# wyhuai/DDNM

Measured on AMD Instinct MI355X. Metric: restored images/sec @256×256, 100 DDIM steps, 4×SR; 1/2/4/8 GPU, higher is better.
Workload: dtype f32 (3x3 convolutions: fp32 operands carried as hi + lo fp16 halves, three fp16 MFMA products per product, fp32 accumulate -- operand error 2^-22, measured closer to fp64 than the fp32 MFMA kernel; everything else fp32); 1 GPU; celeba_hq.yml SVD sr_bicubic 4x, sigma_y=0, eta=0.85, T_sampling=100, batch_size=8 per GPU (BASELINE configs[1]); global_batch=8, image=3x256x256, parallelism=dp1 (image sharding)

## Files before the change

ddnm_amd/_lib.py:

```python
import ctypes
import os
from ctypes import POINTER, Structure, c_char_p, c_float, c_int32, c_int64, c_uint32, c_void_p

_HERE = os.path.dirname(os.path.abspath(__file__))
LIB_PATH = os.path.join(_HERE, "libddnm_hip.so")

c_f32p = c_void_p


class ConvDesc(Structure):
    _fields_ = [
        ("src0", c_void_p), ("src1", c_void_p), ("weight", c_void_p), ("bias", c_void_p),
        ("badd", c_void_p), ("res", c_void_p), ("gn_scale", c_void_p), ("gn_shift", c_void_p),
        ("out", c_void_p),
        ("B", c_int32), ("Hin", c_int32), ("Win", c_int32),
        ("C0", c_int32), ("C1", c_int32), ("Cout", c_int32),
        ("ksize", c_int32), ("stride", c_int32), ("pad", c_int32),
        ("Ho", c_int32), ("Wo", c_int32),
        ("ups", c_int32), ("gn_silu", c_int32), ("out_nchw", c_int32),
        ("badd_stride", c_int32), ("tile", c_int32),
        ("workspace", c_void_p), ("workspace_floats", c_int64),
        ("res_ups", c_int32), ("src_f16", c_int32),
        ("stats_out", c_void_p),
        ("skip0", c_void_p), ("skip1", c_void_p), ("skip_weight", c_void_p),
        ("SC0", c_int32), ("SC1", c_int32),
        ("acc_scale", c_float), ("flags", c_int32),
        ("amax_in", c_void_p),
    ]


class GemmDesc(Structure):
    _fields_ = [
        ("A", c_void_p), ("Bm", c_void_p), ("D", c_void_p), ("C", c_void_p),
        ("M", c_int32), ("N", c_int32), ("K", c_int32),
        ("lda", c_int32), ("ldb", c_int32), ("ldc", c_int32), ("ldd", c_int32),
        ("transb", c_int32), ("batch", c_int32), ("inner", c_int32),
        ("sAo", c_int64), ("sAi", c_int64), ("sBo", c_int64), ("sBi", c_int64),
        ("sCo", c_int64), ("sCi", c_int64), ("sDo", c_int64), ("sDi", c_int64),
        ("alpha", c_float), ("beta", c_float),
        ("transa", c_int32), ("reserved", c_int32),
    ]


class Conv16Desc(Structure):
    _fields_ = [
        ("src", c_void_p), ("weight", c_void_p), ("bias", c_void_p), ("res", c_void_p),
        ("skip0", c_void_p), ("skip1", c_void_p), ("skip_weight", c_void_p),
        ("out", c_void_p), ("stats_out", c_void_p),
        ("workspace", c_void_p), ("workspace_floats", c_int64),
        ("B", c_int32), ("H", c_int32), ("W", c_int32),
        ("Cin", c_int32), ("Cout", c_int32), ("ksize", c_int32),
        ("ups", c_int32), ("res_ups", c_int32),
        ("SC0", c_int32), ("SC1", c_int32),
        ("src1", c_void_p), ("gn_scale", c_void_p), ("gn_shift", c_void_p),
        ("C0", c_int32), ("gn_silu", c_int32),
        ("out_nchw_f32", c_int32), ("reserved", c_int32),
        ("fin_gamma", c_void_p), ("fin_beta", c_void_p), ("fin_film", c_void_p),
        ("fin_scale", c_void_p), ("fin_shift", c_void_p),
        ("fin_eps", c_float), ("fin_film_stride", c_int32), ("fin_groups", c_int32), ("reserved2", c_int32),
    ]


class StepScalars(Structure):
    _fields_ = [("sqrt_1m_at", c_float), ("sqrt_at", c_float), ("sqrt_at_next", c_float),
                ("c1", c_float), ("c2", c_float), ("lam", c_float),
                ("rng_on", c_uint32), ("rng_seed_lo", c_uint32), ("rng_seed_hi", c_uint32), ("rng_iter", c_uint32),
                ("rng_image_base", c_uint32), ("reserved_rng", c_uint32)]


PROTOTYPES = {
    "ddnm_version": (c_int32, []),
    "ddnm_error_string": (c_char_p, [c_int32]),
    "ddnm_build_digest": (c_char_p, []),
    "ddnm_sizeof": (c_int32, [c_int32]),
    "ddnm_conv2d_f32": (c_int32, [POINTER(ConvDesc), c_void_p]),
    "ddnm_conv3x3_small_cout_f32": (c_int32, [POINTER(ConvDesc), c_void_p]),
    "ddnm_conv3x3_small_cout_f32_supported": (c_int32, [POINTER(ConvDesc)]),
    "ddnm_conv2d_f32_tile_n": (c_int32, [POINTER(ConvDesc)]),
    "ddnm_conv2d_f32_workspace_floats": (c_int64, [POINTER(ConvDesc)]),
    "ddnm_conv2d_f32_stats_tiles": (c_int32, [POINTER(ConvDesc)]),
    "ddnm_conv2d_f32_fuses_skip": (c_int32, [POINTER(ConvDesc)]),
    "ddnm_spectral_mix_f32": (c_int32, [c_void_p, c_void_p, c_void_p, c_int64, c_void_p, c_int64, c_float, c_float, c_float,
                                        c_float, c_int32, c_void_p]),
    "ddnm_hq_x0_f32": (c_int32, [c_void_p, c_void_p, c_int64, c_void_p, c_int32, c_int64, c_float, c_float, c_int32,
                                 c_void_p]),
    "ddnm_hq_project_f32": (c_int32, [c_void_p, c_void_p, c_void_p, c_void_p, c_int64, c_float, c_void_p]),
    "ddnm_copy_rect_f32": (c_int32, [c_void_p, c_int32, c_int32, c_int32, c_int32, c_void_p, c_int32, c_int32, c_int32,
                                     c_int32, c_int32, c_int32, c_int32, c_void_p]),
    "ddnm_hq_sample_f32": (c_int32, [c_void_p, c_void_p, c_void_p, c_void_p, c_void_p, c_int64, c_float, c_float, c_float,
                                     c_float, c_void_p]),
    "ddnm_patchify_f32": (c_int32, [c_void_p, c_void_p, c_int32, c_int32, c_int32, c_int32, c_void_p]),
    "ddnm_im2col3x3_f16": (c_int32, [c_void_p, c_void_p, c_void_p, c_void_p, c_void_p, c_int32, c_int32, c_int32, c_int32,
                                     c_int32, c_int32, c_void_p]),
    "ddnm_gn_apply_f16": (c_int32, [c_void_p, c_void_p, c_void_p, c_void_p, c_void_p, c_int32, c_int32, c_int32, c_int32,
                                    c_int32, c_void_p]),
    "ddnm_gn_finalize_tiles_f32": (c_int32, [c_void_p, c_int32, c_int32, c_void_p, c_int32, c_int32, c_void_p, c_void_p,
                                             c_int32, c_int32, c_int32, c_float, c_void_p, c_void_p, c_void_p, c_int32,
                                             c_void_p, c_void_p]),
    "ddnm_gn_finalize_tiles_amax_f32": (c_int32, [c_void_p, c_int32, c_int32, c_void_p, c_int32, c_int32, c_void_p, c_void_p,
                                                  c_int32, c_int32, c_int32, c_float, c_void_p, c_void_p, c_void_p, c_int32,
                                                  c_void_p, c_void_p, c_void_p]),
    "ddnm_amax_bound_f32": (c_int32, [c_void_p, c_int64, c_int32, c_void_p, c_int64, c_int32, c_void_p, c_int32, c_void_p]),
    "ddnm_conv3x3_f16_f32": (c_int32, [POINTER(ConvDesc), c_void_p]),
    "ddnm_conv3x3_f16_supported": (c_int32, [POINTER(ConvDesc)]),
    "ddnm_conv3x3_f16_workspace_floats": (c_int64, [POINTER(ConvDesc)]),
    "ddnm_conv3x3_f16_stats_tiles": (c_int32, [POINTER(ConvDesc)]),
    "ddnm_conv3x3_s16_f32": (c_int32, [POINTER(ConvDesc), c_void_p]),
    "ddnm_conv3x3_s16_supported": (c_int32, [POINTER(ConvDesc)]),
    "ddnm_conv3x3_s16_persistent": (c_int32, [POINTER(ConvDesc)]),
    "ddnm_conv3x3_s16_workspace_floats": (c_int64, [POINTER(ConvDesc)]),
    "ddnm_conv3x3_s16_stats_tiles": (c_int32, [POINTER(ConvDesc)]),
    "ddnm_conv3x3_s16_act_scale": (c_float, []),
    "ddnm_conv_gather_s16_f32": (c_int32, [POINTER(ConvDesc), c_void_p]),
    "ddnm_conv_gather_s16_supported": (c_int32, [POINTER(ConvDesc)]),
    "ddnm_conv_gather_s16_workspace_floats": (c_int64, [POINTER(ConvDesc)]),
    "ddnm_conv_gather_s16_stats_tiles": (c_int32, [POINTER(ConvDesc)]),
    "ddnm_conv16": (c_int32, [POINTER(Conv16Desc), c_void_p]),
    "ddnm_conv16_supported": (c_int32, [POINTER(Conv16Desc)]),
    "ddnm_conv16_fuses_fin": (c_int32, [POINTER(Conv16Desc)]),
    "ddnm_conv16_workspace_floats": (c_int64, [POINTER(Conv16Desc)]),
    "ddnm_conv16_stats_tiles": (c_int32, [POINTER(Conv16Desc)]),
    "ddnm_gn_apply_h16": (c_int32, [c_void_p, c_void_p, c_void_p, c_void_p, c_void_p, c_int32, c_int32, c_int32, c_int32,
                                    c_int32, c_int32, c_int32, c_void_p]),
    "ddnm_im2col3x3_h16": (c_int32, [c_void_p, c_void_p, c_void_p, c_void_p, c_void_p, c_int32, c_int32, c_int32, c_int32,
                                     c_int32, c_int32, c_void_p]),
    "ddnm_nchw_to_nhwc_h16": (c_int32, [c_void_p, c_void_p, c_int32, c_int32, c_int32, c_int32, c_void_p]),
    "ddnm_gn_stats_h16": (c_int32, [c_void_p, c_void_p, c_int32, c_int32, c_int32, c_int32, c_void_p]),
    "ddnm_attn16_d64": (c_int32, [c_void_p, c_void_p, c_int32, c_int32, c_int32, c_void_p]),
    "ddnm_conv1x1_f16_f32": (c_int32, [POINTER(ConvDesc), c_void_p]),
    "ddnm_conv1x1_f16_supported": (c_int32, [POINTER(ConvDesc)]),
    "ddnm_conv1x1_f16_workspace_floats": (c_int64, [POINTER(ConvDesc)]),
    "ddnm_conv1x1_f16_stats_tiles": (c_int32, [POINTER(ConvDesc)]),
    "ddnm_gn_stats_f32": (c_int32, [c_void_p, c_void_p, c_int32, c_int32, c_int32, c_int32, c_int32, c_void_p,
                                    c_int32, c_void_p]),
    "ddnm_gn_nchunk": (c_int32, [c_int32, c_int32]),
    "ddnm_gn_finalize_f32": (c_int32, [c_void_p, c_int32, c_void_p, c_void_p, c_int32, c_int32, c_int32, c_int32,
                                       c_float, c_void_p, c_void_p, c_void_p, c_int32, c_void_p, c_void_p]),
    "ddnm_bgemm_f32": (c_int32, [POINTER(GemmDesc), c_void_p]),
    "ddnm_gn_bwd_f32": (c_int32, [c_void_p, c_void_p, c_int32, c_void_p, c_void_p, c_void_p, c_int32, c_void_p, c_int32,
                                  c_int32, c_int32, c_int32, c_int32, c_int32, c_void_p, c_int32, c_void_p, c_void_p,
                                  c_void_p]),
    "ddnm_gn_bwd_nchunk": (c_int32, [c_int32, c_int32]),
    "ddnm_gn_bwd_h16": (c_int32, [c_void_p, c_void_p, c_int32, c_void_p, c_void_p, c_void_p, c_int32, c_void_p, c_int32,
                                  c_int32, c_int32, c_int32, c_int32, c_int32, c_void_p, c_int32, c_void_p, c_void_p,
                                  c_void_p]),
    "ddnm_pool_tokens_h16": (c_int32, [c_void_p, c_void_p, c_void_p, c_void_p, c_void_p, c_int32, c_int32, c_int32,
                                       c_void_p]),
    "ddnm_pool_tokens_bwd_h16": (c_int32, [c_void_p, c_void_p, c_int32, c_int32, c_int32, c_void_p]),
    "ddnm_attn16_d64_lse": (c_int32, [c_void_p, c_void_p, c_void_p, c_int32, c_int32, c_int32, c_void_p]),
    "ddnm_attn16_d64_bwd": (c_int32, [c_void_p, c_void_p, c_void_p, c_void_p, c_void_p, c_void_p, c_int32, c_int32,
                                      c_int32, c_void_p]),
    "ddnm_softmax_bwd_rows_f32": (c_int32, [c_void_p, c_void_p, c_int64, c_int32, c_int32, c_float, c_void_p]),
    "ddnm_pool_tokens_f32": (c_int32, [c_void_p, c_void_p, c_void_p, c_void_p, c_void_p, c_int32, c_int32, c_int32,
                                       c_void_p]),
    "ddnm_pool_attn_fwd_f32": (c_int32, [c_void_p, c_void_p, c_void_p, c_int32, c_int32, c_int32, c_int32, c_void_p]),
    "ddnm_pool_attn_bwd_f32": (c_int32, [c_void_p, c_void_p, c_void_p, c_void_p, c_int32, c_int32, c_int32, c_int32,
                                         c_void_p]),
    "ddnm_pool_tokens_bwd_f32": (c_int32, [c_void_p, c_void_p, c_int32, c_int32, c_int32, c_void_p]),
    "ddnm_logsoftmax_grad_f32": (c_int32, [c_void_p, c_void_p, c_void_p, c_int32, c_int32, c_void_p]),
    "ddnm_softmax_rows_f32": (c_int32, [c_void_p, c_int64, c_int32, c_int32, c_float, c_void_p]),
    "ddnm_linear_f32": (c_int32, [c_void_p, c_void_p, c_void_p, c_void_p, c_int32, c_int32, c_int32, c_int32,
                                  c_void_p]),
    "ddnm_timestep_embedding_f32": (c_int32, [c_void_p, c_void_p, c_void_p, c_int32, c_int32, c_int32, c_void_p]),
    "ddnm_avgpool2_nhwc_f32": (c_int32, [c_void_p, c_void_p, c_void_p, c_int32, c_void_p, c_int32, c_int32, c_int32,
                                         c_int32, c_void_p]),
    "ddnm_embedding_add_f32": (c_int32, [c_void_p, c_void_p, c_void_p, c_int32, c_int32, c_int32, c_void_p]),
    "ddnm_nchw_im2col3x3_pad_f32": (c_int32, [c_void_p, c_void_p, c_int32, c_int32, c_int32, c_int32, c_int32, c_void_p]),
    "ddnm_nchw_to_nhwc_pad_f32": (c_int32, [c_void_p, c_void_p, c_int32, c_int32, c_int32, c_int32, c_void_p]),
    "ddnm_step_x0_f32": (c_int32, [c_void_p, c_void_p, c_int64, c_void_p, c_int32, c_int64, POINTER(StepScalars),
                                   c_void_p]),
    "ddnm_step_combine_f32": (c_int32, [c_void_p, c_void_p, c_void_p, c_void_p, c_void_p, c_int64, c_void_p,
                                        c_int32, c_int64, POINTER(StepScalars), c_void_p]),
    "ddnm_step_sr_avgpool_f32": (c_int32, [c_void_p, c_void_p, c_int64, c_void_p, c_void_p, c_void_p, c_void_p,
                                           c_int32, c_int32, c_int32, c_int32, POINTER(StepScalars), c_void_p]),
    "ddnm_step_color_f32": (c_int32, [c_void_p, c_void_p, c_int64, c_void_p, c_void_p, c_void_p, c_void_p,
                                      c_int32, c_int32, POINTER(c_float), POINTER(StepScalars), c_void_p]),
    "ddnm_step_inpaint_f32": (c_int32, [c_void_p, c_void_p, c_int64, c_void_p, c_void_p, c_void_p, c_int32,
                                        c_void_p, c_void_p, c_int32, c_int32, POINTER(StepScalars), c_void_p]),
    "ddnm_step_denoise_f32": (c_int32, [c_void_p, c_void_p, c_int64, c_void_p, c_void_p, c_void_p, c_void_p,
                                        c_int32, c_int64, POINTER(StepScalars), c_void_p]),
    "ddnm_axpby_f32": (c_int32, [c_void_p, c_void_p, c_void_p, c_int64, c_float, c_float, c_void_p]),
    "ddnm_axpby_strided_f32": (c_int32, [c_void_p, c_int64, c_void_p, c_void_p, c_int32, c_int64, c_float, c_float,
                                         c_void_p]),
    "ddnm_mask_mix_f32": (c_int32, [c_void_p, c_void_p, c_void_p, c_int32, c_int64, c_void_p, c_int64, c_float, c_float,
                                    c_float, c_float, c_void_p]),
    "ddnm_site_spectral_f32": (c_int32, [c_void_p, c_void_p, c_void_p, c_int32, c_int32, c_int32, c_int32, c_int32,
                                         c_int32, c_int32, c_void_p, c_int32, c_float, c_float, c_float, c_float,
                                         c_void_p]),
    "ddnm_gather_scale_f32": (c_int32, [c_void_p, c_void_p, c_void_p, c_void_p, c_int32, c_int64, c_int64, c_void_p]),
    "ddnm_site_matmul_f32": (c_int32, [c_void_p, c_void_p, c_void_p, c_int32, c_int64, c_int32, c_int64, c_int64, c_int64,
                                       c_int32, c_void_p]),
    "ddnm_mul_planes_f32": (c_int32, [c_void_p, c_void_p, c_int32, c_int64, c_void_p, c_int64, c_void_p]),
    "ddnm_fill_f32": (c_int32, [c_void_p, c_int64, c_float, c_void_p]),
    "ddnm_attn_fused_f32": (c_int32, [c_void_p, c_void_p, c_int32, c_int32, c_int32, c_float, c_float, c_float, c_void_p]),
    "ddnm_attn_fused_supported": (c_int32, [c_int32, c_int32]),
    "ddnm_randn_philox_f32": (c_int32, [c_void_p, c_int32, c_int64, c_uint32, c_uint32, c_uint32, c_uint32, c_void_p]),
    "ddnm_randn_philox_keyed_f32": (c_int32, [c_void_p, c_int32, c_int64, c_void_p, c_uint32, c_void_p]),
    "ddnm_step_combine_keyed_f32": (c_int32, [c_void_p, c_void_p, c_void_p, c_void_p, c_void_p, c_int64, c_void_p,
                                              c_int32, c_int64, POINTER(StepScalars), c_void_p]),
    "ddnm_step_sr_avgpool_keyed_f32": (c_int32, [c_void_p, c_void_p, c_int64, c_void_p, c_void_p, c_void_p, c_void_p,
                                                 c_int32, c_int32, c_int32, c_int32, POINTER(StepScalars), c_void_p]),
    "ddnm_step_color_keyed_f32": (c_int32, [c_void_p, c_void_p, c_int64, c_void_p, c_void_p, c_void_p, c_void_p,
                                            c_int32, c_int32, POINTER(c_float), POINTER(StepScalars), c_void_p]),
    "ddnm_step_inpaint_keyed_f32": (c_int32, [c_void_p, c_void_p, c_int64, c_void_p, c_void_p, c_void_p, c_int32,
                                              c_void_p, c_void_p, c_int32, c_int32, POINTER(StepScalars), c_void_p]),
    "ddnm_step_inpaint_pi_f32": (c_int32, [c_void_p, c_void_p, c_int64, c_void_p, c_void_p, c_int64, c_void_p, c_int32,
                                           c_void_p, c_void_p, c_int32, c_int32, POINTER(StepScalars), c_void_p]),
    "ddnm_step_inpaint_pi_keyed_f32": (c_int32, [c_void_p, c_void_p, c_int64, c_void_p, c_void_p, c_int64, c_void_p, c_int32,
                                                 c_void_p, c_void_p, c_int32, c_int32, POINTER(StepScalars), c_void_p]),
    "ddnm_step_denoise_keyed_f32": (c_int32, [c_void_p, c_void_p, c_int64, c_void_p, c_void_p, c_void_p, c_void_p,
                                              c_int32, c_int64, POINTER(StepScalars), c_void_p]),
    "ddnm_step_plus_spectral_f32": (c_int32, [c_void_p, c_void_p, c_void_p, c_void_p, c_int64, c_void_p, c_void_p, c_int32,
                                              c_int32, c_int64, c_float, c_float, c_float, POINTER(StepScalars), c_void_p]),
    "ddnm_step_plus_spectral_keyed_f32": (c_int32, [c_void_p, c_void_p, c_void_p, c_void_p, c_int64, c_void_p, c_void_p,
                                                    c_int32, c_int32, c_int64, c_float, c_float, c_float,
                                                    POINTER(StepScalars), c_void_p]),
    "ddnm_step_plus_cs_pre_f32": (c_int32, [c_void_p, c_void_p, c_int64, c_void_p, c_void_p, c_void_p, c_void_p, c_void_p,
                                            c_int32, c_int32, c_int32, c_int32, c_float, c_float, c_float, c_float,
                                            c_float, POINTER(StepScalars), c_void_p]),
    "ddnm_step_plus_cs_pre_keyed_f32": (c_int32, [c_void_p, c_void_p, c_int64, c_void_p, c_void_p, c_void_p, c_void_p,
                                                  c_void_p, c_int32, c_int32, c_int32, c_int32, c_float, c_float, c_float,
                                                  c_float, c_float, POINTER(StepScalars), c_void_p]),
    "ddnm_step_plus_cs_post_f32": (c_int32, [c_void_p, c_void_p, c_int32, c_int32, c_int32, c_void_p]),
    "ddnm_renoise_f32": (c_int32, [c_void_p, c_void_p, c_void_p, c_int64, c_float, c_float, c_void_p]),
    "ddnm_op_avgpool_f32": (c_int32, [c_void_p, c_void_p, c_int32, c_int32, c_int32, c_int32, c_void_p]),
    "ddnm_op_upsample_f32": (c_int32, [c_void_p, c_void_p, c_int32, c_int32, c_int32, c_int32, c_void_p]),
    "ddnm_op_color_A_f32": (c_int32, [c_void_p, c_void_p, c_int32, c_int32, POINTER(c_float), c_void_p]),
    "ddnm_op_color_pinv_f32": (c_int32, [c_void_p, c_void_p, c_int32, c_int32, POINTER(c_float), c_void_p]),
    "ddnm_op_inpaint_A_f32": (c_int32, [c_void_p, c_void_p, c_int32, c_void_p, c_int32, c_int32, c_void_p]),
    "ddnm_op_inpaint_pinv_f32": (c_int32, [c_void_p, c_void_p, c_int32, c_void_p, c_int32, c_int32, c_void_p]),
    "ddnm_op_inpaint_A_pi_f32": (c_int32, [c_void_p, c_void_p, c_int32, c_void_p, c_int64, c_int32, c_int32, c_void_p]),
    "ddnm_op_inpaint_pinv_pi_f32": (c_int32, [c_void_p, c_int64, c_void_p, c_int32, c_void_p, c_int32, c_int32, c_void_p]),
    "ddnm_fwht2d_f32": (c_int32, [c_void_p, c_void_p, c_int32, c_int32, c_void_p]),
    "ddnm_fwht2d_masked_f32": (c_int32, [c_void_p, c_void_p, c_int32, c_void_p, c_int32, c_int32, c_void_p,
                                         c_void_p]),
    "ddnm_wh_gather_f32": (c_int32, [c_void_p, c_void_p, c_void_p, c_int32, c_int32, c_int32, c_int32, c_void_p]),
    "ddnm_wh_scatter_f32": (c_int32, [c_void_p, c_void_p, c_void_p, c_int32, c_int32, c_int32, c_int32, c_void_p]),
    "ddnm_finalize_psnr_f32": (c_int32, [c_void_p, c_void_p, c_void_p, c_void_p, c_int32, c_int64, c_void_p]),
    "ddnm_ssim_workspace_elems": (c_int64, [c_int32, c_int32, c_int32, c_int32]),
    "ddnm_ssim_f32": (c_int32, [c_void_p, c_void_p, c_void_p, c_void_p, c_int64, c_int32, c_int32, c_int32, c_int32,
                                c_int32, c_void_p]),
}

_lib = None


class DDNMHipError(RuntimeError):
    pass


ABI_VERSION = 7


def lib():
    global _lib
    if _lib is None:
        from . import build as _build
        want = _build._digest()
        stale = not os.path.exists(LIB_PATH) or not os.path.exists(_build.STAMP) or open(_build.STAMP).read() != want
        if stale and os.environ.get("DDNM_NO_AUTOBUILD") != "1":
            try:
                _build.build(force=False)
            except Exception as e:
                raise DDNMHipError(f"{LIB_PATH} is missing or older than its sources and could not be rebuilt: {e}")
        if not os.path.exists(LIB_PATH):
            raise DDNMHipError(
                f"{LIB_PATH} is missing: build it with `python -m ddnm_amd.build` "
                "(the DDNM hot path has no CPU/PyTorch fallback)")
        import torch
        l = ctypes.CDLL(LIB_PATH)
        for name, (res, args) in PROTOTYPES.items():
            fn = getattr(l, name)
            fn.restype = res
            fn.argtypes = args
        got = l.ddnm_build_digest().decode()
        if got != want:
            raise DDNMHipError(f"{LIB_PATH} was built from different sources (binary {got[:12]}, sources {want[:12]}): "
                               "rebuild it with `python -m ddnm_amd.build --force`")
        if l.ddnm_version() != ABI_VERSION:
            raise DDNMHipError(f"ABI version {l.ddnm_version()} != {ABI_VERSION}")
        for idx, st in enumerate((ConvDesc, GemmDesc, Conv16Desc, StepScalars)):
            if l.ddnm_sizeof(idx) != ctypes.sizeof(st):
                raise DDNMHipError(f"{st.__name__}: ctypes mirror is {ctypes.sizeof(st)} bytes, the binary's struct "
                                   f"{l.ddnm_sizeof(idx)}")
        _lib = l
    return _lib


def check(code, what):
    if code != 0:
        msg = lib().ddnm_error_string(code)
        raise DDNMHipError(f"{what} failed with code {code}: {msg.decode() if msg else '?'}")
```

ddnm_amd/build.py:

```python
import hashlib
import os
import shutil
import subprocess
import sys

HERE = os.path.dirname(os.path.abspath(__file__))
CSRC = os.path.join(HERE, "csrc")
LIB = os.path.join(HERE, "libddnm_hip.so")
STAMP = os.path.join(HERE, ".libddnm_hip.stamp")
OBJ = os.path.join(HERE, "_obj")
SOURCES = ["conv_igemm_f32.hip", "conv_igemm_f16.hip", "conv_s16_persist.hip", "conv_gather_s16.hip", "conv_small_f32.hip", "conv1x1_f16.hip", "conv16.hip", "act16.hip", "attn16.hip", "attn_d512.hip", "attn16_bwd.hip", "gemm_f32.hip", "groupnorm.hip", "misc.hip", "ddnm_step.hip", "fwht.hip", "backward.hip", "metrics.hip"]
FLAGS = ["--offload-arch=gfx950", "-O3", "-std=c++17", "-fPIC", "-shared", "-Wall", "-Wno-unused-function"]


def _hipcc():
    for c in (os.environ.get("HIPCC"), shutil.which("hipcc"), "/opt/rocm/bin/hipcc"):
        if c and os.path.exists(c):
            return c
    raise RuntimeError("hipcc not found (set HIPCC)")


def _digest():
    h = hashlib.sha256()
    for f in sorted(os.listdir(CSRC)) + ["../../include/ddnm_hip.h"]:
        with open(os.path.join(CSRC, f), "rb") as fh:
            h.update(f.encode() + fh.read())
    h.update(" ".join(FLAGS).encode())
    return h.hexdigest()


LAST_BUILD = {"compiled": False}


def build(force=False, verbose=False):
    dig = _digest()
    LAST_BUILD["compiled"] = False
    if not force and os.path.exists(LIB) and os.path.exists(STAMP) and open(STAMP).read() == dig:
        return LIB
    LAST_BUILD["compiled"] = True
    tmp = LIB + f".tmp{os.getpid()}"
    os.makedirs(OBJ, exist_ok=True)
    hh = hashlib.sha256()
    for f in sorted(os.listdir(CSRC)) + ["../../include/ddnm_hip.h"]:
        if f.endswith(".h"):
            with open(os.path.join(CSRC, f), "rb") as fh:
                hh.update(f.encode() + fh.read())
    hh.update(" ".join(FLAGS).encode())
    cflags = [f for f in FLAGS if f != "-shared"]
    jobs, objs = [], []
    for s in SOURCES:
        h = hashlib.sha256(hh.digest())
        with open(os.path.join(CSRC, s), "rb") as fh:
            h.update(fh.read())
        extra = [f'-DDDNM_BUILD_DIGEST="{dig}"'] if s == "misc.hip" else []
        h.update(" ".join(extra).encode())
        obj = os.path.join(OBJ, f"{s}.{h.hexdigest()[:16]}.o")
        objs.append(obj)
        if force or not os.path.exists(obj):
            jobs.append((s, [_hipcc()] + cflags + extra + ["-c", os.path.join(CSRC, s), "-o", obj + f".tmp{os.getpid()}"], obj))
    if jobs:
        from concurrent.futures import ThreadPoolExecutor

        def run(job):
            s, cmd, obj = job
            if verbose:
                print(" ".join(cmd), flush=True)
            r = subprocess.run(cmd, capture_output=True, text=True)
            if r.returncode == 0:
                os.replace(cmd[-1], obj)
            return s, r
        with ThreadPoolExecutor(max_workers=min(len(jobs), os.cpu_count() or 4)) as ex:
            results = list(ex.map(run, jobs))
        bad = [(s, r) for s, r in results if r.returncode != 0]
        for s, r in results:
            if r.returncode != 0 or (verbose and r.stderr):
                sys.stderr.write(r.stdout + r.stderr)
        if bad:
            raise RuntimeError("hipcc failed: " + ", ".join(s for s, _ in bad))
    keep = set(objs)
    for f in os.listdir(OBJ):
        if os.path.join(OBJ, f) not in keep and f.endswith(".o"):
            os.remove(os.path.join(OBJ, f))
    cmd = [_hipcc(), "--offload-arch=gfx950", "-shared", "-fPIC"] + objs + ["-o", tmp]
    if verbose:
        print(" ".join(cmd))
    r = subprocess.run(cmd, capture_output=True, text=True)
    if r.returncode != 0:
        sys.stderr.write(r.stdout + r.stderr)
        raise RuntimeError("hipcc (link) failed")
    os.replace(tmp, LIB)
    with open(STAMP, "w") as f:
        f.write(dig)
    return LIB


if __name__ == "__main__":
    print(build(force="--force" in sys.argv, verbose=True))
```

ddnm_amd/csrc/conv_common.h:

```cpp
#pragma once
#include "common.h"

struct ConvArgs {
    ddnm_conv_desc d;
    int Cin, ntaps, Hs, Ws;
    int m_tiles, n_tiles;
    int tiles_x;
    int TW, TW_log2;
    int ksplit;
    float* ws;
};

static inline bool conv_sizes_addressable(const ddnm_conv_desc* d) {
    const int64_t lim = (int64_t)1 << 31;
    const int64_t out_el = (int64_t)d->B * d->Ho * d->Wo * d->Cout;
    const int64_t hs = d->ups ? d->Hin / 2 : d->Hin, ws = d->ups ? d->Win / 2 : d->Win;
    const int64_t cmax = d->C0 > d->C1 ? d->C0 : d->C1;
    const int64_t src_b = (int64_t)d->B * hs * ws * cmax * (d->src_f16 ? 2 : 4);
    const int64_t cout_pad = ((int64_t)d->Cout + 127) / 128 * 128;
    const int64_t w_b = cout_pad * d->ksize * d->ksize * ((int64_t)d->C0 + d->C1) * 4;
    const int64_t sk_el = (int64_t)d->B * d->Ho * d->Wo * (d->SC0 > d->SC1 ? d->SC0 : d->SC1);
    return out_el < lim && src_b < lim && w_b < lim && sk_el < lim;
}

bool conv3x3_s16_persist_eligible(const ConvArgs& p);
int conv3x3_s16_persist_launch(const ConvArgs& p, hipStream_t s);

struct TileMap {
    int img, ty0, tx0, th_unused, TW, TW_log2, flat_base, Wo;
    bool two_d;
    __device__ __forceinline__ void pixel(int r, int& oy, int& ox) const {
        if (two_d) {
            oy = ty0 + (r >> TW_log2);
            ox = tx0 + (r & (TW - 1));
        } else {
            const int pix = flat_base + r;
            oy = pix / Wo;
            ox = pix - oy * Wo;
        }
    }
};

template <int BM>
__device__ __forceinline__ TileMap make_tilemap(const ConvArgs& p, int m_tile) {
    TileMap t;
    const int HWo = p.d.Ho * p.d.Wo;
    const int per_img = HWo / BM;
    t.img = m_tile / per_img;
    const int t_in_img = m_tile - t.img * per_img;
    t.TW = p.TW;
    t.TW_log2 = p.TW_log2;
    t.Wo = p.d.Wo;
    t.two_d = p.tiles_x != 0;
    if (t.two_d) {
        const int ty = t_in_img / p.tiles_x, tx = t_in_img - ty * p.tiles_x;
        t.ty0 = ty * (BM >> p.TW_log2);
        t.tx0 = tx << p.TW_log2;
        t.flat_base = 0;
    } else {
        t.ty0 = t.tx0 = 0;
        t.flat_base = t_in_img * BM;
    }
    return t;
}

template <int WM, int WN, int MT, int NT, bool RES_ALL_UPFRONT = false>
__device__ __forceinline__ void conv_epilogue(const ConvArgs& p, const TileMap& tm, int n_tile, int m_tile, int slice,
                                              f32x16 (&acc)[MT][NT], float* lds, const float acc_scale = 1.f) {
    constexpr int BN = WN * NT * 32;
    const ddnm_conv_desc& d = p.d;
    const int lane = threadIdx.x & 63, wave = threadIdx.x >> 6;
    const int wm = wave / WN, wn = wave % WN;
    const int ncol = lane & 31, rsel = 4 * (lane >> 5);
    const bool partial = p.ksplit > 1;
    float* __restrict__ ws = partial ? p.ws + (size_t)slice * d.B * d.Ho * d.Wo * d.Cout : nullptr;
    const float* __restrict__ res = d.res;
    float* __restrict__ out = d.out;
    const bool want_stats = d.stats_out != nullptr && !partial;
    float cs[NT], cq[NT];
#pragma unroll
    for (int j = 0; j < NT; ++j) cs[j] = cq[j] = 0.f;
    if (RES_ALL_UPFRONT && d.Cout % BN == 0 && !d.out_nchw) {
        unsigned o[MT][NT][16];
        float rv[MT][NT][16];
        const bool use_res = res && !partial;
#pragma unroll
        for (int i = 0; i < MT; ++i)
#pragma unroll
            for (int r = 0; r < 16; ++r) {
                const int row = (wm * MT + i) * 32 + (r & 3) + 8 * (r >> 2) + rsel;
                int oy, ox;
                tm.pixel(row, oy, ox);
                const unsigned pix = (unsigned)((tm.img * d.Ho + oy) * d.Wo + ox);
                const unsigned rpix = d.res_ups ? (unsigned)((tm.img * (d.Ho >> 1) + (oy >> 1)) * (d.Wo >> 1) + (ox >> 1)) : pix;
#pragma unroll
                for (int j = 0; j < NT; ++j) {
                    const unsigned n = (unsigned)(n_tile * BN + (wn * NT + j) * 32 + ncol);
                    o[i][j][r] = pix * (unsigned)d.Cout + n;
                    rv[i][j][r] = use_res ? res[(size_t)rpix * d.Cout + n] : 0.f;
                }
            }
#pragma unroll
        for (int j = 0; j < NT; ++j) {
            const int n = n_tile * BN + (wn * NT + j) * 32 + ncol;
            float add = 0.f;
            if (!partial) {
                if (d.bias) add = d.bias[n];
                if (d.badd) add += d.badd[(size_t)tm.img * d.badd_stride + n];
            }
#pragma unroll
            for (int i = 0; i < MT; ++i)
#pragma unroll
                for (int r = 0; r < 16; ++r) {
                    const float v = acc[i][j][r] * acc_scale + add + rv[i][j][r];
                    if (partial) ws[o[i][j][r]] = v;
                    else out[o[i][j][r]] = v;
                    cs[j] += v;
                    cq[j] = __builtin_fmaf(v, v, cq[j]);
                }
        }
    } else {
#pragma unroll
    for (int j = 0; j < NT; ++j) {
        const int n = n_tile * BN + (wn * NT + j) * 32 + ncol;
        if (n >= d.Cout) continue;
        float add = 0.f;
        if (!partial) {
            if (d.bias) add = d.bias[n];
            if (d.badd) add += d.badd[(size_t)tm.img * d.badd_stride + n];
        }
#pragma unroll
        for (int i = 0; i < MT; ++i) {
            unsigned o[16];
#pragma unroll
            for (int r = 0; r < 16; ++r) {
                const int row = (wm * MT + i) * 32 + (r & 3) + 8 * (r >> 2) + rsel;
                int oy, ox;
                tm.pixel(row, oy, ox);
                const unsigned pix = (unsigned)((tm.img * d.Ho + oy) * d.Wo + ox);
                if (d.res_ups && res && !partial) {
                    o[r] = pix;
                } else {
                    o[r] = d.out_nchw && !partial ? (unsigned)(((tm.img * d.Cout + n) * d.Ho + oy) * d.Wo + ox)
                                                  : pix * (unsigned)d.Cout + (unsigned)n;
                }
            }
            float rv[16];
            if (res && !partial && d.res_ups) {
                const unsigned hw = (unsigned)(d.Ho * d.Wo);
#pragma unroll
                for (int r = 0; r < 16; ++r) {
                    const unsigned pin = o[r] - (unsigned)tm.img * hw;
                    const unsigned oy = pin / (unsigned)d.Wo, ox = pin - oy * (unsigned)d.Wo;
                    rv[r] = res[(size_t)((tm.img * (d.Ho >> 1) + (int)(oy >> 1)) * (d.Wo >> 1) + (int)(ox >> 1)) * d.Cout + n];
                    o[r] = o[r] * (unsigned)d.Cout + (unsigned)n;
                }
            } else {
#pragma unroll
                for (int r = 0; r < 16; ++r) rv[r] = (res && !partial) ? res[o[r]] : 0.f;
            }
#pragma unroll
            for (int r = 0; r < 16; ++r) {
                const float v = acc[i][j][r] * acc_scale + add + rv[r];
                if (partial) ws[o[r]] = v;
                else out[o[r]] = v;
                cs[j] += v;
                cq[j] = __builtin_fmaf(v, v, cq[j]);
            }
            if constexpr (MT * NT > 4) __builtin_amdgcn_sched_barrier(0);
        }
    }
    }
    if (want_stats) {
#pragma unroll
        for (int j = 0; j < NT; ++j) {
            cs[j] += __shfl_xor(cs[j], 32);
            cq[j] += __shfl_xor(cq[j], 32);
        }
        __syncthreads();
        if (lane < 32) {
#pragma unroll
            for (int j = 0; j < NT; ++j) {
                const int c = (wn * NT + j) * 32 + lane;
                lds[(wm * BN + c) * 2 + 0] = cs[j];
                lds[(wm * BN + c) * 2 + 1] = cq[j];
            }
        }
        __syncthreads();
        for (int c = threadIdx.x; c < BN; c += 256) {
            const int n = n_tile * BN + c;
            if (n < d.Cout) {
                float a = 0.f, q = 0.f;
#pragma unroll
                for (int w = 0; w < WM; ++w) { a += lds[(w * BN + c) * 2]; q += lds[(w * BN + c) * 2 + 1]; }
                d.stats_out[((size_t)m_tile * d.Cout + n) * 2 + 0] = a;
                d.stats_out[((size_t)m_tile * d.Cout + n) * 2 + 1] = q;
            }
        }
    }
}

typedef _Float16 half8 __attribute__((ext_vector_type(8)));
typedef _Float16 half4 __attribute__((ext_vector_type(4)));

#define DDNM_S16_ASCALE 1.0f
__device__ __forceinline__ void split_store(_Float16* dst, f32x4 v, const float s) {
    v = v * s;
    const half4 h = {(_Float16)v.x, (_Float16)v.y, (_Float16)v.z, (_Float16)v.w};
    const half4 l = {(_Float16)(v.x - (float)h.x), (_Float16)(v.y - (float)h.y), (_Float16)(v.z - (float)h.z),
                     (_Float16)(v.w - (float)h.w)};
    *reinterpret_cast<half4*>(dst) = h;
    *reinterpret_cast<half4*>(dst + 32) = l;
}
__device__ __forceinline__ void split_store(_Float16* dst, f32x4 v) {
    const half4 h = {(_Float16)v.x, (_Float16)v.y, (_Float16)v.z, (_Float16)v.w};
    const half4 l = {(_Float16)(v.x - (float)h.x), (_Float16)(v.y - (float)h.y), (_Float16)(v.z - (float)h.z),
                     (_Float16)(v.w - (float)h.w)};
    *reinterpret_cast<half4*>(dst) = h;
    *reinterpret_cast<half4*>(dst + 32) = l;
}

__device__ __forceinline__ void s16_operand_scale(const float* __restrict__ amax_in, int img, bool down_only,
                                                  float& scale, float& inv_scale) {
    scale = inv_scale = 1.f;
    if (amax_in == nullptr) return;
    const unsigned* __restrict__ w = reinterpret_cast<const unsigned*>(amax_in) + (size_t)img * DDNM_AMAX_N;
    unsigned m = 0u;
#pragma unroll
    for (int i = 0; i < DDNM_AMAX_N; ++i) m = w[i] > m ? w[i] : m;
    m = __builtin_amdgcn_readfirstlane(m);
    int e = (int)((m >> 23) & 0xffu);
    e = e < 47 ? 47 : (e > 207 ? 207 : e);
    int k = 14 - (e - 127);
    if (down_only && k > 0) k = 0;
    scale = __uint_as_float((unsigned)(127 + k) << 23);
    inv_scale = __uint_as_float((unsigned)(127 - k) << 23);
}

__device__ __forceinline__ f32x4 gn_act(f32x4 v, const f32x4 gsc, const f32x4 gsh, int silu) {
    v = v * gsc + gsh;
    if (silu) { v.x = silu_f(v.x); v.y = silu_f(v.y); v.z = silu_f(v.z); v.w = silu_f(v.w); }
    return v;
}


static __global__ __launch_bounds__(256) void conv_splitk_reduce_kernel(const ConvArgs p, size_t total4) {
    const ddnm_conv_desc& d = p.d;
    const size_t slab4 = total4;
    const int c4n = d.Cout >> 2;
    const size_t hw = (size_t)d.Ho * d.Wo;
    for (size_t i = (size_t)blockIdx.x * 256 + threadIdx.x; i < total4; i += (size_t)gridDim.x * 256) {
        f32x4 v = reinterpret_cast<const f32x4*>(p.ws)[i];
        for (int s = 1; s < p.ksplit; ++s) v = v + reinterpret_cast<const f32x4*>(p.ws)[i + s * slab4];
        const int n = (int)(i % c4n) * 4;
        const size_t pix = i / c4n;
        const size_t b = pix / hw;
        if (d.bias) v = v + *reinterpret_cast<const f32x4*>(d.bias + n);
        if (d.badd) v = v + *reinterpret_cast<const f32x4*>(d.badd + b * d.badd_stride + n);
        if (d.res) {
            if (d.res_ups) {
                const size_t p2 = pix - b * hw;
                const size_t oy = p2 / d.Wo, ox = p2 - oy * d.Wo;
                v = v + *reinterpret_cast<const f32x4*>(d.res + ((b * (d.Ho >> 1) + (oy >> 1)) * (d.Wo >> 1) + (ox >> 1)) * d.Cout + n);
            } else {
                v = v + reinterpret_cast<const f32x4*>(d.res)[i];
            }
        }
        reinterpret_cast<f32x4*>(d.out)[i] = v;
    }
}

static __global__ __launch_bounds__(256) void conv_splitk_reduce_stats_kernel(const ConvArgs p, int tpi) {
    __shared__ f32x4 red[2][256];
    const ddnm_conv_desc& d = p.d;
    const int c4n = d.Cout >> 2;
    const int rows = 256 / c4n, active = rows * c4n;
    const int hw = d.Ho * d.Wo, P = hw / tpi;
    const int b = blockIdx.x / tpi, t = blockIdx.x - b * tpi;
    const size_t slab4 = (size_t)d.B * hw * c4n;
    const int tid = threadIdx.x;
    f32x4 s = {0.f, 0.f, 0.f, 0.f}, ss = {0.f, 0.f, 0.f, 0.f};
    if (tid < active) {
        const int c4 = tid % c4n, prow = tid / c4n, n = c4 * 4;
        f32x4 add = {0.f, 0.f, 0.f, 0.f};
        if (d.bias) add = add + *reinterpret_cast<const f32x4*>(d.bias + n);
        if (d.badd) add = add + *reinterpret_cast<const f32x4*>(d.badd + (size_t)b * d.badd_stride + n);
        for (int pp = prow; pp < P; pp += rows) {
            const int p2 = t * P + pp;
            const size_t i = ((size_t)b * hw + p2) * c4n + c4;
            f32x4 v = reinterpret_cast<const f32x4*>(p.ws)[i];
            for (int k = 1; k < p.ksplit; ++k) v = v + reinterpret_cast<const f32x4*>(p.ws)[i + k * slab4];
            v = v + add;
            if (d.res) {
                if (d.res_ups) {
                    const int oy = p2 / d.Wo, ox = p2 - oy * d.Wo;
                    v = v + *reinterpret_cast<const f32x4*>(d.res + (((size_t)b * (d.Ho >> 1) + (oy >> 1)) * (d.Wo >> 1) + (ox >> 1)) * d.Cout + n);
                } else {
                    v = v + reinterpret_cast<const f32x4*>(d.res)[i];
                }
            }
            reinterpret_cast<f32x4*>(d.out)[i] = v;
            s += v;
            ss += v * v;
        }
    }
    red[0][tid] = s;
    red[1][tid] = ss;
    __syncthreads();
    if (tid < c4n) {
        for (int r = 1; r < rows; ++r) { s += red[0][r * c4n + tid]; ss += red[1][r * c4n + tid]; }
        float* o = d.stats_out + ((size_t)blockIdx.x * d.Cout + tid * 4) * 2;
        f32x4 lo = {s.x, ss.x, s.y, ss.y}, hi = {s.z, ss.z, s.w, ss.w};
        reinterpret_cast<f32x4*>(o)[0] = lo;
        reinterpret_cast<f32x4*>(o)[1] = hi;
    }
}

static inline int splitk_stats_tiles(const ddnm_conv_desc* d) {
    const int hw = d->Ho * d->Wo;
    if (d->out_nchw || d->Cout % 4 || d->Cout > 1024 || hw % 4) return 0;
    int tpi = hw / 4 < 128 ? hw / 4 : 128;
    while (tpi > 1 && hw % tpi) --tpi;
    return tpi;
}

static inline int launch_splitk_reduce(const ConvArgs& p, hipStream_t s) {
    const ddnm_conv_desc& d = p.d;
    if (d.stats_out) {
        const int tpi = splitk_stats_tiles(&d);
// ... 11 lines not shown
```

ddnm_amd/csrc/conv_igemm_f16.hip:

```cpp
#include "conv_common.h"

typedef unsigned u32x4 __attribute__((ext_vector_type(4)));

constexpr int KC16 = 64;
constexpr int F16_BM = 256;
constexpr int F16_KS_TARGET = 256;
constexpr int LDH = KC16 + 8;

template <int WM, int WN, int MT, int NT, bool SRC16, bool SPLIT = false, bool ASCALE = false>
__global__ __launch_bounds__(WM * WN * 64, 1) void conv3x3_halo_f16_kernel(const ConvArgs p) {
    static_assert(!(SPLIT && SRC16), "the split form reads fp32 activations");
    static_assert(SPLIT || !ASCALE, "operand scaling belongs to the split form");
    constexpr int NTHREADS = WM * WN * 64;
    constexpr int BM = WM * MT * 32, BN = WN * NT * 32;
    constexpr int MAXH = BM == 512 ? 612 : (BM == 256 ? 340 : (BM == 128 ? 204 : 136));
    constexpr int KCH = SPLIT ? KC16 / 2 : KC16;
    constexpr int WE = SPLIT ? 2 : 1;
    constexpr int HVEC = SRC16 ? 8 : 4;
    constexpr int HCOLS = KCH / HVEC;
    constexpr int HROWS_PER_PASS = NTHREADS / HCOLS;
    constexpr int HR = (MAXH + HROWS_PER_PASS - 1) / HROWS_PER_PASS;
    static_assert(KC16 == 64, "an LDS weight row is 128 bytes");
    constexpr int BCOLS = 8;
    constexpr int BROWS_PER_PASS = NTHREADS / BCOLS;
// ... 98 lines not shown
            if (row < MAXH) {
                _Float16* dst = &Hs[hbuf * MAXH * LDH + row * LDH + hc * HVEC];
                if constexpr (SRC16) {
                    *reinterpret_cast<uint4*>(dst) = h_st[i];
                } else {
                    f32x4 v = __builtin_bit_cast(f32x4, h_st[i]);
                    if (has_gn && hoff[i] >= 0) v = gn_act(v, gsc, gsh, d.gn_silu);
                    if constexpr (SPLIT && ASCALE) {
                        split_store(dst, v, ascale);
                    } else if constexpr (SPLIT) {
                        split_store(dst, v);
                    } else {
                        half4 h = {(_Float16)v.x, (_Float16)v.y, (_Float16)v.z, (_Float16)v.w};
                        *reinterpret_cast<half4*>(dst) = h;
                    }
                }
            }
        }
    };
    auto stage_b = [&](int buf) {
        char* dst = Bs + buf * WTILE;
        auto put = [&](int r, const uint4& v) { *reinterpret_cast<uint4*>(dst + r * 128 + ((c8 ^ ((r >> 1) & 7)) << 4)) = v; };
        put(brow, b_st0);
        if constexpr (BR >= 2) put(brow + BROWS_PER_PASS, b_st1);
        if constexpr (BR == 4) {
            put(brow + 2 * BROWS_PER_PASS, b_st2);
            put(brow + 3 * BROWS_PER_PASS, b_st3);
        }
    };

    f32x16 acc[MT][NT];
#pragma unroll
    for (int i = 0; i < MT; ++i)
#pragma unroll
        for (int j = 0; j < NT; ++j)
#pragma unroll
            for (int r = 0; r < 16; ++r) acc[i][j][r] = 0.f;

    int a_off[MT];
#pragma unroll
    for (int i = 0; i < MT; ++i) {
        const int m = (wm * MT + i) * 32 + (lane & 31);
        const int ty = m >> p.TW_log2, tx = m & (p.TW - 1);
        a_off[i] = (ty * HWd + tx) * LDH + (lane >> 5) * 8;
    }
    const int b_frag = ((wn * NT * 32 + (lane & 31)) * 128) + ((((lane >> 5) ^ (((lane & 31) >> 1) & 7))) << 4);

    auto mfma_tap = [&](int tap, int buf, int hbuf = 0) {
        const int ky = tap / 3, kx = tap - 3 * ky;
        const int tap_off = (ky * HWd + kx) * LDH + hbuf * MAXH * LDH;
        const char* bf = Bs + buf * WTILE;
        if constexpr (SPLIT) {
#pragma unroll
            for (int ks = 0; ks < KC16 / 32; ++ks) {
                half8 ah[MT], al[MT], bh[NT], bl[NT];
#pragma unroll
                for (int i = 0; i < MT; ++i) {
                    ah[i] = *reinterpret_cast<const half8*>(Hs + a_off[i] + tap_off + ks * 16);
                    al[i] = *reinterpret_cast<const half8*>(Hs + a_off[i] + tap_off + ks * 16 + 32);
                }
#pragma unroll
                for (int j = 0; j < NT; ++j) {
                    bh[j] = *reinterpret_cast<const half8*>(bf + ((b_frag ^ (ks << 5)) + j * 32 * 128));
                    bl[j] = *reinterpret_cast<const half8*>(bf + ((b_frag ^ ((ks + 2) << 5)) + j * 32 * 128));
                }
#pragma unroll
                for (int i = 0; i < MT; ++i)
#pragma unroll
                    for (int j = 0; j < NT; ++j)
                        acc[i][j] = __builtin_amdgcn_mfma_f32_32x32x16_f16(al[i], bh[j], acc[i][j], 0, 0, 0);
#pragma unroll
                for (int i = 0; i < MT; ++i)
#pragma unroll
                    for (int j = 0; j < NT; ++j)
                        acc[i][j] = __builtin_amdgcn_mfma_f32_32x32x16_f16(ah[i], bl[j], acc[i][j], 0, 0, 0);
#pragma unroll
                for (int i = 0; i < MT; ++i)
#pragma unroll
                    for (int j = 0; j < NT; ++j)
                        acc[i][j] = __builtin_amdgcn_mfma_f32_32x32x16_f16(ah[i], bh[j], acc[i][j], 0, 0, 0);
            }
            return;
        }
#pragma unroll
        for (int ks = 0; ks < KC16 / 16; ++ks) {
            half8 a[MT], b[NT];
#pragma unroll
            for (int i = 0; i < MT; ++i) a[i] = *reinterpret_cast<const half8*>(Hs + a_off[i] + tap_off + ks * 16);
#pragma unroll
            for (int j = 0; j < NT; ++j) b[j] = *reinterpret_cast<const half8*>(bf + ((b_frag ^ (ks << 5)) + j * 32 * 128));
#pragma unroll
            for (int i = 0; i < MT; ++i)
#pragma unroll
                for (int j = 0; j < NT; ++j)
                    acc[i][j] = __builtin_amdgcn_mfma_f32_32x32x16_f16(a[i], b[j], acc[i][j], 0, 0, 0);
        }
    };

    if (SPLIT && wave >= WM * WN / 2) __builtin_amdgcn_s_setprio(1);
    if (c_begin < c_end) {
        prefetch_halo(c_begin);
        const int last_step = (c_end - c_begin) * 9 - 1;
        auto issue_step = [&](int q, int buf) {
            q = q < last_step ? q : last_step;
            const int ch = q / 9;
            issue_w(c_begin + ch, q - 9 * ch, buf);
        };
        issue_step(0, 0);
        issue_step(1, 1);
        stage_halo_part(0, 0, HR);
        int hb = 0, step0 = 0;
        for (int chunk = c_begin; chunk < c_end; ++chunk, step0 += 9) {
            const bool more = chunk + 1 < c_end;
#pragma unroll
            for (int tap = 0; tap < 9; ++tap) {
                const int cur = tap % NWB, step = step0 + tap;
                constexpr int GNV = SRC16 ? 0 : 2;
                if (tap == 1 || tap == 2) {
                    asm volatile("s_waitcnt vmcnt(%0) lgkmcnt(0)" ::"n"(BR + HSPLIT + GNV) : "memory");
                } else if (tap == 4 || tap == 5) {
                    asm volatile("s_waitcnt vmcnt(%0) lgkmcnt(0)" ::"n"(BR + HR - HSPLIT) : "memory");
                } else {
                    asm volatile("s_waitcnt vmcnt(%0) lgkmcnt(0)" ::"n"(BR) : "memory");
                }
                __builtin_amdgcn_s_barrier();
                asm volatile("" ::: "memory");
                issue_step(step + 2, cur >= 1 ? cur - 1 : NWB - 1);
                asm volatile("" ::: "memory");
                __builtin_amdgcn_sched_barrier(0);
                const int nchunk = more ? chunk + 1 : chunk;
                if (tap == 0) prefetch_halo_part(nchunk, 0, HSPLIT, more);
                if (tap == 3) {
                    if (more) stage_halo_part(hb ^ 1, 0, HSPLIT);
                    prefetch_halo_part(nchunk, HSPLIT, HR, more);
                }
                if (tap == 6 && more) stage_halo_part(hb ^ 1, HSPLIT, HR);
                __builtin_amdgcn_sched_barrier(0);
                mfma_tap(tap, cur, hb);
            }
            hb ^= 1;
        }
        asm volatile("s_waitcnt vmcnt(0)" ::: "memory");
        __syncthreads();
    }
    if (d.skip0 != nullptr) {
        const int SCin = d.SC0 + d.SC1, nsk_all = SCin / KCH;
        const int s_begin = (int)((long)nsk_all * slice / p.ksplit), s_end = (int)((long)nsk_all * (slice + 1) / p.ksplit);
        const _Float16* swbase = reinterpret_cast<const _Float16*>(d.skip_weight) + (size_t)(n_tile * BN + brow) * SCin * WE + c8 * 8;
        constexpr int SCOLS = KCH / 4;
        constexpr int SR = BM * SCOLS / NTHREADS;
        const int sc = tid % SCOLS, srow = tid / SCOLS;
        int soff[SR], sdst[SR];
#pragma unroll
        for (int i = 0; i < SR; ++i) {
            const int m = srow + (NTHREADS / SCOLS) * i;
            const int ty = m >> p.TW_log2, tx = m & (p.TW - 1);
            const int iy = tm.ty0 + ty, ix = tm.tx0 + tx;
            const int sy = d.ups ? (iy >> 1) : iy, sx = d.ups ? (ix >> 1) : ix;
            soff[i] = (img * p.Hs + sy) * p.Ws + sx;
            sdst[i] = ((ty + 1) * HWd + tx + 1) * LDH + sc * 4;
        }
        f32x4 s_st[SR];
        auto prefetch_skip = [&](int ch) {
            const int cb = ch * KCH;
            const float* src;
            int cs, coff;
            if (cb < d.SC0) { src = d.skip0; cs = d.SC0; coff = cb; }
            else { src = d.skip1; cs = d.SC1; coff = cb - d.SC0; }
#pragma unroll
            for (int i = 0; i < SR; ++i) s_st[i] = *reinterpret_cast<const f32x4*>(src + (size_t)soff[i] * cs + coff + sc * 4);
            b_st0 = *reinterpret_cast<const uint4*>(swbase + cb * WE);
            if constexpr (BR >= 2) b_st1 = *reinterpret_cast<const uint4*>(swbase + ((size_t)BROWS_PER_PASS * SCin + cb) * WE);
            if constexpr (BR == 4) {
                b_st2 = *reinterpret_cast<const uint4*>(swbase + ((size_t)(2 * BROWS_PER_PASS) * SCin + cb) * WE);
                b_st3 = *reinterpret_cast<const uint4*>(swbase + ((size_t)(3 * BROWS_PER_PASS) * SCin + cb) * WE);
            }
        };
        if (s_begin < s_end) prefetch_skip(s_begin);
        for (int ch = s_begin; ch < s_end; ++ch) {
            __syncthreads();
#pragma unroll
            for (int i = 0; i < SR; ++i) {
                const f32x4 v = s_st[i];
                if constexpr (SPLIT && ASCALE) {
                    split_store(&Hs[sdst[i]], v, ascale);
                } else if constexpr (SPLIT) {
                    split_store(&Hs[sdst[i]], v);
                } else {
                    half4 h = {(_Float16)v.x, (_Float16)v.y, (_Float16)v.z, (_Float16)v.w};
                    *reinterpret_cast<half4*>(&Hs[sdst[i]]) = h;
                }
            }
            stage_b(0);
            __syncthreads();
            if (ch + 1 < s_end) prefetch_skip(ch + 1);
            mfma_tap(4, 0);
        }
    }
    conv_epilogue<WM, WN, MT, NT, (MT * NT <= 4)>(p, tm, n_tile, m_tile, slice, acc, stat_lds, epi_scale);
}

struct PlanF16 {
    int BM, TW, TW_log2, tiles_x, ksplit;
};

static bool plan_f16(const ddnm_conv_desc* d, PlanF16* pl, int kch = KC16) {
    const int HWo = d->Ho * d->Wo;
    const int Cin = d->C0 + d->C1;
    if (d->ksize != 3 || d->stride != 1 || d->pad != 1 || d->Ho != d->Hin || d->Wo != d->Win) return false;
    if (Cin % kch || d->C0 % kch || d->Cout % 128 || d->out_nchw) return false;
    {
        const int64_t px = (int64_t)d->B * (d->ups ? d->Hin / 2 : d->Hin) * (d->ups ? d->Win / 2 : d->Win);
        const int64_t cmax = d->C0 > d->C1 ? d->C0 : d->C1;
        if (px * cmax * (d->src_f16 ? 2 : 4) >= (int64_t)1 << 31) return false;
    }
    pl->BM = F16_BM;
    if (HWo % pl->BM) return false;
    int tw = 32;
    while (tw > 8 && (d->Wo % tw || d->Ho % (pl->BM / tw))) tw >>= 1;
    if (d->Wo % tw || d->Ho % (pl->BM / tw)) return false;
    pl->TW = tw;
    pl->TW_log2 = tw == 32 ? 5 : (tw == 16 ? 4 : 3);
    pl->tiles_x = d->Wo / tw;
    const long tiles = (long)d->B * (HWo / pl->BM) * (d->Cout / 128);
    int ks = 1;
    const int nchunks = Cin / kch;
    if (tiles < 192) {
        ks = (int)((F16_KS_TARGET + tiles - 1) / tiles);
        if (ks > nchunks) ks = nchunks;
        if (ks > 16) ks = 16;
    }
    pl->ksplit = ks;
    return true;
}

extern "C" int ddnm_conv3x3_f16_supported(const ddnm_conv_desc* d) {
    PlanF16 pl;
    return d && plan_f16(d, &pl) ? 1 : 0;
}

extern "C" int64_t ddnm_conv3x3_f16_workspace_floats(const ddnm_conv_desc* d) {
    PlanF16 pl;
    if (!d || !plan_f16(d, &pl)) return DDNM_E_SHAPE;
    return pl.ksplit > 1 ? (int64_t)pl.ksplit * d->B * d->Ho * d->Wo * d->Cout : 0;
}

extern "C" int ddnm_conv3x3_f16_stats_tiles(const ddnm_conv_desc* d) {
    PlanF16 pl;
    if (!d || !plan_f16(d, &pl)) return DDNM_E_SHAPE;
    return pl.ksplit > 1 ? splitk_stats_tiles(d) : d->Ho * d->Wo / pl.BM;
}

static int run_f16(const ddnm_conv_desc* d, void* stream, bool split) {
    const int kch = split ? KC16 / 2 : KC16;
    if (!d || !d->src0 || !d->weight || !d->out) return DDNM_E_BADARG;
    if (split && (d->src_f16 || !(d->acc_scale > 0.f))) return DDNM_E_BADARG;
    if (split && !d->amax_in && (!d->gn_scale || d->skip0)) return DDNM_E_BADARG;
    if (d->B <= 0 || d->Cout <= 0 || d->Ho <= 0 || d->Wo <= 0) return DDNM_E_BADARG;
    if (!conv_sizes_addressable(d)) return DDNM_E_SHAPE;
    if (d->C1 > 0 && !d->src1) return DDNM_E_BADARG;
    if (d->gn_scale && !d->gn_shift) return DDNM_E_BADARG;
    if (d->src_f16 && d->gn_scale) return DDNM_E_BADARG;
    if (d->ups && ((d->Hin | d->Win) & 1)) return DDNM_E_SHAPE;
    if (d->res_ups && ((d->Ho | d->Wo) & 1)) return DDNM_E_SHAPE;
    PlanF16 pl;
    if (!plan_f16(d, &pl, kch)) return DDNM_E_SHAPE;
    if (d->skip0) {
        if (d->ups || !d->skip_weight || d->SC0 <= 0 || d->SC0 % kch || d->SC1 % kch || (d->SC1 > 0 && !d->skip1))
            return DDNM_E_SHAPE;
    }
    if (pl.ksplit > 1) {
        const int64_t need = (int64_t)pl.ksplit * d->B * d->Ho * d->Wo * d->Cout;
        if (!d->workspace || d->workspace_floats < need) {
            if (d->stats_out) return DDNM_E_BADARG;
            pl.ksplit = 1;
        }
    }
    ConvArgs p;
    p.d = *d;
    p.Cin = d->C0 + d->C1;
    p.ntaps = 9;
    p.Hs = d->ups ? d->Hin / 2 : d->Hin;
    p.Ws = d->ups ? d->Win / 2 : d->Win;
    p.m_tiles = d->B * (d->Ho * d->Wo / pl.BM);
    p.n_tiles = d->Cout / 128;
    p.TW = pl.TW;
    p.TW_log2 = pl.TW_log2;
    p.tiles_x = pl.tiles_x;
    p.ksplit = pl.ksplit;
    p.ws = d->workspace;
    hipStream_t s = (hipStream_t)stream;
    if (split && !(d->flags & DDNM_CONV_ONE_TILE) && conv3x3_s16_persist_eligible(p)) return conv3x3_s16_persist_launch(p, s);
    const dim3 grid(p.m_tiles * p.n_tiles, pl.ksplit);
    if (split && d->amax_in) { DDNM_LAUNCH((conv3x3_halo_f16_kernel<4, 2, 2, 2, false, true, true>), grid, dim3(512), 0, s, p); }
    else if (split) { DDNM_LAUNCH((conv3x3_halo_f16_kernel<4, 2, 2, 2, false, true>), grid, dim3(512), 0, s, p); }
    else if (d->src_f16) { DDNM_LAUNCH((conv3x3_halo_f16_kernel<4, 2, 2, 2, true>), grid, dim3(512), 0, s, p); }
    else { DDNM_LAUNCH((conv3x3_halo_f16_kernel<4, 2, 2, 2, false>), grid, dim3(512), 0, s, p); }
    if (pl.ksplit > 1) return launch_splitk_reduce(p, s);
    return 0;
}

extern "C" int ddnm_conv3x3_f16_f32(const ddnm_conv_desc* d, void* stream) { return run_f16(d, stream, false); }

extern "C" int ddnm_conv3x3_s16_f32(const ddnm_conv_desc* d, void* stream) { return run_f16(d, stream, true); }

extern "C" float ddnm_conv3x3_s16_act_scale(void) { return DDNM_S16_ASCALE; }

extern "C" int ddnm_conv3x3_s16_persistent(const ddnm_conv_desc* d) {
    PlanF16 pl;
    if (!d || d->src_f16 || (d->flags & DDNM_CONV_ONE_TILE) || !plan_f16(d, &pl, KC16 / 2) || pl.ksplit != 1) return 0;
    ConvArgs p;
    p.d = *d;
    p.Cin = d->C0 + d->C1;
    p.m_tiles = d->B * (d->Ho * d->Wo / pl.BM);
    p.n_tiles = d->Cout / 128;
    p.TW = pl.TW;
    p.ksplit = 1;
    return conv3x3_s16_persist_eligible(p) ? 1 : 0;
}

extern "C" int ddnm_conv3x3_s16_supported(const ddnm_conv_desc* d) {
    PlanF16 pl;
    return d && !d->src_f16 && plan_f16(d, &pl, KC16 / 2) ? 1 : 0;
}

extern "C" int64_t ddnm_conv3x3_s16_workspace_floats(const ddnm_conv_desc* d) {
    PlanF16 pl;
    if (!d || !plan_f16(d, &pl, KC16 / 2)) return DDNM_E_SHAPE;
    return pl.ksplit > 1 ? (int64_t)pl.ksplit * d->B * d->Ho * d->Wo * d->Cout : 0;
}

extern "C" int ddnm_conv3x3_s16_stats_tiles(const ddnm_conv_desc* d) {
    PlanF16 pl;
    if (!d || !plan_f16(d, &pl, KC16 / 2)) return DDNM_E_SHAPE;
    return pl.ksplit > 1 ? splitk_stats_tiles(d) : d->Ho * d->Wo / pl.BM;
}
```

ddnm_amd/csrc/conv_s16_persist.hip:

```cpp
#include <type_traits>

#include "conv_common.h"

typedef unsigned u32x4 __attribute__((ext_vector_type(4)));

namespace {
constexpr int P_WM = 4, P_WN = 2, P_MT = 2, P_NT = 2;
constexpr int P_NTHREADS = 512, P_BN = 128;
constexpr int P_LDH = 72, P_KCH = 32;
constexpr int P_MAXH = 340, P_HWD = 34;
constexpr int P_HCOLS = 8, P_HRPP = P_NTHREADS / P_HCOLS, P_HR = (P_MAXH + P_HRPP - 1) / P_HRPP, P_HSPLIT = (P_HR + 1) / 2;
constexpr int P_BR = P_BN / (P_NTHREADS / 8);
constexpr int P_NWB = 3, P_WTILE = P_BN * 128;
constexpr int P_HBYTES = 2 * P_MAXH * P_LDH * 2;
constexpr int P_NOUT = P_MT * P_NT * 16;
enum { K_MID = 0, K_LAST = 1, K_FIRST = 2 };

constexpr int p_spread(int tap) { return tap == 0 ? 10 : (tap <= 6 ? 9 : 0); }
constexpr int p_first_of(int tap) { return tap == 0 ? 0 : (tap <= 7 ? 10 + 9 * (tap - 1) : P_NOUT); }
static_assert(p_first_of(7) == P_NOUT, "64 values over taps 0..6");
constexpr int p_extra(int kind, int tap, bool has_res, bool ascale) {
    return kind == K_FIRST ? p_spread(tap) + (tap == 0 ? 1 : 0)
                           : (kind == K_LAST ? (tap == 0 ? 4 + (ascale ? 1 : 0) : 0) + (has_res ? p_spread(tap) : 0) : 0);
}
constexpr int p_base(int tap) {
    return (tap == 1 || tap == 2) ? P_BR + P_HSPLIT + 2 : ((tap == 4 || tap == 5) ? P_BR + P_HR - P_HSPLIT : P_BR);
}
constexpr int p_wait(int kind, int tap, bool has_res, bool ascale) {
    return p_base(tap) + (tap >= 1 ? p_extra(kind, tap - 1, has_res, ascale) : 0) + (tap >= 2 ? p_extra(kind, tap - 2, has_res, ascale) : 0);
}
static_assert(p_wait(K_FIRST, 2, true, true) < 64 && p_wait(K_LAST, 2, true, true) < 64, "vmcnt is a 6-bit field");

template <int V>
using ic = std::integral_constant<int, V>;

}

template <bool ASCALE, bool HAS_RES, bool HAS_SKIP = false>
__global__ __launch_bounds__(P_NTHREADS, 1) void conv3x3_s16_persist_kernel(const ConvArgs p, const int total) {
    static_assert(!HAS_SKIP || (ASCALE && !HAS_RES), "a fused shortcut reads a raw operand (bound required) and replaces the residual");
    constexpr int WM = P_WM, WN = P_WN, MT = P_MT, NT = P_NT, BN = P_BN, HR = P_HR, HSPLIT = P_HSPLIT, LDH = P_LDH, KCH = P_KCH;
    constexpr int MAXH = P_MAXH, HWd = P_HWD, NWB = P_NWB, WTILE = P_WTILE, BR = P_BR, NTHREADS = P_NTHREADS;
    __shared__ __attribute__((aligned(1024))) char lds_all[NWB * WTILE + P_HBYTES + WM * BN * 2 * 4];
    char* const Bs = lds_all;
    _Float16* const Hs = reinterpret_cast<_Float16*>(lds_all + NWB * WTILE);
    float* const stat_lds = reinterpret_cast<float*>(lds_all + NWB * WTILE + P_HBYTES);

    const ddnm_conv_desc& d = p.d;
    const int tid = threadIdx.x, lane = tid & 63;
    const int wave = __builtin_amdgcn_readfirstlane(tid >> 6);
    const int wm = wave / WN, wn = wave % WN;
    const int G = gridDim.x;
    const int per_img = (d.Ho * d.Wo) >> 8;
    const int Cout = d.Cout, Wo = d.Wo;

    int t_img, t_ty0, t_tx0, t_ntile, t_mtile;
    auto tile_of = [&](int v) {
        const int tile_id = xcd_swizzle(v, total);
        t_ntile = tile_id % p.n_tiles;
        t_mtile = tile_id / p.n_tiles;
        t_img = t_mtile / per_img;
        const int t = t_mtile - t_img * per_img;
        const int ty = t / p.tiles_x;
        t_ty0 = ty * 8;
        t_tx0 = (t - ty * p.tiles_x) * 32;
    };

    const int hc = tid % P_HCOLS, prow = tid / P_HCOLS;
    int hoff[HR];
    auto set_hoff = [&]() {
#pragma unroll
        for (int i = 0; i < HR; ++i) {
            const int row = prow + P_HRPP * i;
            const int hy = row / HWd, hx = row - hy * HWd;
            const int iy = t_ty0 - 1 + hy, ix = t_tx0 - 1 + hx;
            const bool ok = row < MAXH && (unsigned)iy < (unsigned)d.Hin && (unsigned)ix < (unsigned)d.Win;
            const int sy = d.ups ? (iy >> 1) : iy, sx = d.ups ? (ix >> 1) : ix;
            hoff[i] = ok ? (t_img * p.Hs + sy) * p.Ws + sx : -1;
        }
    };

    const int lrow = lane >> 3, lpiece = lane & 7;
    const int wswz = (((wave & 1) << 2) | (lrow >> 1));
    const unsigned w_rowlen = 9u * (unsigned)p.Cin * 4u;
    const __amdgpu_buffer_rsrc_t r_w = __builtin_amdgcn_make_buffer_rsrc(
        const_cast<void*>(reinterpret_cast<const void*>(d.weight)), 0, (unsigned)p.n_tiles * BN * w_rowlen, 0x00020000);
    const unsigned w_lane = (unsigned)(wave * 8 + lrow) * w_rowlen + (unsigned)((lpiece ^ wswz) * 16);
    unsigned w_soff = 0;
    auto issue_w = [&](int chunk, int tap, int buf) {
        char* dst = Bs + buf * WTILE + wave * 1024;
        const unsigned so = w_soff + ((unsigned)tap * p.Cin + (unsigned)chunk * KCH) * 4u;
#pragma unroll
        for (int j = 0; j < BR; ++j)
            __builtin_amdgcn_raw_ptr_buffer_load_lds(r_w, (__attribute__((address_space(3))) void*)(dst + j * (NTHREADS / 64) * 1024), 16,
                                                     w_lane, so + (unsigned)j * (NTHREADS / 8) * w_rowlen, 0, 0);
    };

    const int nchunks = p.Cin / KCH;
    uint4 h_st[HR];
    f32x4 gsc = {1.f, 1.f, 1.f, 1.f}, gsh = {0.f, 0.f, 0.f, 0.f};
    const bool has_gn = d.gn_scale != nullptr;
    constexpr unsigned HOOB = 0x80000000u;
    const __amdgpu_buffer_rsrc_t r_s0 = __builtin_amdgcn_make_buffer_rsrc(
        const_cast<void*>(reinterpret_cast<const void*>(d.src0)), 0, (unsigned)d.B * p.Hs * p.Ws * d.C0 * 4, 0x00020000);
    const __amdgpu_buffer_rsrc_t r_s1 = __builtin_amdgcn_make_buffer_rsrc(
        const_cast<void*>(reinterpret_cast<const void*>(d.C1 > 0 ? d.src1 : d.src0)), 0,
        (unsigned)d.B * p.Hs * p.Ws * (d.C1 > 0 ? d.C1 : d.C0) * 4, 0x00020000);
    const __amdgpu_buffer_rsrc_t r_amax = __builtin_amdgcn_make_buffer_rsrc(
        const_cast<void*>(reinterpret_cast<const void*>(d.amax_in)), 0, d.amax_in ? (unsigned)d.B * DDNM_AMAX_N * 4u : 0u, 0x00020000);
    auto amax_request = [&](int img, bool live) {
        return __builtin_amdgcn_raw_buffer_load_b32(r_amax, (lane < DDNM_AMAX_N && live) ? (unsigned)lane * 4u : HOOB, (unsigned)img * DDNM_AMAX_N * 4u, 0);
    };
    auto amax_scales = [&](unsigned m, bool down_only, float& scale, float& inv_scale) {
#pragma unroll
        for (int o = 32; o >= 1; o >>= 1) {
            const unsigned t = (unsigned)__shfl_xor((int)m, o);
            m = t > m ? t : m;
        }
        m = __builtin_amdgcn_readfirstlane(m);
        int e = (int)((m >> 23) & 0xffu);
        e = e < 47 ? 47 : (e > 207 ? 207 : e);
        int k = 14 - (e - 127);
        if (down_only && k > 0) k = 0;
        scale = __uint_as_float((unsigned)(127 + k) << 23);
        inv_scale = __uint_as_float((unsigned)(127 - k) << 23);
    };
    unsigned amax_bits = 0;
    int gn_img = 0;
    float ascale_stage = 1.f;
    auto prefetch_halo_part = [&](int chunk, int i0, int i1, bool live = true) {
        const int cb = chunk * KCH;
        const bool first = cb < d.C0;
        const unsigned cs = first ? d.C0 : d.C1, coff = first ? cb : cb - d.C0;
        const __amdgpu_buffer_rsrc_t r_s = first ? r_s0 : r_s1;
#pragma unroll
        for (int i = 0; i < HR; ++i) {
            if (i < i0 || i >= i1) continue;
            const unsigned vo = (hoff[i] >= 0 && live) ? ((unsigned)hoff[i] * cs + hc * 4) * 4 : HOOB;
            const u32x4 v = __builtin_amdgcn_raw_buffer_load_b128(r_s, vo, coff * 4, 0);
            h_st[i] = uint4{v.x, v.y, v.z, v.w};
        }
        if (i0 == 0) {
            const float* gb = has_gn ? d.gn_scale + (size_t)gn_img * p.Cin + hc * 4 + cb : reinterpret_cast<const float*>(d.weight);
            const float* hb2 = has_gn ? d.gn_shift + (size_t)gn_img * p.Cin + hc * 4 + cb : reinterpret_cast<const float*>(d.weight);
            gsc = *reinterpret_cast<const f32x4*>(gb);
            gsh = *reinterpret_cast<const f32x4*>(hb2);
        }
    };
    auto stage_halo_part = [&](int hbuf, int i0, int i1) {
#pragma unroll
        for (int i = 0; i < HR; ++i) {
            if (i < i0 || i >= i1) continue;
            const int row = prow + P_HRPP * i;
            if (row < MAXH) {
                _Float16* dst = &Hs[hbuf * MAXH * LDH + row * LDH + hc * 4];
                f32x4 v = __builtin_bit_cast(f32x4, h_st[i]);
                if (has_gn && hoff[i] >= 0) v = gn_act(v, gsc, gsh, d.gn_silu);
                if constexpr (ASCALE) split_store(dst, v, ascale_stage);
                else split_store(dst, v);
            }
        }
    };

    f32x16 acc[MT][NT];
#pragma unroll
    for (int i = 0; i < MT; ++i)
#pragma unroll
        for (int j = 0; j < NT; ++j)
#pragma unroll
            for (int r = 0; r < 16; ++r) acc[i][j][r] = 0.f;
    int a_off[MT];
#pragma unroll
    for (int i = 0; i < MT; ++i) {
        const int m = (wm * MT + i) * 32 + (lane & 31);
        a_off[i] = ((m >> 5) * HWd + (m & 31)) * LDH + (lane >> 5) * 8;
    }
    const int b_frag = ((wn * NT * 32 + (lane & 31)) * 128) + ((((lane >> 5) ^ (((lane & 31) >> 1) & 7))) << 4);
    auto mfma_tap = [&](int tap, int buf, int hbuf) {
        const int ky = tap / 3, kx = tap - 3 * ky;
        const int tap_off = (ky * HWd + kx) * LDH + hbuf * MAXH * LDH;
        const char* bf = Bs + buf * WTILE;
#pragma unroll
        for (int ks = 0; ks < 2; ++ks) {
            half8 ah[MT], al[MT], bh[NT], bl[NT];
#pragma unroll
            for (int i = 0; i < MT; ++i) {
                ah[i] = *reinterpret_cast<const half8*>(Hs + a_off[i] + tap_off + ks * 16);
                al[i] = *reinterpret_cast<const half8*>(Hs + a_off[i] + tap_off + ks * 16 + 32);
            }
#pragma unroll
            for (int j = 0; j < NT; ++j) {
                bh[j] = *reinterpret_cast<const half8*>(bf + ((b_frag ^ (ks << 5)) + j * 32 * 128));
                bl[j] = *reinterpret_cast<const half8*>(bf + ((b_frag ^ ((ks + 2) << 5)) + j * 32 * 128));
            }
#pragma unroll
            for (int i = 0; i < MT; ++i)
#pragma unroll
                for (int j = 0; j < NT; ++j) acc[i][j] = __builtin_amdgcn_mfma_f32_32x32x16_f16(al[i], bh[j], acc[i][j], 0, 0, 0);
#pragma unroll
            for (int i = 0; i < MT; ++i)
#pragma unroll
                for (int j = 0; j < NT; ++j) acc[i][j] = __builtin_amdgcn_mfma_f32_32x32x16_f16(ah[i], bl[j], acc[i][j], 0, 0, 0);
#pragma unroll
            for (int i = 0; i < MT; ++i)
#pragma unroll
                for (int j = 0; j < NT; ++j) acc[i][j] = __builtin_amdgcn_mfma_f32_32x32x16_f16(ah[i], bh[j], acc[i][j], 0, 0, 0);
        }
    };

    const int ncol = lane & 31, rsel = 4 * (lane >> 5);
    const unsigned out_bytes = (unsigned)d.B * d.Ho * Wo * Cout * 4u;
    const __amdgpu_buffer_rsrc_t r_out = __builtin_amdgcn_make_buffer_rsrc(reinterpret_cast<void*>(d.out), 0, out_bytes, 0x00020000);
    const __amdgpu_buffer_rsrc_t r_res = __builtin_amdgcn_make_buffer_rsrc(
        const_cast<void*>(reinterpret_cast<const void*>(d.res)), 0, d.res ? out_bytes : 0u, 0x00020000);
    const __amdgpu_buffer_rsrc_t r_bias = __builtin_amdgcn_make_buffer_rsrc(
        const_cast<void*>(reinterpret_cast<const void*>(d.bias)), 0, d.bias ? (unsigned)Cout * 4u : 0u, 0x00020000);
    const __amdgpu_buffer_rsrc_t r_badd = __builtin_amdgcn_make_buffer_rsrc(
        const_cast<void*>(reinterpret_cast<const void*>(d.badd)), 0, d.badd ? (unsigned)d.B * d.badd_stride * 4u : 0u, 0x00020000);
    const __amdgpu_buffer_rsrc_t r_stats = __builtin_amdgcn_make_buffer_rsrc(
        reinterpret_cast<void*>(d.stats_out), 0, d.stats_out ? (unsigned)p.m_tiles * Cout * 8u : 0u, 0x00020000);
    const unsigned o_lane = (unsigned)(((wm * MT * Wo + rsel) * Cout + wn * NT * 32 + ncol) * 4);
    auto o_soff = [&](unsigned base, int k) {
        const int i = k >> 5, j = (k >> 4) & 1, r = k & 15;
        return base + (unsigned)(((i * Wo + (r & 3) + 8 * (r >> 2)) * Cout + j * 32) * 4);
    };
    auto tile_base = [&]() { return (unsigned)((((t_img * d.Ho + t_ty0) * Wo + t_tx0) * Cout + t_ntile * BN) * 4); };
    const unsigned c_lane = (unsigned)((wn * NT * 32 + ncol) * 4);
    const unsigned st_lane = tid < 2 * BN ? (unsigned)(tid * 4) : HOOB;

    float outv[P_NOUT];
    float addv[NT][2];
#pragma unroll
    for (int k = 0; k < P_NOUT; ++k) outv[k] = 0.f;
#pragma unroll
    for (int j = 0; j < NT; ++j) addv[j][0] = addv[j][1] = 0.f;
    unsigned pend_base = 0, pend_stats = 0;
    unsigned cur_base = 0, cur_stats = 0;
    float epi_cur = d.acc_scale;

    auto finalize = [&]() {
        float cs[NT], cq[NT];
#pragma unroll
        for (int j = 0; j < NT; ++j) {
            cs[j] = cq[j] = 0.f;
            const float add = addv[j][0];
#pragma unroll
            for (int i = 0; i < MT; ++i)
#pragma unroll
                for (int r = 0; r < 16; ++r) {
                    const int k = (i * NT + j) * 16 + r;
                    const float v = acc[i][j][r] * epi_cur + add + (HAS_RES ? outv[k] : 0.f);
                    outv[k] = v;
                    cs[j] += v;
                    cq[j] = __builtin_fmaf(v, v, cq[j]);
                    acc[i][j][r] = 0.f;
                }
            cs[j] += __shfl_xor(cs[j], 32);
            cq[j] += __shfl_xor(cq[j], 32);
        }
        if (lane < 32) {
#pragma unroll
            for (int j = 0; j < NT; ++j) {
                const int c = (wn * NT + j) * 32 + lane;
                stat_lds[(wm * BN + c) * 2 + 0] = cs[j];
                stat_lds[(wm * BN + c) * 2 + 1] = cq[j];
            }
        }
        pend_base = cur_base;
        pend_stats = cur_stats;
    };
    auto store_stats = [&]() {
        const int c = (tid >> 1) & (BN - 1), which = tid & 1;
        float a = 0.f;
#pragma unroll
        for (int w = 0; w < WM; ++w) a += stat_lds[(w * BN + c) * 2 + which];
        __builtin_amdgcn_raw_buffer_store_b32(__float_as_uint(a), r_stats, st_lane, pend_stats, 0);
    };

    int v = blockIdx.x;
    tile_of(v);
    set_hoff();
    gn_img = t_img;
    w_soff = (unsigned)t_ntile * BN * w_rowlen;
    cur_base = tile_base();
    cur_stats = (unsigned)((t_mtile * Cout + t_ntile * BN) * 8);
    if constexpr (ASCALE) {
        float inv;
        amax_scales(amax_request(t_img, true), has_gn, ascale_stage, inv);
        epi_cur = d.acc_scale * inv;
    }
    prefetch_halo_part(0, 0, HR);
    issue_w(0, 0, 0);
    issue_w(0, 1, 1);
    stage_halo_part(0, 0, HR);
    if (wave >= WM * WN / 2) __builtin_amdgcn_s_setprio(1);

    int hb = 0, n_img_next = 0;
    bool have_next = false;
    float epi_next = epi_cur;
    unsigned next_base = 0, next_stats = 0, next_wsoff = 0;

    auto tap_body = [&](auto KIND, auto TAP, int chunk) {
        constexpr int kind = decltype(KIND)::value, tap = decltype(TAP)::value;
        constexpr int cur = tap % NWB;
        asm volatile("s_waitcnt vmcnt(%0) lgkmcnt(0)" ::"n"(p_wait(kind, tap, HAS_RES, ASCALE)) : "memory");
        __builtin_amdgcn_s_barrier();
        asm volatile("" ::: "memory");
        if constexpr (kind == K_LAST && tap >= 7) {
            if (tap == 7 && have_next) w_soff = next_wsoff;
            issue_w(0, tap - 7, cur >= 1 ? cur - 1 : NWB - 1);
        } else {
            issue_w(tap + 2 < 9 ? chunk : chunk + 1, (tap + 2) % 9, cur >= 1 ? cur - 1 : NWB - 1);
        }
        asm volatile("" ::: "memory");
        __builtin_amdgcn_sched_barrier(0);
        const int nchunk = kind == K_LAST ? 0 : chunk + 1;
        const bool live = kind == K_LAST ? have_next : true;
        if constexpr (tap == 0) prefetch_halo_part(nchunk, 0, HSPLIT, live);
        if constexpr (tap == 3) {
            if constexpr (kind == K_LAST && ASCALE) {
                if (have_next) {
                    float inv;
                    amax_scales(amax_bits, has_gn, ascale_stage, inv);
                    epi_next = d.acc_scale * inv;
                }
            }
            if (live) stage_halo_part(hb ^ 1, 0, HSPLIT);
            prefetch_halo_part(nchunk, HSPLIT, HR, live);
        }
        if constexpr (tap == 6) {
            if (live) stage_halo_part(hb ^ 1, HSPLIT, HR);
        }
        asm volatile("" ::: "memory");
        __builtin_amdgcn_sched_barrier(0);
        if constexpr (kind == K_FIRST) {
            if constexpr (tap == 0) store_stats();
#pragma unroll
            for (int k = p_first_of(tap); k < p_first_of(tap + 1); ++k)
                __builtin_amdgcn_raw_buffer_store_b32(__float_as_uint(outv[k]), r_out, o_lane, o_soff(pend_base, k), 0);
        }
        if constexpr (kind == K_LAST) {
            if constexpr (tap == 0) {
                if constexpr (ASCALE) amax_bits = amax_request(n_img_next, have_next);
#pragma unroll
                for (int j = 0; j < NT; ++j) {
                    addv[j][0] = __uint_as_float(__builtin_amdgcn_raw_buffer_load_b32(r_bias, c_lane + j * 128, (unsigned)(t_ntile * BN * 4), 0));
                    addv[j][1] = __uint_as_float(__builtin_amdgcn_raw_buffer_load_b32(r_badd, c_lane + j * 128, (unsigned)((t_img * d.badd_stride + t_ntile * BN) * 4), 0));
                }
            }
            if constexpr (tap == 4) {
#pragma unroll
                for (int j = 0; j < NT; ++j) addv[j][0] = addv[j][0] + addv[j][1];
            }
            if constexpr (HAS_RES) {
#pragma unroll
                for (int k = p_first_of(tap); k < p_first_of(tap + 1); ++k)
                    outv[k] = __uint_as_float(__builtin_amdgcn_raw_buffer_load_b32(r_res, o_lane, o_soff(cur_base, k), 0));
            }
        }
        asm volatile("" ::: "memory");
        __builtin_amdgcn_sched_barrier(0);
        mfma_tap(tap, cur, hb);
    };
    auto run_chunk = [&](auto KIND, int chunk) {
        tap_body(KIND, ic<0>{}, chunk);
        tap_body(KIND, ic<1>{}, chunk);
        tap_body(KIND, ic<2>{}, chunk);
        tap_body(KIND, ic<3>{}, chunk);
        tap_body(KIND, ic<4>{}, chunk);
        tap_body(KIND, ic<5>{}, chunk);
        tap_body(KIND, ic<6>{}, chunk);
        tap_body(KIND, ic<7>{}, chunk);
        tap_body(KIND, ic<8>{}, chunk);
        hb ^= 1;
    };

    constexpr int SR = 4;
    const int sc8 = tid & 7, srow = tid >> 3;
    int s_img = 0, s_ty0 = 0, s_tx0 = 0;
    f32x4 s_st[SR];
    const int SCin = d.SC0 + d.SC1;
    const unsigned sw_rowlen = (unsigned)SCin * 4u;
    const __amdgpu_buffer_rsrc_t r_sw = __builtin_amdgcn_make_buffer_rsrc(
        const_cast<void*>(reinterpret_cast<const void*>(d.skip_weight)), 0, HAS_SKIP ? (unsigned)p.n_tiles * BN * sw_rowlen : 0u, 0x00020000);
    const unsigned sw_lane = (unsigned)(wave * 8 + lrow) * sw_rowlen + (unsigned)((lpiece ^ wswz) * 16);
    unsigned sw_soff = 0;
    auto skip_setup = [&](int img, int ty0, int tx0, int ntile) {
        s_img = img;
        s_ty0 = ty0;
        s_tx0 = tx0;
        sw_soff = (unsigned)ntile * BN * sw_rowlen;
    };
    auto skip_prefetch = [&](int ch) {
        const int cb = ch * KCH;
        const float* src;
        int cs, coff;
        if (cb < d.SC0) { src = d.skip0; cs = d.SC0; coff = cb; }
        else { src = d.skip1; cs = d.SC1; coff = cb - d.SC0; }
#pragma unroll
        for (int i = 0; i < SR; ++i) {
            const int m = srow + 64 * i;
            const int so = (s_img * p.Hs + s_ty0 + (m >> 5)) * p.Ws + s_tx0 + (m & 31);
            s_st[i] = *reinterpret_cast<const f32x4*>(src + (size_t)so * cs + coff + sc8 * 4);
        }
    };
    auto skip_issue_w = [&](int ch) {
        char* dst = Bs + 2 * WTILE + wave * 1024;
#pragma unroll
        for (int j = 0; j < BR; ++j)
            __builtin_amdgcn_raw_ptr_buffer_load_lds(r_sw, (__attribute__((address_space(3))) void*)(dst + j * (NTHREADS / 64) * 1024), 16,
                                                     sw_lane, sw_soff + (unsigned)ch * KCH * 4u + (unsigned)j * (NTHREADS / 8) * sw_rowlen, 0, 0);
    };
    auto skip_phase = [&](int hbuf, float ascale_cur, int img, int ty0, int tx0, int ntile) {
        const int nsk = SCin / KCH;
        skip_setup(img, ty0, tx0, ntile);
        skip_prefetch(0);
        for (int ch = 0; ch < nsk; ++ch) {
            __syncthreads();
            skip_issue_w(ch);
#pragma unroll
            for (int i = 0; i < SR; ++i) {
                const int m = srow + 64 * i;
                split_store(&Hs[hbuf * MAXH * LDH + (((m >> 5) + 1) * HWd + (m & 31) + 1) * LDH + sc8 * 4], s_st[i], ascale_cur);
            }
            asm volatile("s_waitcnt vmcnt(0)" ::: "memory");
            __syncthreads();
            if (ch + 1 < nsk) skip_prefetch(ch + 1);
            mfma_tap(4, 2, hbuf);
        }
    };

    bool pending = false;
    for (;;) {
        int c0 = 0;
        if (pending) {
            run_chunk(ic<K_FIRST>{}, 0);
            c0 = 1;
        }
        for (int chunk = c0; chunk < nchunks - 1; ++chunk) run_chunk(ic<K_MID>{}, chunk);
        const int vn = v + G;
        have_next = vn < total;
        const int c_img = t_img, c_ntile = t_ntile;
        const float ascale_cur = ascale_stage;
        const int c_ty0 = t_ty0, c_tx0 = t_tx0;
        if (have_next) {
            tile_of(vn);
            set_hoff();
            gn_img = t_img;
            next_wsoff = (unsigned)t_ntile * BN * w_rowlen;
            next_base = tile_base();
            next_stats = (unsigned)((t_mtile * Cout + t_ntile * BN) * 8);
            n_img_next = t_img;
        }
        {
            const int n_img = t_img, n_ntile = t_ntile;
            t_img = c_img;
            t_ntile = c_ntile;
            run_chunk(ic<K_LAST>{}, nchunks - 1);
            t_img = n_img;
            t_ntile = n_ntile;
        }
        if constexpr (HAS_SKIP) skip_phase(hb ^ 1, ascale_cur, c_img, c_ty0, c_tx0, c_ntile);
        finalize();
        if (!have_next) break;
        v = vn;
        cur_base = next_base;
        cur_stats = next_stats;
        epi_cur = epi_next;
        pending = true;
    }
    __syncthreads();
    store_stats();
#pragma unroll
    for (int k = 0; k < P_NOUT; ++k) __builtin_amdgcn_raw_buffer_store_b32(__float_as_uint(outv[k]), r_out, o_lane, o_soff(pend_base, k), 0);
}

bool conv3x3_s16_persist_eligible(const ConvArgs& p) {
    const ddnm_conv_desc& d = p.d;
    const long tiles = (long)p.m_tiles * p.n_tiles;
    if (d.skip0 && (!d.amax_in || d.res)) return false;
    return p.ksplit == 1 && tiles >= 512 && p.TW == 32 && !d.res_ups && !d.out_nchw && p.Cin / P_KCH >= 2 &&
           (int64_t)d.B * d.Ho * d.Wo * d.Cout * 4 < ((int64_t)1 << 31) && (int64_t)p.m_tiles * d.Cout * 8 < ((int64_t)1 << 31);
}

int conv3x3_s16_persist_launch(const ConvArgs& p, hipStream_t s) {
    int dev = 0, cus = 0;
    if (hipGetDevice(&dev) != hipSuccess || hipDeviceGetAttribute(&cus, hipDeviceAttributeMultiprocessorCount, dev) != hipSuccess || cus <= 0)
        cus = 256;
    const int total = p.m_tiles * p.n_tiles;
    cus -= cus % 8;
    const dim3 grid(total < cus ? total : cus);
    const bool asc = p.d.amax_in != nullptr, res = p.d.res != nullptr;
    if (p.d.skip0) { DDNM_LAUNCH((conv3x3_s16_persist_kernel<true, false, true>), grid, dim3(P_NTHREADS), 0, s, p, total); }
    else if (asc && res) { DDNM_LAUNCH((conv3x3_s16_persist_kernel<true, true>), grid, dim3(P_NTHREADS), 0, s, p, total); }
    else if (asc) { DDNM_LAUNCH((conv3x3_s16_persist_kernel<true, false>), grid, dim3(P_NTHREADS), 0, s, p, total); }
    else if (res) { DDNM_LAUNCH((conv3x3_s16_persist_kernel<false, true>), grid, dim3(P_NTHREADS), 0, s, p, total); }
    else { DDNM_LAUNCH((conv3x3_s16_persist_kernel<false, false>), grid, dim3(P_NTHREADS), 0, s, p, total); }
    return 0;
}
```

ddnm_amd/guided_diffusion/models.py:

```python
import math
import os
from collections import OrderedDict

import torch

from .. import ops
from . import _net

GN_EPS = 1e-6
SPLIT16 = os.environ.get("DDNM_CONV_F32", "split16") != "mfma32"
CIN_PAD = 32


class _ResBlock:
    def __init__(self, name, cin, cout):
        self.name, self.cin, self.cout = name, cin, cout
        self.temb_off = None


class _Attn:
    def __init__(self, name, c):
        self.name, self.c = name, c


class Model(_net.GraphedNet):
    def __init__(self, config, device=None, split16=None):
        self.config = config
        self.split16 = SPLIT16 if split16 is None else bool(split16)
        self.fused_attn = self.split16
        self.fused_attn_max_tokens = 64
        m = config.model
        self.ch, self.out_ch, self.ch_mult = m.ch, m.out_ch, tuple(m.ch_mult)
        self.num_res_blocks = m.num_res_blocks
        self.attn_resolutions = list(m.attn_resolutions)
        self.in_channels = m.in_channels
        self.resolution = config.data.image_size
        self.temb_ch = 4 * self.ch
        self.num_resolutions = len(self.ch_mult)
        if not m.resamp_with_conv:
            raise NotImplementedError("resamp_with_conv=False is not on the DDNM hot path")
        self.device = torch.device("cuda") if device is None else torch.device(device)
        self._plan()
        self.w = None
        self._reset_host_state()

    def _plan(self):
        ch, mult, nrb = self.ch, self.ch_mult, self.num_res_blocks
        in_mult = (1,) + mult
        res = self.resolution
        self.down = []
        self.res_blocks = []
        block_in = None
        chans = [ch]
        for lvl in range(self.num_resolutions):
            block_in = ch * in_mult[lvl]
            block_out = ch * mult[lvl]
            blocks, attns = [], []
            for ib in range(nrb):
                rb = _ResBlock(f"down.{lvl}.block.{ib}", block_in, block_out)
                rb.res = res
                blocks.append(rb)
                self.res_blocks.append(rb)
                block_in = block_out
                if res in self.attn_resolutions:
                    attns.append(_Attn(f"down.{lvl}.attn.{ib}", block_in))
                    attns[-1].res = res
                chans.append(block_in)
            has_down = lvl != self.num_resolutions - 1
            if has_down:
                res //= 2
                chans.append(block_in)
            self.down.append((blocks, attns, has_down, block_in))
        self.mid = [_ResBlock("mid.block_1", block_in, block_in), _Attn("mid.attn_1", block_in),
                    _ResBlock("mid.block_2", block_in, block_in)]
        for m in self.mid:
            m.res = res
        self.res_blocks += [self.mid[0], self.mid[2]]
        self.up = {}
        for lvl in reversed(range(self.num_resolutions)):
            block_out = ch * mult[lvl]
            blocks, attns = [], []
            for ib in range(nrb + 1):
                skip = chans.pop()
                rb = _ResBlock(f"up.{lvl}.block.{ib}", block_in + skip, block_out)
                rb.split = (block_in, skip)
                rb.res = res
                blocks.append(rb)
                self.res_blocks.append(rb)
                block_in = block_out
                if res in self.attn_resolutions:
                    attns.append(_Attn(f"up.{lvl}.attn.{ib}", block_in))
                    attns[-1].res = res
            has_up = lvl != 0
            if has_up:
                res *= 2
            self.up[lvl] = (blocks, attns, has_up, block_in)
        self.final_ch = block_in
        off = 0
        for rb in self.res_blocks:
            rb.temb_off = off
            off += rb.cout
        self.temb_total = off
        self.max_ch = max(rb.cin for rb in self.res_blocks)

    def state_dict_shapes(self):
        s = OrderedDict()

        def conv(n, co, ci, k):
            s[n + ".weight"], s[n + ".bias"] = (co, ci, k, k), (co,)

        def vec2(n, c):
            s[n + ".weight"], s[n + ".bias"] = (c,), (c,)

        def resblock(rb):
            n = rb.name
            vec2(n + ".norm1", rb.cin)
            conv(n + ".conv1", rb.cout, rb.cin, 3)
            s[n + ".temb_proj.weight"], s[n + ".temb_proj.bias"] = (rb.cout, self.temb_ch), (rb.cout,)
            vec2(n + ".norm2", rb.cout)
            conv(n + ".conv2", rb.cout, rb.cout, 3)
            if rb.cin != rb.cout:
                conv(n + ".nin_shortcut", rb.cout, rb.cin, 1)

        def attn(a):
            vec2(a.name + ".norm", a.c)
            for p in ("q", "k", "v", "proj_out"):
                conv(f"{a.name}.{p}", a.c, a.c, 1)

        s["temb.dense.0.weight"], s["temb.dense.0.bias"] = (self.temb_ch, self.ch), (self.temb_ch,)
        s["temb.dense.1.weight"], s["temb.dense.1.bias"] = (self.temb_ch, self.temb_ch), (self.temb_ch,)
        conv("conv_in", self.ch, self.in_channels, 3)
        for lvl, (blocks, attns, has_down, c) in enumerate(self.down):
            for rb in blocks:
                resblock(rb)
            for a in attns:
                attn(a)
            if has_down:
                conv(f"down.{lvl}.downsample.conv", c, c, 3)
        resblock(self.mid[0]), attn(self.mid[1]), resblock(self.mid[2])
        for lvl in range(self.num_resolutions):
            blocks, attns, has_up, c = self.up[lvl]
            for rb in blocks:
                resblock(rb)
            for a in attns:
                attn(a)
            if has_up:
                conv(f"up.{lvl}.upsample.conv", c, c, 3)
        vec2("norm_out", self.final_ch)
        conv("conv_out", self.out_ch, self.final_ch, 3)
        return s

    def random_state_dict(self, seed=1234):
        return _net.random_state_dict(self.state_dict_shapes(), seed)

    def load_state_dict(self, sd, strict=True):
        dev = self.device
        g = lambda k: sd[k].detach().to(device=dev, dtype=torch.float32).contiguous()
        w = {}

        def s16(t):
            sc = ops.s16_weight_scale(t)
            return (ops.pack_conv_weight_s16(t, sc), sc, None)
        for k in ("temb.dense.0", "temb.dense.1"):
            w[k + ".weight"], w[k + ".bias"] = g(k + ".weight"), g(k + ".bias")
        w["conv_in.weight"] = ops.pack_conv_weight(g("conv_in.weight"), cin_pad=CIN_PAD)
        w["conv_in.bias"] = g("conv_in.bias")
        if 9 * self.in_channels <= CIN_PAD:
            w["conv_in.weight.im2col"] = ops.pack_conv_in_weight_im2col(g("conv_in.weight"), CIN_PAD)
        tw, tb = [], []
        for rb in self.res_blocks:
            n = rb.name
            for norm in ("norm1", "norm2"):
                w[f"{n}.{norm}.weight"], w[f"{n}.{norm}.bias"] = g(f"{n}.{norm}.weight"), g(f"{n}.{norm}.bias")
            w[f"{n}.conv1.weight"] = ops.pack_conv_weight(g(f"{n}.conv1.weight"))
            w[f"{n}.conv2.weight"] = ops.pack_conv_weight(g(f"{n}.conv2.weight"))
            w[f"{n}.conv2.bias"] = g(f"{n}.conv2.bias")
            if self.split16:
                w1, w2 = g(f"{n}.conv1.weight"), g(f"{n}.conv2.weight")
                wsk = g(f"{n}.nin_shortcut.weight") if rb.cin != rb.cout else None
                s1 = ops.s16_weight_scale(w1)
                s2 = ops.s16_weight_scale(w2) if wsk is None else ops.s16_weight_scale(w2, wsk)
                w[f"{n}.conv1.s16"] = (ops.pack_conv_weight_s16(w1, s1), s1, None)
                w[f"{n}.conv2.s16"] = (ops.pack_conv_weight_s16(w2, s2), s2,
                                       None if wsk is None else ops.pack_conv_weight_s16(wsk, s2))
                if wsk is not None:
                    w[f"{n}.nin_shortcut.s16"] = s16(wsk)
            tw.append(g(f"{n}.temb_proj.weight"))
            tb.append(g(f"{n}.temb_proj.bias") + g(f"{n}.conv1.bias"))
            if rb.cin != rb.cout:
                w[f"{n}.nin_shortcut.weight"] = ops.pack_conv_weight(g(f"{n}.nin_shortcut.weight"))
                w[f"{n}.nin_shortcut.bias"] = g(f"{n}.nin_shortcut.bias")
                w[f"{n}.nin_shortcut.fused"] = ops.pack_skip_weight(g(f"{n}.nin_shortcut.weight"))
                w[f"{n}.conv2_plus_shortcut.bias"] = (g(f"{n}.conv2.bias") + g(f"{n}.nin_shortcut.bias")).contiguous()
        w["temb_proj_cat.weight"] = torch.cat(tw, 0).contiguous()
        w["temb_proj_cat.bias"] = torch.cat(tb, 0).contiguous()
        attns = [a for (_, at, _, _) in self.down for a in at] + [self.mid[1]] + \
                [a for lvl in self.up for a in self.up[lvl][1]]
        for a in attns:
            n = a.name
            w[f"{n}.norm.weight"], w[f"{n}.norm.bias"] = g(f"{n}.norm.weight"), g(f"{n}.norm.bias")
            wq = torch.cat([g(f"{n}.{p}.weight") for p in ("q", "k", "v")], 0)
            w[f"{n}.qkv.weight"] = ops.pack_conv_weight(wq)
            if self.split16:
                w[f"{n}.qkv.s16"] = s16(wq)
                w[f"{n}.proj_out.s16"] = s16(g(f"{n}.proj_out.weight"))
            w[f"{n}.qkv.bias"] = torch.cat([g(f"{n}.{p}.bias") for p in ("q", "k", "v")], 0).contiguous()
            gmax = math.sqrt(a.res * a.res * max(1, a.c // 32)) * float(sd[f"{n}.norm.weight"].detach().abs().max()) + \
                float(sd[f"{n}.norm.bias"].detach().abs().max())

            def _pow2(*names):
                bnd = max(float(sd[f"{n}.{p}.weight"].detach().float().abs().flatten(1).sum(1).max()) * gmax +
                          float(sd[f"{n}.{p}.bias"].detach().abs().max()) for p in names)
                return 2.0 ** (14 - math.ceil(math.log2(max(bnd, 1e-30))))
            w[f"{n}.attn_scales"] = (_pow2("q", "k"), _pow2("v"))
            w[f"{n}.proj_out.weight"] = ops.pack_conv_weight(g(f"{n}.proj_out.weight"))
            w[f"{n}.proj_out.bias"] = g(f"{n}.proj_out.bias")
        for lvl, (_, _, has_down, c) in enumerate(self.down):
            if has_down:
                w[f"down.{lvl}.downsample.conv.weight"] = ops.pack_conv_weight(g(f"down.{lvl}.downsample.conv.weight"))
                w[f"down.{lvl}.downsample.conv.bias"] = g(f"down.{lvl}.downsample.conv.bias")
                if self.split16:
                    w[f"down.{lvl}.downsample.conv.s16"] = s16(g(f"down.{lvl}.downsample.conv.weight"))
        for lvl, (_, _, has_up, c) in self.up.items():
            if has_up:
                w[f"up.{lvl}.upsample.conv.weight"] = ops.pack_conv_weight(g(f"up.{lvl}.upsample.conv.weight"))
                if self.split16:
                    wu = g(f"up.{lvl}.upsample.conv.weight")
                    su = ops.s16_weight_scale(wu)
                    w[f"up.{lvl}.upsample.conv.s16"] = (ops.pack_conv_weight_s16(wu, su), su, None)
                w[f"up.{lvl}.upsample.conv.bias"] = g(f"up.{lvl}.upsample.conv.bias")
        w["norm_out.weight"], w["norm_out.bias"] = g("norm_out.weight"), g("norm_out.bias")
        w["conv_out.weight"] = ops.pack_conv_weight(g("conv_out.weight"))
        w["conv_out.bias"] = g("conv_out.bias")
        if self.split16:
            self._guard_normalised_operands(sd, w)
        half = self.ch // 2
        freq = torch.exp(torch.arange(half, dtype=torch.float32) * -(math.log(10000) / (half - 1)))
        w["temb.freq"] = freq.to(dev)
        self.w = w
        self._reset_host_state()
        return self

    def _guard_normalised_operands(self, sd, w):
        groups = 32
        dropped = []

        def bound(norm, res, channels):
            g = sd[norm + ".weight"].detach().abs().max().item()
            b = sd[norm + ".bias"].detach().abs().max().item()
            return math.sqrt(res * res * max(1, channels // groups)) * g + b
        for rb in self.res_blocks:
            for norm, conv, ch in (("norm1", "conv1", rb.cin), ("norm2", "conv2", rb.cout)):
                if bound(f"{rb.name}.{norm}", rb.res, ch) >= 32768.0 and w.pop(f"{rb.name}.{conv}.s16", None) is not None:
                    dropped.append(f"{rb.name}.{conv}")
        attns = [a for (_, at, _, _) in self.down for a in at] + [self.mid[1]] + [a for lvl in self.up for a in self.up[lvl][1]]
        for a in attns:
            if bound(f"{a.name}.norm", a.res, a.c) >= 32768.0 and w.pop(f"{a.name}.qkv.s16", None) is not None:
                dropped.append(f"{a.name}.qkv")
        self.s16_dropped = dropped
        return dropped

    def _max_gn_partials(self):
        max_partial = 0
        res = self.resolution
        for _ in range(self.num_resolutions):
            for c in (self.ch, self.max_ch):
                max_partial = max(max_partial, ops.gn_nchunk(res * res, c))
            res //= 2
        return max_partial

    def _gn(self, x0, x1, name, want_amax=False):
        return ops.group_norm_affine(x0, x1, self.w[name + ".weight"], self.w[name + ".bias"], GN_EPS, self._ws,
                                     want_amax=want_amax)

    def _resblock(self, rb, x0, x1, tproj):
        w, n = self.w, rb.name
        x_amax = None
        if rb.cin != rb.cout and self.split16:
            *gn1, x_amax = self._gn(x0, x1, n + ".norm1", want_amax=True)
            gn1 = tuple(gn1)
        else:
            gn1 = self._gn(x0, x1, n + ".norm1")
        h = ops.conv2d(x0, w[n + ".conv1.weight"], rb.cout, 3, src1=x1, gn=gn1, gn_silu=True,
                       badd=tproj[:, rb.temb_off:], badd_stride=self.temb_total, emit_stats=True,
                       weight_s16=w.get(n + ".conv1.s16"))
        gn2 = self._gn(h, None, n + ".norm2")
        if rb.cin != rb.cout:
            B, H, W, _ = h.t.shape
            fuse = ops.conv_fuses_skip(B, H, W, rb.cout, rb.cout)
            if (fuse and self.split16 and not ops.conv_runs_s16(B, H, W, rb.cout, rb.cout)
                    and ops.conv_runs_s16_gather(B, H, W, rb.cout, rb.cout)):
                fuse = False
            if fuse:
                return ops.conv2d(h, w[n + ".conv2.weight"], rb.cout, 3, gn=gn2, gn_silu=True,
                                  bias=w[n + ".conv2_plus_shortcut.bias"], skip=(x0, x1),
                                  skip_weight=w[n + ".nin_shortcut.fused"], emit_stats=True,
                                  weight_s16=w.get(n + ".conv2.s16"), raw_amax=x_amax)
            xs = ops.conv2d(x0, w[n + ".nin_shortcut.weight"], rb.cout, 1, src1=x1, bias=w[n + ".nin_shortcut.bias"],
                            weight_s16=w.get(n + ".nin_shortcut.s16"), raw_amax=x_amax)
        else:
            assert x1 is None
            xs = x0
        s16 = w.get(n + ".conv2.s16")
        if s16 is not None:
            s16 = (s16[0], s16[1], None)
        return ops.conv2d(h, w[n + ".conv2.weight"], rb.cout, 3, gn=gn2, gn_silu=True, bias=w[n + ".conv2.bias"],
                          res=xs, emit_stats=True, weight_s16=s16)

    def _attn(self, a, x):
        w, n = self.w, a.name
        B, H, W, C = x.t.shape
        T = H * W
        gn = self._gn(x, None, n + ".norm")
        qkv = ops.conv2d(x, w[n + ".qkv.weight"], 3 * C, 1, gn=gn, gn_silu=False, bias=w[n + ".qkv.bias"],
                         weight_s16=w.get(n + ".qkv.s16"))
        sc = w.get(n + ".attn_scales")
        if sc is not None and self.fused_attn and T <= self.fused_attn_max_tokens and ops.attn_fused_supported(T, C):
            o = ops.attn_fused(qkv, B, T, C, sc[0], sc[1], float(int(C) ** (-0.5))).view(B, H, W, C)
            return ops.conv2d(o, w[n + ".proj_out.weight"], C, 1, bias=w[n + ".proj_out.bias"], res=x, emit_stats=True,
                              weight_s16=w.get(n + ".proj_out.s16"))
        S = torch.empty(B, T, T, dtype=torch.float32, device=qkv.device)
        q, k, v = qkv.view(-1)[0:], qkv.view(-1)[C:], qkv.view(-1)[2 * C:]
        ops.bgemm(q, k, S, T, T, C, lda=3 * C, ldb=3 * C, ldc=T, transb=True, batch=B,
                  sA=(T * 3 * C, 0), sB=(T * 3 * C, 0), sC=(T * T, 0))
        ops.softmax_rows_(S, B * T, T, T, float(int(C) ** (-0.5)))
        o = torch.empty(B, H, W, C, dtype=torch.float32, device=qkv.device)
        ops.bgemm(S, v, o, T, C, T, lda=T, ldb=3 * C, ldc=C, transb=False, batch=B,
                  sA=(T * T, 0), sB=(T * 3 * C, 0), sC=(T * C, 0))
        return ops.conv2d(o, w[n + ".proj_out.weight"], C, 1, bias=w[n + ".proj_out.bias"], res=x, emit_stats=True,
                          weight_s16=w.get(n + ".proj_out.s16"))

    @property
    def max_forward_batch(self):
        return ops.max_launch_batch(self.resolution * self.resolution * self.ch * 4)

    def _forward_eager(self, x, t, y=None):
        if self.w is None:
            raise RuntimeError("load_state_dict() must be called before forward()")
        assert x.shape[2] == x.shape[3] == self.resolution
        w = self.w
        B = x.shape[0]
        self._workspace(B)
        t = t.to(device=x.device, dtype=torch.float32).contiguous()
        emb = ops.timestep_embedding(t, w["temb.freq"], order=0)
        temb = ops.linear(emb, w["temb.dense.0.weight"], w["temb.dense.0.bias"])
        temb = ops.linear(temb, w["temb.dense.1.weight"], w["temb.dense.1.bias"], silu_in=True)
        tproj = ops.linear(temb, w["temb_proj_cat.weight"], w["temb_proj_cat.bias"], silu_in=True)

        if "conv_in.weight.im2col" in w:
            xin = ops.nchw_im2col3x3_pad(x.contiguous(), CIN_PAD)
            hs = [ops.conv2d(xin, w["conv_in.weight.im2col"], self.ch, 1, bias=w["conv_in.bias"], emit_stats=True)]
        else:
            xin = ops.nchw_to_nhwc_pad(x.contiguous(), CIN_PAD)
            hs = [ops.conv2d(xin, w["conv_in.weight"], self.ch, 3, bias=w["conv_in.bias"], emit_stats=True)]
        for lvl, (blocks, attns, has_down, c) in enumerate(self.down):
            for ib, rb in enumerate(blocks):
                h = self._resblock(rb, hs[-1], None, tproj)
                if attns:
                    h = self._attn(attns[ib], h)
                hs.append(h)
            if has_down:
                n = f"down.{lvl}.downsample.conv"
                src = hs[-1]
                hs.append(ops.conv2d(src, w[n + ".weight"], c, 3, bias=w[n + ".bias"], stride=2, pad=0,
                                     out_hw=(src.t.shape[1] // 2, src.t.shape[2] // 2), emit_stats=True,
                                     weight_s16=w.get(n + ".s16")))
        h = hs[-1]
        h = self._resblock(self.mid[0], h, None, tproj)
        h = self._attn(self.mid[1], h)
        h = self._resblock(self.mid[2], h, None, tproj)
        for lvl in reversed(range(self.num_resolutions)):
            blocks, attns, has_up, c = self.up[lvl]
            for ib, rb in enumerate(blocks):
                h = self._resblock(rb, h, hs.pop(), tproj)
                if attns:
                    h = self._attn(attns[ib], h)
            if has_up:
                n = f"up.{lvl}.upsample.conv"
                h = ops.conv2d(h, w[n + ".weight"], c, 3, bias=w[n + ".bias"], ups=True, emit_stats=True,
                               weight_s16=w.get(n + ".s16"))
        gn = self._gn(h, None, "norm_out")
        return ops.conv2d(h, w["conv_out.weight"], self.out_ch, 3, gn=gn, gn_silu=True, bias=w["conv_out.bias"],
                          out_nchw=True)

    def __call__(self, x, t):
        return self.forward(x, t)
```

ddnm_amd/ops.py:

```python
import ctypes

import numpy as np
import torch

from . import _lib
from ._lib import Conv16Desc, ConvDesc, GemmDesc, StepScalars, check


def _p(t):
    return None if t is None else t.data_ptr()


def _stream():
    return torch.cuda.current_stream().cuda_stream


def _f32c(t, name):
    if t.dtype != torch.float32 or not t.is_contiguous() or not t.is_cuda:
        raise ValueError(f"{name}: expected a contiguous float32 device tensor, got {t.dtype} "
                         f"contiguous={t.is_contiguous()} device={t.device}")
    return t


class KernelTimer:

    def __init__(self):
        self.records = []
        self.shapes = []

    def summary(self):
        torch.cuda.synchronize()
        out = {}
        for variant, flops, e0, e1 in self.records:
            r = out.setdefault(variant, {"launches": 0, "flops": 0.0, "ms": 0.0})
            r["launches"] += 1
            r["flops"] += flops
            r["ms"] += e0.elapsed_time(e1)
        return out


_timer = None


def set_kernel_timer(t):
    global _timer
    _timer = t


def _launch(fn, d, label, record):
    if _timer is None:
        check(fn(ctypes.byref(d), _stream()), label)
        return
    variant, flops, shape = record()
    e0, e1 = torch.cuda.Event(enable_timing=True), torch.cuda.Event(enable_timing=True)
    e0.record()
    check(fn(ctypes.byref(d), _stream()), label)
    e1.record()
    _timer.records.append((variant, flops, e0, e1))
    _timer.shapes.append(shape)


def max_launch_batch(per_image_bytes, margin=2):
    return max(1, (1 << 31) // int(per_image_bytes) // margin)


CONV_COUT_ALIGN = 128


_conv_ws = {}


def _conv_workspace(device, floats):
    key = (device, _stream())
    ws = _conv_ws.get(key)
    if ws is None or ws.numel() < floats:
        ws = torch.empty(int(floats), dtype=torch.float32, device=device)
        _conv_ws[key] = ws
    return ws


def pack_conv_weight(w, cin_pad=None):
    cout, cin, kh, kw = w.shape
    cin_pad = cin if cin_pad is None else cin_pad
    cout_pad = (cout + CONV_COUT_ALIGN - 1) // CONV_COUT_ALIGN * CONV_COUT_ALIGN
    out = torch.zeros(cout_pad, kh * kw, cin_pad, dtype=torch.float32, device=w.device)
    out[:cout, :, :cin] = w.float().permute(0, 2, 3, 1).reshape(cout, kh * kw, cin)
    return out.contiguous()


import os as _os
_NO_FUSED_GN = False
FORCE_ONE_TILE = False


class Act:
    __slots__ = ("t", "stats", "tiles", "gn")

    def __init__(self, t, stats=None, tiles=0, gn=None):
        self.t, self.stats, self.tiles = t, stats, tiles
        self.gn = gn


def tensor_of(x):
    return x.t if isinstance(x, Act) else x


def _shape_desc(B, H, W, cin, cout, ksize=3, stride=1):
    d = ConvDesc()
    d.B, d.Hin, d.Win, d.C0, d.C1, d.Cout = B, H, W, cin, 0, cout
    d.ksize, d.stride, d.pad, d.Ho, d.Wo = ksize, stride, (ksize // 2 if stride == 1 else 0), H // stride, W // stride
    return d


def conv_fuses_skip(B, H, W, cin, cout):
    return _lib.lib().ddnm_conv2d_f32_fuses_skip(ctypes.byref(_shape_desc(B, H, W, cin, cout))) == 1


def pack_skip_weight(w, f16=False):
    p = pack_conv_weight(w).reshape(-1, w.shape[1]).contiguous()
    return p.to(torch.float16) if f16 else p


def pack_conv_weight_f16(w, cin_pad=None):
    return pack_conv_weight(w, cin_pad=cin_pad).to(torch.float16).contiguous()


def s16_weight_scale(*ws):
    import math
    m = max(float(w.abs().max()) for w in ws)
    if not (m > 0.0) or not math.isfinite(m):
        return 1.0
    return 2.0 ** (13 - math.floor(math.log2(m)))


def pack_conv_weight_s16(w, scale):
    p = pack_conv_weight(w) * float(scale)
    cp, taps, cin = p.shape
    if cin % 32:
        raise ValueError("split packing needs Cin % 32 == 0")
    hi = p.to(torch.float16)
    lo = (p - hi.float()).to(torch.float16)
    hi, lo = hi.view(cp, taps, cin // 32, 1, 32), lo.view(cp, taps, cin // 32, 1, 32)
    return torch.cat([hi, lo], 3).contiguous()


def conv_runs_s16(B, H, W, cin, cout, ups=False):
    return _lib.lib().ddnm_conv3x3_s16_supported(ctypes.byref(_shape_desc(B, H, W, cin, cout))) == 1


def conv_runs_s16_gather(B, H, W, cin, cout, ksize=3, stride=1):
    if _NO_S16_GATHER:
        return False
    return _lib.lib().ddnm_conv_gather_s16_supported(ctypes.byref(_shape_desc(B, H, W, cin, cout, ksize, stride))) == 1


_S16_ACT_SCALE = None
_NO_S16_GATHER = False


def _s16_act_scale():
    global _S16_ACT_SCALE
    if _S16_ACT_SCALE is None:
        _S16_ACT_SCALE = float(_lib.lib().ddnm_conv3x3_s16_act_scale())
    return _S16_ACT_SCALE


def conv_runs_f16(B, H, W, cin, cout, ksize=3):
    L = _lib.lib()
    d = _shape_desc(B, H, W, cin, cout, ksize)
    return (L.ddnm_conv3x3_f16_supported if ksize == 3 else L.ddnm_conv1x1_f16_supported)(ctypes.byref(d)) == 1


_F16_PREPASS_MIN_COUT = 256
_f16_scratch_buf = {}


def _f16_scratch(device, numel, slot=0):
    key = (device, slot, _stream())
    buf = _f16_scratch_buf.get(key)
    if buf is None or buf.numel() < numel:
        buf = torch.empty(numel, dtype=torch.float16, device=device)
        _f16_scratch_buf[key] = buf
    return buf


AMAX_N = 32
_S16_CHECK = False


def amax_bound(a0, a1=None):
    def src(a):
        if a is None:
            return None, 0, 0
        if isinstance(a, Act) and a.stats is not None:
            B = a.t.shape[0]
            return a.stats, a.stats.numel() // B, 1
        t = tensor_of(a)
        return _f32c(t, "amax source"), t.numel() // t.shape[0], 0
    t0 = tensor_of(a0)
    B = t0.shape[0]
    p0, n0, k0 = src(a0)
    p1, n1, k1 = src(a1)
    out = torch.empty(B * AMAX_N, dtype=torch.float32, device=t0.device)
    check(_lib.lib().ddnm_amax_bound_f32(_p(p0), n0, k0, _p(p1), n1, k1, _p(out), B, _stream()), "ddnm_amax_bound_f32")
    return out


def conv2d(src0, weight, cout, ksize, *, src1=None, bias=None, badd=None, badd_stride=0, res=None, res_ups=False,
           gn=None, gn_silu=True, stride=1, pad=None, ups=False, out=None, out_nchw=False, out_hw=None, tile=0,
           emit_stats=False, weight_f16=None, skip=None, skip_weight=None, skip_weight_f16=None, weight_s16=None,
           raw_amax=None, one_tile=False):
    a_src0, a_src1 = src0, src1
    src0, src1, res = tensor_of(src0), tensor_of(src1), tensor_of(res)
    B, Hs, Ws, C0 = src0.shape
    C1 = 0 if src1 is None else src1.shape[3]
    Hin, Win = (2 * Hs, 2 * Ws) if ups else (Hs, Ws)
    if pad is None:
        pad = ksize // 2
    if out_hw is None:
        Ho, Wo = (Hin // stride, Win // stride)
    else:
        Ho, Wo = out_hw
    if out is None:
        shape = (B, cout, Ho, Wo) if out_nchw else (B, Ho, Wo, cout)
        out = torch.empty(shape, dtype=torch.float32, device=src0.device)
    d = ConvDesc()
    d.src0, d.src1, d.weight = _p(_f32c(src0, "src0")), _p(src1), _p(_f32c(weight, "weight"))
    d.bias, d.badd, d.res = _p(bias), _p(badd), _p(res)
    d.gn_scale, d.gn_shift = (None, None) if gn is None else (_p(gn[0]), _p(gn[1]))
    d.out = _p(out)
    d.B, d.Hin, d.Win, d.C0, d.C1, d.Cout = B, Hin, Win, C0, C1, cout
    d.ksize, d.stride, d.pad, d.Ho, d.Wo = ksize, stride, pad, Ho, Wo
    d.ups, d.gn_silu, d.out_nchw = int(ups), int(gn_silu), int(out_nchw)
    d.badd_stride, d.tile, d.res_ups = badd_stride, tile, int(res_ups)
    d.flags = 1 if (one_tile or FORCE_ONE_TILE) else 0
    L = _lib.lib()
    if out_nchw and cout <= 4 and skip is None and weight_f16 is None and L.ddnm_conv3x3_small_cout_f32_supported(ctypes.byref(d)) == 1:
        _launch(L.ddnm_conv3x3_small_cout_f32, d, "ddnm_conv3x3_small_cout_f32",
                lambda: ("conv3x3_small_cout_f32", 2.0 * B * Ho * Wo * cout * 9 * C0,
                         (B, Ho, Wo, C0, cout, 3, 1, 0, 0, gn is not None, False)))
        return Act(out, None, 0) if emit_stats else out
    f16, f16_1x1 = False, False
    if skip is not None:
        s0, s1 = tensor_of(skip[0]), tensor_of(skip[1])
        d.skip0, d.skip1 = _p(s0), _p(s1)
        d.SC0, d.SC1 = s0.shape[3], (0 if s1 is None else s1.shape[3])
    s16 = (weight_s16 is not None and weight_f16 is None and ksize == 3 and stride == 1
           and (skip is None or (weight_s16[2] is not None and gn is not None and d.SC0 % 32 == 0 and d.SC1 % 32 == 0))
           and L.ddnm_conv3x3_s16_supported(ctypes.byref(d)) == 1)
    s16g = (not s16 and weight_s16 is not None and weight_f16 is None and skip is None and not _NO_S16_GATHER
            and L.ddnm_conv_gather_s16_supported(ctypes.byref(d)) == 1)
    if s16 or s16g:
        d.weight = weight_s16[0].data_ptr()
        d.acc_scale = 1.0 / (float(weight_s16[1]) * _s16_act_scale())
        if gn is None or skip is not None:
            if raw_amax is None:
                raw_amax = amax_bound(*skip) if skip is not None else amax_bound(a_src0, a_src1)
            d.amax_in = raw_amax.data_ptr()
    if weight_f16 is not None:
        if ksize == 3:
            f16 = L.ddnm_conv3x3_f16_supported(ctypes.byref(d)) == 1
            if (not f16 and stride == 1 and not ups and skip is None and not out_nchw and not res_ups
                    and Hs * Ws < 256 and (C0 | C1) % 8 == 0):
                d.ksize, d.pad, d.C0, d.C1, d.gn_scale, d.gn_shift = 1, 0, 9 * (C0 + C1), 0, None, None
                if L.ddnm_conv1x1_f16_supported(ctypes.byref(d)) == 1:
                    col = _f16_scratch(src0.device, B * Hs * Ws * 9 * (C0 + C1), slot=1)
                    check(L.ddnm_im2col3x3_f16(_p(src0), _p(src1), None if gn is None else _p(gn[0]),
                                               None if gn is None else _p(gn[1]), col.data_ptr(), B, Hs, Ws, C0, C1,
                                               int(gn_silu), _stream()), "ddnm_im2col3x3_f16")
                    d.src0, d.src1, d.src_f16 = col.data_ptr(), None, 1
                    f16 = f16_1x1 = True
                    gn = None
                else:
                    d.ksize, d.pad, d.C0, d.C1 = 3, pad, C0, C1
                    d.gn_scale, d.gn_shift = (None, None) if gn is None else (_p(gn[0]), _p(gn[1]))
        elif ksize == 1 and skip is None:
            d.gn_scale, d.gn_shift = None, None
            f16 = f16_1x1 = L.ddnm_conv1x1_f16_supported(ctypes.byref(d)) == 1
            if not f16 and gn is not None:
                d.gn_scale, d.gn_shift = _p(gn[0]), _p(gn[1])
    if f16:
        d.weight = weight_f16.data_ptr()
        if gn is not None and (f16_1x1 or cout >= _F16_PREPASS_MIN_COUT):
            h16 = _f16_scratch(src0.device, B * Hs * Ws * (C0 + C1))
            check(L.ddnm_gn_apply_f16(_p(src0), _p(src1), _p(gn[0]), _p(gn[1]), h16.data_ptr(), B, Hs * Ws, C0, C1,
                                      int(gn_silu), _stream()), "ddnm_gn_apply_f16")
            d.src0, d.src1, d.C0, d.C1 = h16.data_ptr(), None, C0 + C1, 0
            d.gn_scale, d.gn_shift, d.src_f16 = None, None, 1
    if skip is not None:
        d.skip_weight = _p(skip_weight_f16) if f16 else (weight_s16[2].data_ptr() if s16 else _p(skip_weight))
        if f16 and skip_weight_f16 is None:
            raise ValueError("fp16 launch with a fused shortcut needs skip_weight_f16")
    if f16_1x1:
        fn_run, fn_tiles, fn_ws = L.ddnm_conv1x1_f16_f32, L.ddnm_conv1x1_f16_stats_tiles, L.ddnm_conv1x1_f16_workspace_floats
    elif f16:
        fn_run, fn_tiles, fn_ws = L.ddnm_conv3x3_f16_f32, L.ddnm_conv3x3_f16_stats_tiles, L.ddnm_conv3x3_f16_workspace_floats
    elif s16:
        fn_run, fn_tiles, fn_ws = L.ddnm_conv3x3_s16_f32, L.ddnm_conv3x3_s16_stats_tiles, L.ddnm_conv3x3_s16_workspace_floats
    elif s16g:
        fn_run, fn_tiles, fn_ws = (L.ddnm_conv_gather_s16_f32, L.ddnm_conv_gather_s16_stats_tiles,
                                   L.ddnm_conv_gather_s16_workspace_floats)
    else:
        fn_run, fn_tiles, fn_ws = L.ddnm_conv2d_f32, L.ddnm_conv2d_f32_stats_tiles, L.ddnm_conv2d_f32_workspace_floats
    stats, tiles = None, 0
    if emit_stats and not _NO_FUSED_GN:
        tiles = fn_tiles(ctypes.byref(d))
        if tiles > 0:
            stats = torch.empty(B * tiles * cout * 2, dtype=torch.float32, device=src0.device)
            d.stats_out = stats.data_ptr()
    need = fn_ws(ctypes.byref(d))
    if need > 0:
        ws = _conv_workspace(src0.device, need)
        d.workspace, d.workspace_floats = ws.data_ptr(), ws.numel()

    def record():
        if f16_1x1:
            variant = "conv1x1_f16<256x128>"
        elif f16:
            variant = "conv3x3_halo_f16<256x128>"
        elif s16:
            variant = "conv3x3_s16_persist<256x128>" if L.ddnm_conv3x3_s16_persistent(ctypes.byref(d)) == 1 else "conv3x3_halo_s16<256x128>"
        elif s16g:
            variant = "conv_gather_s16"
        else:
            tn = L.ddnm_conv2d_f32_tile_n(ctypes.byref(d))
            kind = "conv3x3_halo_f32" if (ksize == 3 and stride == 1) else "conv_gather_f32"
            variant = kind + {128: "<128x128>", 64: "<64x64>", 32: "<128x32>"}[tn]
        flops = 2.0 * B * Ho * Wo * cout * (ksize * ksize * (C0 + C1) + d.SC0 + d.SC1)
        return variant, flops, (B, Ho, Wo, C0 + C1, cout, ksize, stride, int(ups), d.SC0 + d.SC1, gn is not None,
                                res is not None)
    _launch(fn_run, d, "ddnm_conv2d", record)
    if _S16_CHECK and (s16 or s16g) and not bool(torch.isfinite(out).all()):
        raise FloatingPointError(f"split-fp16 launch produced non-finite values (B={B}, {Hin}x{Win}, Cin={C0 + C1}, "
                                 f"Cout={cout}, k={ksize}): an operand left fp16 range; DDNM_CONV_F32=mfma32 selects the "
                                 "all-fp32 engine")
    if emit_stats:
        return Act(out, stats, tiles)
    return out


CONV16_COUT_ALIGN = 256


def _f16c(t, name):
    if t.dtype != torch.float16 or not t.is_contiguous() or not t.is_cuda:
        raise ValueError(f"{name}: expected a contiguous float16 device tensor, got {t.dtype} "
                         f"contiguous={t.is_contiguous()} device={t.device}")
    return t


def pack_conv_weight16(w, cin_pad=None):
    if w.dim() == 2:
        w = w[:, :, None, None]
    cout, cin, kh, kw = w.shape
    cin_pad = cin if cin_pad is None else cin_pad
    cout_pad = (cout + CONV16_COUT_ALIGN - 1) // CONV16_COUT_ALIGN * CONV16_COUT_ALIGN
    out = torch.zeros(cout_pad, kh * kw, cin_pad, dtype=torch.float16, device=w.device)
    out[:cout, :, :cin] = w.float().permute(0, 2, 3, 1).reshape(cout, kh * kw, cin).to(torch.float16)
    return out.contiguous()


def _conv16_desc(src, weight, cout, ksize, H, W, ups, skip, skip_weight, bias, res, res_ups, src1=None, gn=None,
                 gn_silu=True):
    B = src.shape[0]
    d = Conv16Desc()
    d.src, d.weight, d.bias, d.res = _p(_f16c(src, "src")), _p(_f16c(weight, "weight")), _p(bias), _p(res)
    cin = src.shape[-1]
    if src1 is not None:
        d.src1, d.C0 = _p(_f16c(src1, "src1")), cin
        cin += src1.shape[-1]
    if gn is not None:
        d.gn_scale, d.gn_shift, d.gn_silu = _p(gn[0]), _p(gn[1]), int(gn_silu)
    d.B, d.H, d.W, d.Cin, d.Cout, d.ksize = B, H, W, cin, cout, ksize
    d.ups, d.res_ups = int(ups), int(res_ups)
    if skip is not None:
        s0, s1 = skip
        d.skip0, d.skip1, d.skip_weight = _p(_f16c(s0, "skip0")), _p(s1), _p(_f16c(skip_weight, "skip_weight"))
        d.SC0, d.SC1 = s0.shape[-1], (0 if s1 is None else s1.shape[-1])
    return d


def conv16_supported(B, H, W, cin, cout, ksize, ups=False):
    d = Conv16Desc()
    d.B, d.H, d.W, d.Cin, d.Cout, d.ksize, d.ups = B, H, W, cin, cout, ksize, int(ups)
    return _lib.lib().ddnm_conv16_supported(ctypes.byref(d)) == 1


def conv16(src, weight, cout, ksize, *, src1=None, gn=None, gn_silu=True, bias=None, res=None, res_ups=False, ups=False,
           skip=None, skip_weight=None, emit_stats=True, out=None, fin=None):
    src, src1, res = tensor_of(src), tensor_of(src1), tensor_of(res)
    B, Hs, Ws, _ = src.shape
    H, W = (2 * Hs, 2 * Ws) if ups else (Hs, Ws)
    if skip is not None:
        skip = tuple(tensor_of(s) for s in skip)
    d = _conv16_desc(src, weight, cout, ksize, H, W, ups, skip, skip_weight, bias, res, res_ups, src1, gn, gn_silu)
    L = _lib.lib()
    if out is None:
        out = torch.empty(B, H, W, cout, dtype=torch.float16, device=src.device)
    d.out = _p(_f16c(out, "out"))
    fused_fin = False
    if fin is not None and emit_stats:
        name, gamma, beta, film, film_stride, eps, ws = fin
        d.fin_gamma, d.fin_beta, d.fin_film = _p(gamma), _p(beta), _p(film)
        d.fin_scale, d.fin_shift = _p(ws.scale), _p(ws.shift)
        d.fin_eps, d.fin_film_stride, d.fin_groups = eps, film_stride, 32
        fused_fin = ws.scale.numel() >= B * cout and L.ddnm_conv16_fuses_fin(ctypes.byref(d)) == 1
        if not fused_fin:
            d.fin_gamma = None
        else:
            ws.generation += 1
    stats, tiles = None, 0
    if emit_stats:
        tiles = L.ddnm_conv16_stats_tiles(ctypes.byref(d))
        if tiles < 0:
            check(tiles, "ddnm_conv16_stats_tiles")
        if tiles > 0:
            stats = torch.empty(B * tiles * cout * 2, dtype=torch.float32, device=src.device)
            d.stats_out = stats.data_ptr()
    need = L.ddnm_conv16_workspace_floats(ctypes.byref(d))
    if need < 0:
        check(int(need), "ddnm_conv16_workspace_floats")
    if need > 0:
        ws = _conv_workspace(src.device, need)
        d.workspace, d.workspace_floats = ws.data_ptr(), ws.numel()
    _launch(L.ddnm_conv16, d, "ddnm_conv16",
            lambda: (f"conv16<{ksize}x{ksize}>", 2.0 * B * H * W * cout * (ksize * ksize * d.Cin + d.SC0 + d.SC1),
                     (B, H, W, d.Cin, cout, ksize, 1, int(ups), d.SC0 + d.SC1, False, res is not None)))
    return Act(out, stats, tiles, gn=(fin[6].scale, fin[6].shift, fin[0], fin[6], fin[6].generation) if fused_fin else None)


def conv16_out(src, weight, cout, bias=None, gn=None, gn_silu=True):
    src = tensor_of(src)
    B, H, W, _ = src.shape
    d = _conv16_desc(src, weight, cout, 3, H, W, False, None, None, bias, None, False, None, gn, gn_silu)
    d.out_nchw_f32 = 1
    out = torch.empty(B, cout, H, W, dtype=torch.float32, device=src.device)
    d.out = out.data_ptr()
    _launch(_lib.lib().ddnm_conv16, d, "ddnm_conv16(out)",
            lambda: ("conv16<out>", 2.0 * B * H * W * cout * 9 * d.Cin, (B, H, W, d.Cin, cout, 3, 1, 0, 0, False, False)))
    return out


def gn_apply16(src0, src1, gn, silu, pool=False):
    src0, src1 = tensor_of(src0), tensor_of(src1)
    B, H, W, C0 = src0.shape
    C1 = 0 if src1 is None else src1.shape[3]
    Ho, Wo = (H // 2, W // 2) if pool else (H, W)
    out = torch.empty(B, Ho, Wo, C0 + C1, dtype=torch.float16, device=src0.device)
    sc, sh = (None, None) if gn is None else gn
    check(_lib.lib().ddnm_gn_apply_h16(_p(_f16c(src0, "src0")), _p(src1), _p(sc), _p(sh), _p(out), B, H, W, C0, C1,
                                       int(silu), int(pool), _stream()), "ddnm_gn_apply_h16")
    return out


def im2col16(src0, src1, gn, silu):
    src0, src1 = tensor_of(src0), tensor_of(src1)
    B, H, W, C0 = src0.shape
    C1 = 0 if src1 is None else src1.shape[3]
    out = torch.empty(B, H, W, 9 * (C0 + C1), dtype=torch.float16, device=src0.device)
    sc, sh = (None, None) if gn is None else gn
    check(_lib.lib().ddnm_im2col3x3_h16(_p(_f16c(src0, "src0")), _p(src1), _p(sc), _p(sh), _p(out), B, H, W, C0, C1,
                                        int(silu), _stream()), "ddnm_im2col3x3_h16")
    return out


def nchw_to_nhwc16(x, cpad):
    B, C, H, W = x.shape
    out = torch.empty(B, H, W, cpad, dtype=torch.float16, device=x.device)
    check(_lib.lib().ddnm_nchw_to_nhwc_h16(_p(_f32c(x, "x")), _p(out), B, C, H * W, cpad, _stream()),
          "ddnm_nchw_to_nhwc_h16")
    return out


def gn_stats16(t):
    B, H, W, C = t.shape
    hw = H * W
    tiles = 1
    for cand in (64, 32, 16, 8, 4, 2):
        if hw % cand == 0 and hw // cand >= 4:
            tiles = cand
            break
    stats = torch.empty(B * tiles * C * 2, dtype=torch.float32, device=t.device)
    check(_lib.lib().ddnm_gn_stats_h16(_p(_f16c(t, "t")), _p(stats), B, hw, C, tiles, _stream()), "ddnm_gn_stats_h16")
    return Act(t, stats, tiles)


def attn16(qkv, C, lse=None):
    B, H, W, C3 = qkv.shape
    assert C3 == 3 * C
    out = torch.empty(B, H, W, C, dtype=torch.float16, device=qkv.device)
    if lse is None:
        check(_lib.lib().ddnm_attn16_d64(_p(_f16c(qkv, "qkv")), _p(out), B, H * W, C, _stream()), "ddnm_attn16_d64")
    else:
        if lse.dtype != torch.float32 or lse.numel() != B * (C // 64) * H * W or not lse.is_contiguous():
            raise ValueError("attn16: lse must be a contiguous float32 tensor [B, C/64, H*W]")
        check(_lib.lib().ddnm_attn16_d64_lse(_p(_f16c(qkv, "qkv")), _p(out), _p(lse), B, H * W, C, _stream()),
              "ddnm_attn16_d64_lse")
    return out


def attn16_bwd(qkv, o, dO, lse):
    B, H, W, C3 = qkv.shape
    C = C3 // 3
    dqkv = torch.empty_like(qkv)
    dsum = torch.empty_like(lse)
    check(_lib.lib().ddnm_attn16_d64_bwd(_p(_f16c(qkv, "qkv")), _p(_f16c(o, "o")), _p(_f16c(dO, "dO")), _p(lse), _p(dsum),
                                         _p(dqkv), B, H * W, C, _stream()), "ddnm_attn16_d64_bwd")
    return dqkv


class GroupNormWorkspace:

    def __init__(self, device, max_batch, max_channels, max_partial_doubles):
        self.partial = torch.empty(max_partial_doubles, dtype=torch.float64, device=device)
        self.scale = torch.empty(max_batch * max_channels, dtype=torch.float32, device=device)
        self.shift = torch.empty(max_batch * max_channels, dtype=torch.float32, device=device)
        self.generation = 0


def gn_nchunk(hw, c):
    n = _lib.lib().ddnm_gn_nchunk(hw, c)
    if n <= 0:
        check(n, "ddnm_gn_nchunk")
    return n


def group_norm_affine(src0, src1, gamma, beta, eps, ws, groups=32, film=None, film_stride=0, keep=None, want_amax=False):
    a0 = src0 if isinstance(src0, Act) else Act(src0)
    a1 = None if src1 is None else (src1 if isinstance(src1, Act) else Act(src1))
    if a0.t.dtype == torch.float16:
        if a0.stats is None:
            a0 = gn_stats16(a0.t)
        if a1 is not None and a1.stats is None:
            a1 = gn_stats16(a1.t)
    src0, src1 = a0.t, (None if a1 is None else a1.t)
    B, H, W, C0 = src0.shape
    C1 = 0 if src1 is None else src1.shape[3]
    C, HW = C0 + C1, H * W
    sc_buf, sh_buf, mr = ws.scale, ws.shift, None
    if keep is None:
        ws.generation += 1
    if keep is not None:
        sc_buf = torch.empty(B * C, dtype=torch.float32, device=src0.device)
        sh_buf = torch.empty(B * C, dtype=torch.float32, device=src0.device)
        mr = torch.empty(B * groups * 2, dtype=torch.float32, device=src0.device)
        keep.update(scale=sc_buf, shift=sh_buf, mean_rstd=mr, groups=groups)
    if a0.stats is not None and (a1 is None or a1.stats is not None):
        if sc_buf.numel() < B * C:
            raise ValueError("GroupNorm workspace too small")
        amax = None
        if want_amax and groups == AMAX_N:
            amax = torch.empty(B * AMAX_N, dtype=torch.float32, device=src0.device)
        check(_lib.lib().ddnm_gn_finalize_tiles_amax_f32(_p(a0.stats), a0.tiles, C0, None if a1 is None else _p(a1.stats),
                                                         0 if a1 is None else a1.tiles, C1, _p(gamma), _p(beta), B, HW,
                                                         groups, eps, _p(sc_buf), _p(sh_buf), _p(film), film_stride,
                                                         _p(mr), _p(amax), _stream()), "ddnm_gn_finalize_tiles_amax_f32")
        if want_amax:
            return sc_buf, sh_buf, (amax if amax is not None else amax_bound(a0, a1))
        return sc_buf, sh_buf
    nchunk = gn_nchunk(HW, C)
    need = B * nchunk * groups * 2
    if ws.partial.numel() < need or sc_buf.numel() < B * C:
        raise ValueError("GroupNorm workspace too small")
    L = _lib.lib()
    check(L.ddnm_gn_stats_f32(_p(src0), _p(src1), B, HW, C0, C1, groups, _p(ws.partial), nchunk, _stream()),
          "ddnm_gn_stats_f32")
    check(L.ddnm_gn_finalize_f32(_p(ws.partial), nchunk, _p(gamma), _p(beta), B, HW, C, groups, eps, _p(sc_buf),
                                 _p(sh_buf), _p(film), film_stride, _p(mr), _stream()), "ddnm_gn_finalize_f32")
    if want_amax:
        return sc_buf, sh_buf, amax_bound(a0, a1)
    return sc_buf, sh_buf


def bgemm(A, Bm, C, M, N, K, *, lda, ldb, ldc, transb, batch=1, inner=1, sA=(0, 0), sB=(0, 0), sC=(0, 0),
          D=None, ldd=0, sD=(0, 0), alpha=1.0, beta=0.0, transa=False):
    d = GemmDesc()
    d.A, d.Bm, d.D, d.C = _p(A), _p(Bm), _p(D), _p(C)
    d.M, d.N, d.K, d.lda, d.ldb, d.ldc, d.ldd = M, N, K, lda, ldb, ldc, ldd
    d.transb, d.batch, d.inner = int(transb), batch, inner
    d.sAo, d.sAi, d.sBo, d.sBi, d.sCo, d.sCi, d.sDo, d.sDi = sA[0], sA[1], sB[0], sB[1], sC[0], sC[1], sD[0], sD[1]
    d.alpha, d.beta, d.transa = alpha, beta, int(transa)
    _launch(_lib.lib().ddnm_bgemm_f32, d, "ddnm_bgemm_f32",
            lambda: ("bgemm_f32", 2.0 * M * N * K * batch, (batch, M, N, K, 0, 1, 1, 0, 0, False, False)))
    return C


def attn_fused_supported(T, C):
    return _lib.lib().ddnm_attn_fused_supported(int(T), int(C)) == 1


def attn_fused(qkv, B, T, C, s_qk, s_v, scale, out=None):
    if out is None:
        out = torch.empty(B, T, C, dtype=torch.float32, device=qkv.device)
    check(_lib.lib().ddnm_attn_fused_f32(_p(_f32c(qkv, "qkv")), _p(out), B, T, C, float(s_qk), float(s_v), float(scale), _stream()),
          "ddnm_attn_fused_f32")
    return out


def softmax_rows_(x, rows, n, ld, scale):
    check(_lib.lib().ddnm_softmax_rows_f32(_p(x), rows, n, ld, scale, _stream()), "ddnm_softmax_rows_f32")
    return x


def linear(x, W, bias, silu_in=False, out=None):
    B, K = x.shape
    N = W.shape[0]
    if out is None:
        out = torch.empty(B, N, dtype=torch.float32, device=x.device)
    check(_lib.lib().ddnm_linear_f32(_p(x), _p(W), _p(bias), _p(out), B, K, N, int(silu_in), _stream()),
          "ddnm_linear_f32")
    return out


def timestep_embedding(t, freq, order):
    B, half = t.shape[0], freq.shape[0]
    emb = torch.empty(B, 2 * half, dtype=torch.float32, device=t.device)
    check(_lib.lib().ddnm_timestep_embedding_f32(_p(t), _p(freq), _p(emb), B, half, order, _stream()),
          "ddnm_timestep_embedding_f32")
    return emb


def avgpool2_nhwc(x, gn=None, silu=False):
    B, H, W, C = x.shape
    out = torch.empty(B, H // 2, W // 2, C, dtype=torch.float32, device=x.device)
    sc, sh = (None, None) if gn is None else gn
    check(_lib.lib().ddnm_avgpool2_nhwc_f32(_p(_f32c(x, "x")), _p(sc), _p(sh), int(silu), _p(out), B, H // 2, W // 2, C,
                                            _stream()), "ddnm_avgpool2_nhwc_f32")
    return out


def embedding_add_(emb, table, idx):
# ... 240 lines not shown
```

include/ddnm_hip.h:

```cpp
#ifndef DDNM_HIP_H
#define DDNM_HIP_H

#include <stdint.h>

#ifdef __cplusplus
extern "C" {
#endif

#define DDNM_E_BADARG (-1)
#define DDNM_E_SHAPE (-2)

int ddnm_version(void);
const char* ddnm_build_digest(void);
int ddnm_sizeof(int which);
const char* ddnm_error_string(int code);

typedef struct ddnm_conv_desc {
    const float* src0;
    const float* src1;
    const float* weight;
    const float* bias;
    const float* badd;
    const float* res;
    const float* gn_scale;
    const float* gn_shift;
    float* out;
    int32_t B, Hin, Win;
    int32_t C0, C1;
    int32_t Cout;
    int32_t ksize;
    int32_t stride;
    int32_t pad;
    int32_t Ho, Wo;
    int32_t ups;
    int32_t gn_silu;
    int32_t out_nchw;
    int32_t badd_stride;
    int32_t tile;
    float* workspace;
    int64_t workspace_floats;
    int32_t res_ups;
    int32_t src_f16;
    float* stats_out;
    const float* skip0;
    const float* skip1;
    const float* skip_weight;
    int32_t SC0, SC1;
    float acc_scale;
    int32_t flags;
    const float* amax_in;
} ddnm_conv_desc;

#define DDNM_CONV_ONE_TILE 1
#define DDNM_AMAX_N 32

int ddnm_conv2d_f32(const ddnm_conv_desc* d, void* stream);
int ddnm_conv2d_f32_tile_n(const ddnm_conv_desc* d);
int64_t ddnm_conv2d_f32_workspace_floats(const ddnm_conv_desc* d);
int ddnm_conv2d_f32_stats_tiles(const ddnm_conv_desc* d);
int ddnm_conv2d_f32_fuses_skip(const ddnm_conv_desc* d);

int ddnm_conv3x3_small_cout_f32(const ddnm_conv_desc* d, void* stream);
int ddnm_conv3x3_small_cout_f32_supported(const ddnm_conv_desc* d);

int ddnm_conv3x3_f16_f32(const ddnm_conv_desc* d, void* stream);
int ddnm_conv3x3_f16_supported(const ddnm_conv_desc* d);
int64_t ddnm_conv3x3_f16_workspace_floats(const ddnm_conv_desc* d);
int ddnm_conv3x3_f16_stats_tiles(const ddnm_conv_desc* d);

int ddnm_conv3x3_s16_f32(const ddnm_conv_desc* d, void* stream);
int ddnm_conv3x3_s16_supported(const ddnm_conv_desc* d);
int ddnm_conv3x3_s16_persistent(const ddnm_conv_desc* d);
int64_t ddnm_conv3x3_s16_workspace_floats(const ddnm_conv_desc* d);
int ddnm_conv3x3_s16_stats_tiles(const ddnm_conv_desc* d);
float ddnm_conv3x3_s16_act_scale(void);

int ddnm_conv_gather_s16_f32(const ddnm_conv_desc* d, void* stream);
int ddnm_conv_gather_s16_supported(const ddnm_conv_desc* d);
int64_t ddnm_conv_gather_s16_workspace_floats(const ddnm_conv_desc* d);
int ddnm_conv_gather_s16_stats_tiles(const ddnm_conv_desc* d);

int ddnm_conv1x1_f16_f32(const ddnm_conv_desc* d, void* stream);
int ddnm_conv1x1_f16_supported(const ddnm_conv_desc* d);
int64_t ddnm_conv1x1_f16_workspace_floats(const ddnm_conv_desc* d);
int ddnm_conv1x1_f16_stats_tiles(const ddnm_conv_desc* d);

typedef struct ddnm_conv16_desc {
    const void* src;
    const void* weight;
    const float* bias;
    const void* res;
    const void* skip0;
    const void* skip1;
    const void* skip_weight;
    void* out;
    float* stats_out;
    float* workspace;
    int64_t workspace_floats;
    int32_t B, H, W;
    int32_t Cin, Cout;
    int32_t ksize;
    int32_t ups, res_ups;
    int32_t SC0, SC1;
    const void* src1;
    const float* gn_scale;
    const float* gn_shift;
    int32_t C0;
    int32_t gn_silu;
    int32_t out_nchw_f32;
    int32_t reserved;
    const float* fin_gamma;
    const float* fin_beta;
    const float* fin_film;
    float* fin_scale;
    float* fin_shift;
    float fin_eps;
    int32_t fin_film_stride;
    int32_t fin_groups;
    int32_t reserved2;
} ddnm_conv16_desc;

int ddnm_conv16(const ddnm_conv16_desc* d, void* stream);
int ddnm_conv16_fuses_fin(const ddnm_conv16_desc* d);
int ddnm_conv16_supported(const ddnm_conv16_desc* d);
int64_t ddnm_conv16_workspace_floats(const ddnm_conv16_desc* d);
int ddnm_conv16_stats_tiles(const ddnm_conv16_desc* d);

int ddnm_gn_apply_h16(const void* src0, const void* src1, const float* scale, const float* shift, void* out, int32_t B,
                      int32_t H, int32_t W, int32_t C0, int32_t C1, int32_t silu, int32_t pool, void* stream);
int ddnm_im2col3x3_h16(const void* src0, const void* src1, const float* scale, const float* shift, void* out, int32_t B,
                       int32_t H, int32_t W, int32_t C0, int32_t C1, int32_t silu, void* stream);
int ddnm_nchw_to_nhwc_h16(const float* x, void* out, int32_t B, int32_t C, int32_t HW, int32_t cpad, void* stream);
int ddnm_gn_stats_h16(const void* src, float* stats, int32_t B, int32_t HW, int32_t C, int32_t tiles, void* stream);

int ddnm_attn16_d64(const void* qkv, void* out, int32_t B, int32_t T, int32_t C, void* stream);
int ddnm_attn16_d64_lse(const void* qkv, void* out, float* lse, int32_t B, int32_t T, int32_t C, void* stream);
int ddnm_attn16_d64_bwd(const void* qkv, const void* o, const void* dO, const float* lse, float* dsum, void* dqkv,
                        int32_t B, int32_t T, int32_t C, void* stream);

int ddnm_gn_stats_f32(const float* src0, const float* src1, int32_t B, int32_t HW, int32_t C0, int32_t C1,
                      int32_t groups, double* partial , int32_t nchunk, void* stream);
int ddnm_gn_nchunk(int32_t HW, int32_t C);
int ddnm_gn_finalize_f32(const double* partial, int32_t nchunk, const float* gamma, const float* beta,
                         int32_t B, int32_t HW, int32_t C, int32_t groups, float eps,
                         float* scale , float* shift ,
                         const float* film ,
                         int32_t film_stride, float* mean_rstd ,
                         void* stream);

int ddnm_gn_apply_f16(const float* src0, const float* src1, const float* scale, const float* shift, void* out_f16,
                      int32_t B, int32_t HW, int32_t C0, int32_t C1, int32_t silu, void* stream);
int ddnm_im2col3x3_f16(const float* src0, const float* src1, const float* scale, const float* shift, void* out_f16,
                       int32_t B, int32_t H, int32_t W, int32_t C0, int32_t C1, int32_t silu, void* stream);
int ddnm_gn_finalize_tiles_f32(const float* part0, int32_t tiles_per_img0, int32_t C0, const float* part1,
                               int32_t tiles_per_img1, int32_t C1, const float* gamma, const float* beta, int32_t B,
                               int32_t HW, int32_t groups, float eps, float* scale, float* shift, const float* film,
                               int32_t film_stride, float* mean_rstd, void* stream);
int ddnm_gn_finalize_tiles_amax_f32(const float* part0, int32_t tiles_per_img0, int32_t C0, const float* part1,
                                    int32_t tiles_per_img1, int32_t C1, const float* gamma, const float* beta, int32_t B,
                                    int32_t HW, int32_t groups, float eps, float* scale, float* shift, const float* film,
                                    int32_t film_stride, float* mean_rstd, float* amax_out, void* stream);
int ddnm_amax_bound_f32(const float* src0, int64_t per_image0, int32_t kind0, const float* src1, int64_t per_image1,
                        int32_t kind1, float* out, int32_t B, void* stream);

typedef struct ddnm_gemm_desc {
    const float* A; const float* Bm; const float* D; float* C;
    int32_t M, N, K;
    int32_t lda, ldb, ldc, ldd;
    int32_t transb;
    int32_t batch, inner;
    int64_t sAo, sAi, sBo, sBi, sCo, sCi, sDo, sDi;
    float alpha, beta;
    int32_t transa;
    int32_t reserved;
} ddnm_gemm_desc;
int ddnm_bgemm_f32(const ddnm_gemm_desc* d, void* stream);

int ddnm_gn_bwd_f32(const float* x, const float* dA, int32_t dA_ups, const float* gn_scale, const float* gn_shift,
                    const float* mean_rstd, int32_t silu, const float* add, int32_t add_ups, int32_t B, int32_t H,
                    int32_t W, int32_t C, int32_t groups, double* partial , int32_t nchunk,
                    float* coef , float* dx, void* stream);
int ddnm_gn_bwd_nchunk(int32_t HW, int32_t C);
int ddnm_gn_bwd_h16(const void* x, const void* dA, int32_t dA_ups, const float* gn_scale, const float* gn_shift,
                    const float* mean_rstd, int32_t silu, const void* add, int32_t add_ups, int32_t B, int32_t H,
                    int32_t W, int32_t C, int32_t groups, double* partial , int32_t nchunk,
                    float* coef , void* dx, void* stream);
int ddnm_softmax_bwd_rows_f32(const float* P, float* dP, int64_t rows, int32_t n, int32_t ld, float scale, void* stream);
int ddnm_pool_tokens_f32(const float* h, const float* gn_scale, const float* gn_shift, const float* pos ,
                         float* X , int32_t B, int32_t HW, int32_t C, void* stream);
int ddnm_pool_attn_fwd_f32(const float* qkv , float* P , float* a0 ,
                           int32_t B, int32_t T, int32_t C, int32_t heads, void* stream);
int ddnm_pool_attn_bwd_f32(const float* qkv, const float* P, const float* da0, float* dqkv, int32_t B, int32_t T,
                           int32_t C, int32_t heads, void* stream);
int ddnm_pool_tokens_bwd_f32(const float* dX, float* dact , int32_t B, int32_t HW, int32_t C, void* stream);
int ddnm_logsoftmax_grad_f32(const float* logits, const int64_t* y, float* dlogits, int32_t B, int32_t N, void* stream);
int ddnm_pool_tokens_h16(const void* h, const float* gn_scale, const float* gn_shift, const float* pos ,
                         float* X , int32_t B, int32_t HW, int32_t C, void* stream);
int ddnm_pool_tokens_bwd_h16(const float* dX, void* dact , int32_t B, int32_t HW, int32_t C, void* stream);

int ddnm_attn_fused_f32(const float* qkv, float* out, int32_t B, int32_t T, int32_t C, float s_qk, float s_v,
                        float softmax_scale, void* stream);
int ddnm_attn_fused_supported(int32_t T, int32_t C);

int ddnm_softmax_rows_f32(float* x, int64_t rows, int32_t n, int32_t ld, float scale, void* stream);

int ddnm_linear_f32(const float* x, const float* W, const float* bias, float* y, int32_t B, int32_t K,
                    int32_t N, int32_t silu_in, void* stream);
int ddnm_timestep_embedding_f32(const float* t, const float* freq, float* emb, int32_t B, int32_t half,
                                int32_t order, void* stream);

int ddnm_avgpool2_nhwc_f32(const float* in, const float* gn_scale, const float* gn_shift, int32_t silu, float* out,
                           int32_t B, int32_t Ho, int32_t Wo, int32_t C, void* stream);
int ddnm_embedding_add_f32(float* emb, const float* table, const int64_t* idx, int32_t B, int32_t D, int32_t rows,
                           void* stream);

int ddnm_nchw_to_nhwc_pad_f32(const float* src, float* dst, int32_t B, int32_t C, int32_t HW, int32_t Cpad,
                              void* stream);
int ddnm_nchw_im2col3x3_pad_f32(const float* src, float* dst, int32_t B, int32_t C, int32_t H, int32_t W, int32_t Cpad,
                                void* stream);

typedef struct ddnm_step_scalars {
    float sqrt_1m_at;
    float sqrt_at;
    float sqrt_at_next;
    float c1, c2;
    float lambda;
    uint32_t rng_on;
    uint32_t rng_seed_lo, rng_seed_hi;
    uint32_t rng_iter;
    uint32_t rng_image_base;
    uint32_t reserved_rng;
} ddnm_step_scalars;


int ddnm_randn_philox_f32(float* out, int32_t B, int64_t chw, uint32_t seed_lo, uint32_t seed_hi, uint32_t iter,
                          uint32_t image_base, void* stream);

int ddnm_randn_philox_keyed_f32(float* out, int32_t B, int64_t n, const uint32_t* rng_keys, uint32_t iter,
                                void* stream);
int ddnm_step_combine_keyed_f32(const float* x0, const float* proj, const float* apy, const uint32_t* rng_keys,
                                const float* et, int64_t et_bstride, float* xt_next, int32_t B, int64_t chw,
                                const ddnm_step_scalars* s, void* stream);
int ddnm_step_sr_avgpool_keyed_f32(const float* xt, const float* et, int64_t et_bstride, const uint32_t* rng_keys,
                                   const float* y, float* x0, float* xt_next, int32_t B, int32_t H, int32_t W,
                                   int32_t r, const ddnm_step_scalars* s, void* stream);
int ddnm_step_color_keyed_f32(const float* xt, const float* et, int64_t et_bstride, const uint32_t* rng_keys,
                              const float* y, float* x0, float* xt_next, int32_t B, int32_t HW,
                              const float* w3_host, const ddnm_step_scalars* s, void* stream);
int ddnm_step_inpaint_keyed_f32(const float* xt, const float* et, int64_t et_bstride, const uint32_t* rng_keys,
                                const float* y, const int32_t* rank, int32_t n_kept, float* x0, float* xt_next,
                                int32_t B, int32_t HW, const ddnm_step_scalars* s, void* stream);
int ddnm_step_denoise_keyed_f32(const float* xt, const float* et, int64_t et_bstride, const uint32_t* rng_keys,
                                const float* y, float* x0, float* xt_next, int32_t B, int64_t chw,
                                const ddnm_step_scalars* s, void* stream);

int ddnm_step_x0_f32(const float* xt, const float* et, int64_t et_bstride, float* x0, int32_t B, int64_t chw,
                     const ddnm_step_scalars* s, void* stream);
int ddnm_step_combine_f32(const float* x0, const float* proj, const float* apy, const float* noise,
                          const float* et, int64_t et_bstride, float* xt_next, int32_t B, int64_t chw,
                          const ddnm_step_scalars* s, void* stream);
int ddnm_step_sr_avgpool_f32(const float* xt, const float* et, int64_t et_bstride, const float* noise,
                             const float* y , float* x0, float* xt_next, int32_t B,
                             int32_t H, int32_t W, int32_t r, const ddnm_step_scalars* s, void* stream);
int ddnm_step_color_f32(const float* xt, const float* et, int64_t et_bstride, const float* noise,
                        const float* y , float* x0, float* xt_next, int32_t B, int32_t HW,
                        const float* w3_host, const ddnm_step_scalars* s, void* stream);
int ddnm_step_inpaint_f32(const float* xt, const float* et, int64_t et_bstride, const float* noise,
                          const float* y ,
                          const int32_t* rank ,
                          int32_t n_kept, float* x0, float* xt_next, int32_t B, int32_t HW,
                          const ddnm_step_scalars* s, void* stream);
int ddnm_step_denoise_f32(const float* xt, const float* et, int64_t et_bstride, const float* noise,
                          const float* y, float* x0, float* xt_next, int32_t B, int64_t chw,
                          const ddnm_step_scalars* s, void* stream);
int ddnm_step_inpaint_pi_f32(const float* xt, const float* et, int64_t et_bstride, const float* noise, const float* y,
                             int64_t y_stride, const int32_t* rank, int32_t n_kept_max, float* x0, float* xt_next,
                             int32_t B, int32_t HW, const ddnm_step_scalars* s, void* stream);
int ddnm_step_inpaint_pi_keyed_f32(const float* xt, const float* et, int64_t et_bstride, const uint32_t* rng_keys,
                                   const float* y, int64_t y_stride, const int32_t* rank, int32_t n_kept_max, float* x0,
                                   float* xt_next, int32_t B, int32_t HW, const ddnm_step_scalars* s, void* stream);
int ddnm_renoise_f32(const float* x0, const float* noise, float* xt_next, int64_t n, float a, float b, void* stream);

int ddnm_axpby_f32(const float* x, const float* y, float* out, int64_t n, float a, float b, void* stream);
int ddnm_axpby_strided_f32(const float* x, int64_t x_bstride, const float* y, float* out, int32_t B, int64_t chw,
                           float a, float b, void* stream);
int ddnm_fill_f32(float* out, int64_t n, float value, void* stream);
int ddnm_mask_mix_f32(const float* x, const float* y, const float* mask, int32_t planes_mask, int64_t plane_elems,
                      float* out, int64_t total, float cx_m, float cx_n, float cy_m, float cy_n, void* stream);
int ddnm_gather_scale_f32(const float* in, const int32_t* idx, const float* scale, float* out, int32_t B, int64_t n_in,
                          int64_t n_out, void* stream);
int ddnm_site_matmul_f32(const float* in, const float* M, float* out, int32_t B, int64_t sites, int32_t n, int64_t sb,
                         int64_t ss, int64_t sj, int32_t trans, void* stream);
int ddnm_site_spectral_f32(const float* x, const float* y, const float* V, int32_t n, int32_t mode, int32_t r,
                           int32_t B, int32_t C, int32_t H, int32_t W, float* out, int32_t op, float c0, float c1,
                           float c2, float c3, void* stream);

int ddnm_mul_planes_f32(const float* x, const float* table, int32_t planes_table, int64_t plane_elems, float* out,
                        int64_t total, void* stream);

int ddnm_spectral_mix_f32(const float* x, const float* y, const float* singulars, int64_t plane_elems, float* out,
                          int64_t total, float a, float sigma_y, float sigma_t, float eta, int32_t mode, void* stream);

int ddnm_step_plus_spectral_f32(const float* xt_hat, const float* et_hat, const float* y_hat, const float* gains,
                                int64_t gains_cstride, const float* noise, float* out_hat, int32_t B, int32_t C,
                                int64_t plane, float sigma_y, float sigma_t, float eta, const ddnm_step_scalars* s,
                                void* stream);
int ddnm_step_plus_spectral_keyed_f32(const float* xt_hat, const float* et_hat, const float* y_hat, const float* gains,
                                      int64_t gains_cstride, const uint32_t* rng_keys, float* out_hat, int32_t B,
                                      int32_t C, int64_t plane, float sigma_y, float sigma_t, float eta,
                                      const ddnm_step_scalars* s, void* stream);

int ddnm_op_avgpool_f32(const float* x, float* y, int32_t BC, int32_t H, int32_t W, int32_t r, void* stream);
int ddnm_op_upsample_f32(const float* y, float* x, int32_t BC, int32_t H, int32_t W, int32_t r, void* stream);
int ddnm_op_color_A_f32(const float* x, float* y, int32_t B, int32_t HW, const float* w3_host, void* stream);
int ddnm_op_color_pinv_f32(const float* y, float* x, int32_t B, int32_t HW, const float* w3_host, void* stream);
int ddnm_op_inpaint_A_f32(const float* x, const int32_t* rank, int32_t n_kept, float* y, int32_t B, int32_t HW,
                          void* stream);
int ddnm_op_inpaint_pinv_f32(const float* y, const int32_t* rank, int32_t n_kept, float* x, int32_t B,
                             int32_t HW, void* stream);
int ddnm_op_inpaint_A_pi_f32(const float* x, const int32_t* rank, int32_t n_kept_max, float* y, int64_t y_stride,
                             int32_t B, int32_t HW, void* stream);
int ddnm_op_inpaint_pinv_pi_f32(const float* y, int64_t y_stride, const int32_t* rank, int32_t n_kept_max, float* x,
                                int32_t B, int32_t HW, void* stream);
int ddnm_fwht2d_f32(const float* in, float* out, int32_t planes, int32_t n, void* stream);
int ddnm_fwht2d_masked_f32(const float* in, const float* mask, int32_t planes_mask, float* out,
                           int32_t planes, int32_t n, float* scratch , void* stream);
int ddnm_wh_gather_f32(const float* planes, const int32_t* perm, float* y, int32_t B, int32_t C, int32_t N,
                       int32_t n_keep, void* stream);
int ddnm_wh_scatter_f32(const float* y, const int32_t* perm, float* planes, int32_t B, int32_t C, int32_t N,
                        int32_t n_keep, void* stream);

int ddnm_patchify_f32(const float* src, float* dst, int32_t planes, int32_t D, int32_t ps, int32_t inverse, void* stream);

int ddnm_step_plus_cs_pre_f32(const float* xt, const float* et, int64_t et_bstride, const float* noise, const float* aty,
                              float* x0_out, float* xt_next, float* w, int32_t B, int32_t C, int32_t D, int32_t ps,
                              float a_lambda, float d1n, float d2n, float dd1, float dd2, const ddnm_step_scalars* s,
                              void* stream);
int ddnm_step_plus_cs_pre_keyed_f32(const float* xt, const float* et, int64_t et_bstride, const uint32_t* rng_keys,
                                    const float* aty, float* x0_out, float* xt_next, float* w, int32_t B, int32_t C,
                                    int32_t D, int32_t ps, float a_lambda, float d1n, float d2n, float dd1, float dd2,
                                    const ddnm_step_scalars* s, void* stream);
int ddnm_step_plus_cs_post_f32(const float* P, float* xt_next, int32_t planes, int32_t D, int32_t ps, void* stream);

int ddnm_hq_x0_f32(const float* xt, const float* eps, int64_t eps_bstride, float* x0, int32_t B, int64_t chw,
                   float c_recip, float c_recipm1, int32_t clip, void* stream);
int ddnm_hq_project_f32(const float* x0, const float* apy, const float* apax0, float* x0_hat, int64_t n, float lam,
                        void* stream);
int ddnm_copy_rect_f32(const float* src, int32_t Hs, int32_t Ws, int32_t sy, int32_t sx, float* dst, int32_t Hd, int32_t Wd,
                       int32_t dy, int32_t dx, int32_t planes, int32_t h, int32_t w, void* stream);
int ddnm_hq_sample_f32(const float* x0_hat, const float* xt, const float* grad, const float* noise, float* out, int64_t n,
                       float coef1, float coef2, float gamma, float noise_scale, void* stream);

int ddnm_finalize_psnr_f32(const float* x, const float* x_orig, float* img , double* sse ,
                           int32_t B, int64_t chw, void* stream);

int64_t ddnm_ssim_workspace_elems(int32_t B, int32_t C, int32_t H, int32_t W);
int ddnm_ssim_f32(const float* x, const float* y, double* ssim , double* work, int64_t work_elems, int32_t B,
                  int32_t C, int32_t H, int32_t W, int32_t transform, void* stream);

#ifdef __cplusplus
}
#endif
#endif
```

Measured before the change: 6.122 images/sec.

## Replace nearest-upsample 3x3 convs with sub-pixel 2x2 phase convolutions

Nearest-neighbour upsampling followed by a 3x3 conv is rewritten as four 2x2 phase convolutions on the low-resolution input. Phase weights are precomputed in fp64 and packed as split fp16 hi/lo pairs, and a new persistent MFMA kernel writes the interleaved high-resolution output and GroupNorm stats directly. This cuts the upsample-conv FLOPs to 16/36 and avoids reading the upsampled input. The cost is a new kernel path with its own tiling and a changed rounding order from folding the weight sums. It is enabled by default, gated on a minimum tile count, and also includes a small fix to a buffer-resource bound.

Result: faster. 6.308 images/sec, median of 6 (+3.0%).

```diff
diff --git a/ddnm_amd/_lib.py b/ddnm_amd/_lib.py
--- a/ddnm_amd/_lib.py
+++ b/ddnm_amd/_lib.py
@@ -108,6 +108,7 @@
     "ddnm_conv3x3_s16_f32": (c_int32, [POINTER(ConvDesc), c_void_p]),
     "ddnm_conv3x3_s16_supported": (c_int32, [POINTER(ConvDesc)]),
     "ddnm_conv3x3_s16_persistent": (c_int32, [POINTER(ConvDesc)]),
+    "ddnm_conv3x3_s16_ups_subpixel_supported": (c_int32, [POINTER(ConvDesc)]),
     "ddnm_conv3x3_s16_workspace_floats": (c_int64, [POINTER(ConvDesc)]),
     "ddnm_conv3x3_s16_stats_tiles": (c_int32, [POINTER(ConvDesc)]),
     "ddnm_conv3x3_s16_act_scale": (c_float, []),
diff --git a/ddnm_amd/build.py b/ddnm_amd/build.py
--- a/ddnm_amd/build.py
+++ b/ddnm_amd/build.py
@@ -9,7 +9,7 @@
 LIB = os.path.join(HERE, "libddnm_hip.so")
 STAMP = os.path.join(HERE, ".libddnm_hip.stamp")
 OBJ = os.path.join(HERE, "_obj")
-SOURCES = ["conv_igemm_f32.hip", "conv_igemm_f16.hip", "conv_s16_persist.hip", "conv_gather_s16.hip", "conv_small_f32.hip", "conv1x1_f16.hip", "conv16.hip", "act16.hip", "attn16.hip", "attn_d512.hip", "attn16_bwd.hip", "gemm_f32.hip", "groupnorm.hip", "misc.hip", "ddnm_step.hip", "fwht.hip", "backward.hip", "metrics.hip"]
+SOURCES = ["conv_igemm_f32.hip", "conv_igemm_f16.hip", "conv_s16_persist.hip", "conv_s16_subpixel.hip", "conv_gather_s16.hip", "conv_small_f32.hip", "conv1x1_f16.hip", "conv16.hip", "act16.hip", "attn16.hip", "attn_d512.hip", "attn16_bwd.hip", "gemm_f32.hip", "groupnorm.hip", "misc.hip", "ddnm_step.hip", "fwht.hip", "backward.hip", "metrics.hip"]
 FLAGS = ["--offload-arch=gfx950", "-O3", "-std=c++17", "-fPIC", "-shared", "-Wall", "-Wno-unused-function"]
 
 
diff --git a/ddnm_amd/csrc/conv_common.h b/ddnm_amd/csrc/conv_common.h
--- a/ddnm_amd/csrc/conv_common.h
+++ b/ddnm_amd/csrc/conv_common.h
@@ -25,6 +25,9 @@
 
 bool conv3x3_s16_persist_eligible(const ConvArgs& p);
 int conv3x3_s16_persist_launch(const ConvArgs& p, hipStream_t s);
+bool conv3x3_s16_ups_subpixel_ok(const ddnm_conv_desc* d);
+int conv3x3_s16_ups_subpixel_run(const ddnm_conv_desc* d, hipStream_t s);
+int conv_persist_grid_cus();
 
 struct TileMap {
     int img, ty0, tx0, th_unused, TW, TW_log2, flat_base, Wo;
diff --git a/ddnm_amd/csrc/conv_igemm_f16.hip b/ddnm_amd/csrc/conv_igemm_f16.hip
--- a/ddnm_amd/csrc/conv_igemm_f16.hip
+++ b/ddnm_amd/csrc/conv_igemm_f16.hip
@@ -424,13 +424,18 @@
 
 extern "C" int ddnm_conv3x3_f16_f32(const ddnm_conv_desc* d, void* stream) { return run_f16(d, stream, false); }
 
-extern "C" int ddnm_conv3x3_s16_f32(const ddnm_conv_desc* d, void* stream) { return run_f16(d, stream, true); }
+extern "C" int ddnm_conv3x3_s16_f32(const ddnm_conv_desc* d, void* stream) {
+    if (d && (d->flags & DDNM_CONV_UPS_SUBPIXEL)) return conv3x3_s16_ups_subpixel_run(d, (hipStream_t)stream);
+    return run_f16(d, stream, true);
+}
+
+extern "C" int ddnm_conv3x3_s16_ups_subpixel_supported(const ddnm_conv_desc* d) { return conv3x3_s16_ups_subpixel_ok(d) ? 1 : 0; }
 
 extern "C" float ddnm_conv3x3_s16_act_scale(void) { return DDNM_S16_ASCALE; }
 
 extern "C" int ddnm_conv3x3_s16_persistent(const ddnm_conv_desc* d) {
     PlanF16 pl;
-    if (!d || d->src_f16 || (d->flags & DDNM_CONV_ONE_TILE) || !plan_f16(d, &pl, KC16 / 2) || pl.ksplit != 1) return 0;
+    if (!d || (d->flags & DDNM_CONV_UPS_SUBPIXEL) || d->src_f16 || (d->flags & DDNM_CONV_ONE_TILE) || !plan_f16(d, &pl, KC16 / 2) || pl.ksplit != 1) return 0;
     ConvArgs p;
     p.d = *d;
     p.Cin = d->C0 + d->C1;
@@ -448,12 +453,14 @@
 
 extern "C" int64_t ddnm_conv3x3_s16_workspace_floats(const ddnm_conv_desc* d) {
     PlanF16 pl;
+    if (d && (d->flags & DDNM_CONV_UPS_SUBPIXEL)) return conv3x3_s16_ups_subpixel_ok(d) ? 0 : DDNM_E_SHAPE;
     if (!d || !plan_f16(d, &pl, KC16 / 2)) return DDNM_E_SHAPE;
     return pl.ksplit > 1 ? (int64_t)pl.ksplit * d->B * d->Ho * d->Wo * d->Cout : 0;
 }
 
 extern "C" int ddnm_conv3x3_s16_stats_tiles(const ddnm_conv_desc* d) {
     PlanF16 pl;
+    if (d && (d->flags & DDNM_CONV_UPS_SUBPIXEL)) return conv3x3_s16_ups_subpixel_ok(d) ? d->Ho * d->Wo / 256 : DDNM_E_SHAPE;
     if (!d || !plan_f16(d, &pl, KC16 / 2)) return DDNM_E_SHAPE;
     return pl.ksplit > 1 ? splitk_stats_tiles(d) : d->Ho * d->Wo / pl.BM;
 }
diff --git a/ddnm_amd/csrc/conv_s16_persist.hip b/ddnm_amd/csrc/conv_s16_persist.hip
--- a/ddnm_amd/csrc/conv_s16_persist.hip
+++ b/ddnm_amd/csrc/conv_s16_persist.hip
@@ -216,7 +216,8 @@
     const __amdgpu_buffer_rsrc_t r_bias = __builtin_amdgcn_make_buffer_rsrc(
         const_cast<void*>(reinterpret_cast<const void*>(d.bias)), 0, d.bias ? (unsigned)Cout * 4u : 0u, 0x00020000);
     const __amdgpu_buffer_rsrc_t r_badd = __builtin_amdgcn_make_buffer_rsrc(
-        const_cast<void*>(reinterpret_cast<const void*>(d.badd)), 0, d.badd ? (unsigned)d.B * d.badd_stride * 4u : 0u, 0x00020000);
+        const_cast<void*>(reinterpret_cast<const void*>(d.badd)), 0,
+        d.badd ? (unsigned)((d.B - 1) * d.badd_stride + Cout) * 4u : 0u, 0x00020000);
     const __amdgpu_buffer_rsrc_t r_stats = __builtin_amdgcn_make_buffer_rsrc(
         reinterpret_cast<void*>(d.stats_out), 0, d.stats_out ? (unsigned)p.m_tiles * Cout * 8u : 0u, 0x00020000);
     const unsigned o_lane = (unsigned)(((wm * MT * Wo + rsel) * Cout + wn * NT * 32 + ncol) * 4);
@@ -484,11 +485,8 @@
 }
 
 int conv3x3_s16_persist_launch(const ConvArgs& p, hipStream_t s) {
-    int dev = 0, cus = 0;
-    if (hipGetDevice(&dev) != hipSuccess || hipDeviceGetAttribute(&cus, hipDeviceAttributeMultiprocessorCount, dev) != hipSuccess || cus <= 0)
-        cus = 256;
+    const int cus = conv_persist_grid_cus();
     const int total = p.m_tiles * p.n_tiles;
-    cus -= cus % 8;
     const dim3 grid(total < cus ? total : cus);
     const bool asc = p.d.amax_in != nullptr, res = p.d.res != nullptr;
     if (p.d.skip0) { DDNM_LAUNCH((conv3x3_s16_persist_kernel<true, false, true>), grid, dim3(P_NTHREADS), 0, s, p, total); }
diff --git a/ddnm_amd/csrc/conv_s16_subpixel.hip b/ddnm_amd/csrc/conv_s16_subpixel.hip
--- /dev/null
+++ b/ddnm_amd/csrc/conv_s16_subpixel.hip
@@ -0,0 +1,417 @@
+#include <type_traits>
+
+#include "conv_common.h"
+
+typedef unsigned u32x4 __attribute__((ext_vector_type(4)));
+
+namespace {
+constexpr int Q_WM = 4, Q_WN = 2, Q_MT = 2, Q_NT = 2;
+constexpr int Q_NTHREADS = 512, Q_BN = 128;
+constexpr int Q_LDH = 72, Q_KCH = 32;
+constexpr int Q_MAXH = 340, Q_HWD = 34;
+constexpr int Q_HCOLS = 8, Q_HRPP = Q_NTHREADS / Q_HCOLS, Q_HR = (Q_MAXH + Q_HRPP - 1) / Q_HRPP;
+constexpr int Q_BR = Q_BN / (Q_NTHREADS / 8);
+constexpr int Q_NWB = 3, Q_WTILE = Q_BN * 128;
+constexpr int Q_HBYTES = 2 * Q_MAXH * Q_LDH * 2;
+constexpr int Q_NOUT = Q_MT * Q_NT * 16;
+constexpr int Q_STEPS = 4;
+enum { Q_MID = 0, Q_LAST = 1, Q_FIRST = 2 };
+
+constexpr int q_first_of(int s) { return s == 0 ? 0 : (s == 1 ? 22 : (s == 2 ? 43 : Q_NOUT)); }
+constexpr int q_extra(int kind, int s) {
+    return (s == 0 ? Q_HR : 0) + (kind == Q_FIRST ? q_first_of(s + 1) - q_first_of(s) + (s == 0 ? 1 : 0) : (kind == Q_LAST && s == 0 ? 3 : 0));
+}
+constexpr int q_wait(int kind, int s) { return Q_BR + (s >= 1 ? q_extra(kind, s - 1) : q_extra(kind, 3)); }
+static_assert(q_extra(Q_FIRST, 3) == 0 && q_extra(Q_MID, 3) == 0 && q_extra(Q_LAST, 3) == 0, "step 3 issues its weight tile only");
+static_assert(q_wait(Q_FIRST, 1) < 64 && q_wait(Q_FIRST, 2) < 64 && q_wait(Q_FIRST, 3) < 64 && q_wait(Q_LAST, 1) < 64, "vmcnt is a 6-bit field");
+
+template <int V>
+using ic = std::integral_constant<int, V>;
+}
+
+__global__ __launch_bounds__(Q_NTHREADS, 1) void conv2x2x4_s16_subpixel_kernel(const ConvArgs p, const int total) {
+    constexpr int WM = Q_WM, WN = Q_WN, MT = Q_MT, NT = Q_NT, BN = Q_BN, HR = Q_HR, LDH = Q_LDH, KCH = Q_KCH;
+    constexpr int MAXH = Q_MAXH, HWd = Q_HWD, NWB = Q_NWB, WTILE = Q_WTILE, BR = Q_BR, NTHREADS = Q_NTHREADS;
+    __shared__ __attribute__((aligned(1024))) char lds_all[NWB * WTILE + Q_HBYTES + WM * BN * 2 * 4];
+    char* const Bs = lds_all;
+    _Float16* const Hs = reinterpret_cast<_Float16*>(lds_all + NWB * WTILE);
+    float* const stat_lds = reinterpret_cast<float*>(lds_all + NWB * WTILE + Q_HBYTES);
+
+    const ddnm_conv_desc& d = p.d;
+    const int tid = threadIdx.x, lane = tid & 63;
+    const int wave = __builtin_amdgcn_readfirstlane(tid >> 6);
+    const int wm = wave / WN, wn = wave % WN;
+    const int G = gridDim.x;
+    const int per_img = (p.Hs * p.Ws) >> 8;
+    const int Cout = d.Cout, Wo = d.Wo, Ho = d.Ho;
+
+    int t_img, t_ty0, t_tx0, t_ntile, t_mtile;
+    auto tile_of = [&](int v) {
+        const int tile_id = xcd_swizzle(v, total);
+        t_ntile = tile_id % p.n_tiles;
+        t_mtile = tile_id / p.n_tiles;
+        t_img = t_mtile / per_img;
+        const int t = t_mtile - t_img * per_img;
+        const int ty = t / p.tiles_x;
+        t_ty0 = ty * 8;
+        t_tx0 = (t - ty * p.tiles_x) * 32;
+    };
+
+    const int hc = tid % Q_HCOLS, prow = tid / Q_HCOLS;
+    auto halo_src = [&](int i) {
+        const int row = prow + Q_HRPP * i;
+        const int hy = row / HWd, hx = row - hy * HWd;
+        const int iy = t_ty0 - 1 + hy, ix = t_tx0 - 1 + hx;
+        const bool ok = row < MAXH && (unsigned)iy < (unsigned)p.Hs && (unsigned)ix < (unsigned)p.Ws;
+        return ok ? (t_img * p.Hs + iy) * p.Ws + ix : -1;
+    };
+
+    const int lrow = lane >> 3, lpiece = lane & 7;
+    const int wswz = (((wave & 1) << 2) | (lrow >> 1));
+    const unsigned w_rowlen = (unsigned)Q_STEPS * (unsigned)p.Cin * 4u;
+    const __amdgpu_buffer_rsrc_t r_w = __builtin_amdgcn_make_buffer_rsrc(
+        const_cast<void*>(reinterpret_cast<const void*>(d.weight)), 0, (unsigned)p.n_tiles * BN * w_rowlen, 0x00020000);
+    const unsigned w_lane = (unsigned)(wave * 8 + lrow) * w_rowlen + (unsigned)((lpiece ^ wswz) * 16);
+    unsigned w_soff = 0;
+    auto issue_w = [&](int chunk, int step, int buf) {
+        char* dst = Bs + buf * WTILE + wave * 1024;
+        const unsigned so = w_soff + ((unsigned)step * p.Cin + (unsigned)chunk * KCH) * 4u;
+#pragma unroll
+        for (int j = 0; j < BR; ++j)
+            __builtin_amdgcn_raw_ptr_buffer_load_lds(r_w, (__attribute__((address_space(3))) void*)(dst + j * (NTHREADS / 64) * 1024), 16,
+                                                     w_lane, so + (unsigned)j * (NTHREADS / 8) * w_rowlen, 0, 0);
+    };
+
+    const int nchunks = p.Cin / KCH;
+    uint4 h_st[HR];
+    constexpr unsigned HOOB = 0x80000000u;
+    const __amdgpu_buffer_rsrc_t r_s0 = __builtin_amdgcn_make_buffer_rsrc(
+        const_cast<void*>(reinterpret_cast<const void*>(d.src0)), 0, (unsigned)d.B * p.Hs * p.Ws * d.C0 * 4, 0x00020000);
+    const __amdgpu_buffer_rsrc_t r_s1 = __builtin_amdgcn_make_buffer_rsrc(
+        const_cast<void*>(reinterpret_cast<const void*>(d.C1 > 0 ? d.src1 : d.src0)), 0,
+        (unsigned)d.B * p.Hs * p.Ws * (d.C1 > 0 ? d.C1 : d.C0) * 4, 0x00020000);
+    const __amdgpu_buffer_rsrc_t r_amax = __builtin_amdgcn_make_buffer_rsrc(
+        const_cast<void*>(reinterpret_cast<const void*>(d.amax_in)), 0, (unsigned)d.B * DDNM_AMAX_N * 4u, 0x00020000);
+    auto amax_request = [&](int img, bool live) {
+        return __builtin_amdgcn_raw_buffer_load_b32(r_amax, (lane < DDNM_AMAX_N && live) ? (unsigned)lane * 4u : HOOB, (unsigned)img * DDNM_AMAX_N * 4u, 0);
+    };
+    auto amax_scales = [&](unsigned m, float& scale, float& inv_scale) {
+#pragma unroll
+        for (int o = 32; o >= 1; o >>= 1) {
+            const unsigned t = (unsigned)__shfl_xor((int)m, o);
+            m = t > m ? t : m;
+        }
+        m = __builtin_amdgcn_readfirstlane(m);
+        int e = (int)((m >> 23) & 0xffu);
+        e = e < 47 ? 47 : (e > 207 ? 207 : e);
+        const int k = 14 - (e - 127);
+        scale = __uint_as_float((unsigned)(127 + k) << 23);
+        inv_scale = __uint_as_float((unsigned)(127 - k) << 23);
+    };
+    unsigned amax_bits = 0;
+    float ascale_stage = 1.f;
+    auto prefetch_halo = [&](int chunk, bool live) {
+        const int cb = chunk * KCH;
+        const bool first = cb < d.C0;
+        const unsigned cs = first ? d.C0 : d.C1, coff = first ? cb : cb - d.C0;
+        const __amdgpu_buffer_rsrc_t r_s = first ? r_s0 : r_s1;
+#pragma unroll
+        for (int i = 0; i < HR; ++i) {
+            const int ho = halo_src(i);
+            const unsigned vo = (ho >= 0 && live) ? ((unsigned)ho * cs + hc * 4) * 4 : HOOB;
+            const u32x4 v = __builtin_amdgcn_raw_buffer_load_b128(r_s, vo, coff * 4, 0);
+            h_st[i] = uint4{v.x, v.y, v.z, v.w};
+        }
+    };
+    auto stage_halo_part = [&](int hbuf, int i0, int i1) {
+#pragma unroll
+        for (int i = 0; i < HR; ++i) {
+            if (i < i0 || i >= i1) continue;
+            const int row = prow + Q_HRPP * i;
+            if (row < MAXH) split_store(&Hs[hbuf * MAXH * LDH + row * LDH + hc * 4], __builtin_bit_cast(f32x4, h_st[i]), ascale_stage);
+        }
+    };
+
+    f32x16 acc[MT][NT];
+#pragma unroll
+    for (int i = 0; i < MT; ++i)
+#pragma unroll
+        for (int j = 0; j < NT; ++j)
+#pragma unroll
+            for (int r = 0; r < 16; ++r) acc[i][j][r] = 0.f;
+    int a_off[MT];
+#pragma unroll
+    for (int i = 0; i < MT; ++i) {
+        const int m = (wm * MT + i) * 32 + (lane & 31);
+        a_off[i] = ((m >> 5) * HWd + (m & 31) + wn) * LDH + (lane >> 5) * 8;
+    }
+    const int b_frag = ((wn * NT * 32 + (lane & 31)) * 128) + ((((lane >> 5) ^ (((lane & 31) >> 1) & 7))) << 4);
+    int cur_py = 0;
+    auto mfma_step = [&](int a, int b, int buf, int hbuf) {
+        const int step_off = ((cur_py + a) * HWd + b) * LDH + hbuf * MAXH * LDH;
+        const char* bf = Bs + buf * WTILE;
+#pragma unroll
+        for (int ks = 0; ks < 2; ++ks) {
+            half8 ah[MT], al[MT], bh[NT], bl[NT];
+#pragma unroll
+            for (int i = 0; i < MT; ++i) {
+                ah[i] = *reinterpret_cast<const half8*>(Hs + a_off[i] + step_off + ks * 16);
+                al[i] = *reinterpret_cast<const half8*>(Hs + a_off[i] + step_off + ks * 16 + 32);
+            }
+#pragma unroll
+            for (int j = 0; j < NT; ++j) {
+                bh[j] = *reinterpret_cast<const half8*>(bf + ((b_frag ^ (ks << 5)) + j * 32 * 128));
+                bl[j] = *reinterpret_cast<const half8*>(bf + ((b_frag ^ ((ks + 2) << 5)) + j * 32 * 128));
+            }
+#pragma unroll
+            for (int i = 0; i < MT; ++i)
+#pragma unroll
+                for (int j = 0; j < NT; ++j) acc[i][j] = __builtin_amdgcn_mfma_f32_32x32x16_f16(al[i], bh[j], acc[i][j], 0, 0, 0);
+#pragma unroll
+            for (int i = 0; i < MT; ++i)
+#pragma unroll
+                for (int j = 0; j < NT; ++j) acc[i][j] = __builtin_amdgcn_mfma_f32_32x32x16_f16(ah[i], bl[j], acc[i][j], 0, 0, 0);
+#pragma unroll
+            for (int i = 0; i < MT; ++i)
+#pragma unroll
+                for (int j = 0; j < NT; ++j) acc[i][j] = __builtin_amdgcn_mfma_f32_32x32x16_f16(ah[i], bh[j], acc[i][j], 0, 0, 0);
+        }
+    };
+
+    const int ncol = lane & 31, rsel = 4 * (lane >> 5);
+    const unsigned out_bytes = (unsigned)d.B * Ho * Wo * Cout * 4u;
+    const __amdgpu_buffer_rsrc_t r_out = __builtin_amdgcn_make_buffer_rsrc(reinterpret_cast<void*>(d.out), 0, out_bytes, 0x00020000);
+    const __amdgpu_buffer_rsrc_t r_bias = __builtin_amdgcn_make_buffer_rsrc(
+        const_cast<void*>(reinterpret_cast<const void*>(d.bias)), 0, d.bias ? (unsigned)Cout * 4u : 0u, 0x00020000);
+    const __amdgpu_buffer_rsrc_t r_stats = __builtin_amdgcn_make_buffer_rsrc(
+        reinterpret_cast<void*>(d.stats_out), 0, d.stats_out ? (unsigned)p.m_tiles * 4u * Cout * 8u : 0u, 0x00020000);
+    const unsigned o_lane = (unsigned)(((2 * wm * MT * Wo + 2 * rsel + wn) * Cout + ncol) * 4);
+    auto o_soff = [&](unsigned base, int k) {
+        const int i = k >> 5, j = (k >> 4) & 1, r = k & 15;
+        return base + (unsigned)(((2 * i * Wo + 2 * ((r & 3) + 8 * (r >> 2))) * Cout + j * 32) * 4);
+    };
+    auto tile_base = [&]() { return (unsigned)((((t_img * Ho + 2 * t_ty0 + (t_ntile & 1)) * Wo + 2 * t_tx0) * Cout + (t_ntile >> 1) * 64) * 4); };
+    auto stats_base = [&]() { return (unsigned)((((t_mtile * 2 + (t_ntile & 1)) * 2) * Cout + (t_ntile >> 1) * 64) * 8); };
+    const unsigned c_lane = (unsigned)(ncol * 4);
+    const unsigned st_lane = tid < 2 * BN ? (unsigned)(((((tid >> 1) >> 6) * Cout + ((tid >> 1) & 63)) * 2 + (tid & 1)) * 4) : HOOB;
+
+    float outv[Q_NOUT];
+    float addv[NT];
+#pragma unroll
+    for (int k = 0; k < Q_NOUT; ++k) outv[k] = 0.f;
+#pragma unroll
+    for (int j = 0; j < NT; ++j) addv[j] = 0.f;
+    unsigned pend_base = 0, pend_stats = 0;
+    unsigned cur_base = 0, cur_stats = 0;
+    float epi_cur = d.acc_scale;
+
+    auto finalize = [&]() {
+        float cs[NT], cq[NT];
+#pragma unroll
+        for (int j = 0; j < NT; ++j) {
+            cs[j] = cq[j] = 0.f;
+            const float add = addv[j];
+#pragma unroll
+            for (int i = 0; i < MT; ++i)
+#pragma unroll
+                for (int r = 0; r < 16; ++r) {
+                    const int k = (i * NT + j) * 16 + r;
+                    const float v = acc[i][j][r] * epi_cur + add;
+                    outv[k] = v;
+                    cs[j] += v;
+                    cq[j] = __builtin_fmaf(v, v, cq[j]);
+                    acc[i][j][r] = 0.f;
+                }
+            cs[j] += __shfl_xor(cs[j], 32);
+            cq[j] += __shfl_xor(cq[j], 32);
+        }
+        if (lane < 32) {
+#pragma unroll
+            for (int j = 0; j < NT; ++j) {
+                const int c = (wn * NT + j) * 32 + lane;
+                stat_lds[(wm * BN + c) * 2 + 0] = cs[j];
+                stat_lds[(wm * BN + c) * 2 + 1] = cq[j];
+            }
+        }
+        pend_base = cur_base;
+        pend_stats = cur_stats;
+    };
+    auto store_stats = [&]() {
+        const int c = (tid >> 1) & (BN - 1), which = tid & 1;
+        float a = 0.f;
+#pragma unroll
+        for (int w = 0; w < WM; ++w) a += stat_lds[(w * BN + c) * 2 + which];
+        __builtin_amdgcn_raw_buffer_store_b32(__float_as_uint(a), r_stats, st_lane, pend_stats, 0);
+    };
+
+    int v = blockIdx.x;
+    tile_of(v);
+    w_soff = (unsigned)t_ntile * BN * w_rowlen;
+    cur_base = tile_base();
+    cur_stats = stats_base();
+    cur_py = t_ntile & 1;
+    {
+        float inv;
+        amax_scales(amax_request(t_img, true), ascale_stage, inv);
+        epi_cur = d.acc_scale * inv;
+    }
+    prefetch_halo(0, true);
+    asm volatile("" ::: "memory");
+    __builtin_amdgcn_sched_barrier(0);
+    issue_w(0, 0, 0);
+    issue_w(0, 1, 1);
+    stage_halo_part(0, 0, HR);
+    if (wave >= WM * WN / 2) __builtin_amdgcn_s_setprio(1);
+
+    int hb = 0, wb = 0, n_img_next = 0, next_py = 0;
+    bool have_next = false;
+    float epi_next = epi_cur;
+    unsigned next_base = 0, next_stats = 0, next_wsoff = 0;
+
+    auto step_body = [&](auto KIND, auto STEP, int chunk) {
+        constexpr int kind = decltype(KIND)::value, step = decltype(STEP)::value;
+        asm volatile("s_waitcnt vmcnt(%0) lgkmcnt(0)" ::"n"(q_wait(kind, step)) : "memory");
+        __builtin_amdgcn_s_barrier();
+        asm volatile("" ::: "memory");
+        const bool live = kind == Q_LAST ? have_next : true;
+        if constexpr (step == 0) prefetch_halo(kind == Q_LAST ? 0 : chunk + 1, live);
+        if constexpr (step == 2) {
+            if constexpr (kind == Q_LAST) {
+                if (have_next) {
+                    float inv;
+                    amax_scales(amax_bits, ascale_stage, inv);
+                    epi_next = d.acc_scale * inv;
+                }
+            }
+            if (live) stage_halo_part(hb ^ 1, 0, HR / 2);
+        }
+        if constexpr (step == 3) {
+            if (live) stage_halo_part(hb ^ 1, HR / 2, HR);
+        }
+        asm volatile("" ::: "memory");
+        __builtin_amdgcn_sched_barrier(0);
+        if constexpr (kind == Q_FIRST) {
+            if constexpr (step == 0) store_stats();
+#pragma unroll
+            for (int k = q_first_of(step); k < q_first_of(step + 1); ++k)
+                __builtin_amdgcn_raw_buffer_store_b32(__float_as_uint(outv[k]), r_out, o_lane, o_soff(pend_base, k), 0);
+        }
+        if constexpr (kind == Q_LAST && step == 0) {
+            amax_bits = amax_request(n_img_next, have_next);
+#pragma unroll
+            for (int j = 0; j < NT; ++j)
+                addv[j] = __uint_as_float(__builtin_amdgcn_raw_buffer_load_b32(r_bias, c_lane + j * 128, (unsigned)((t_ntile >> 1) * 64 * 4), 0));
+        }
+        asm volatile("" ::: "memory");
+        __builtin_amdgcn_sched_barrier(0);
+        const int nb = wb == 0 ? NWB - 1 : wb - 1;
+        if constexpr (kind == Q_LAST && step >= 2) {
+            if (step == 2 && have_next) w_soff = next_wsoff;
+            issue_w(0, step - 2, nb);
+        } else {
+            issue_w(step + 2 < Q_STEPS ? chunk : chunk + 1, (step + 2) % Q_STEPS, nb);
+        }
+        asm volatile("" ::: "memory");
+        __builtin_amdgcn_sched_barrier(0);
+        mfma_step(step >> 1, step & 1, wb, hb);
+        wb = wb == NWB - 1 ? 0 : wb + 1;
+    };
+    auto run_chunk = [&](auto KIND, int chunk) {
+        step_body(KIND, ic<0>{}, chunk);
+        step_body(KIND, ic<1>{}, chunk);
+        step_body(KIND, ic<2>{}, chunk);
+        step_body(KIND, ic<3>{}, chunk);
+        hb ^= 1;
+    };
+
+    auto run_last = [&]() {
+        const int vn = v + G;
+        have_next = vn < total;
+        const int c_ntile = t_ntile;
+        if (have_next) {
+            tile_of(vn);
+            next_wsoff = (unsigned)t_ntile * BN * w_rowlen;
+            next_base = tile_base();
+            next_stats = stats_base();
+            next_py = t_ntile & 1;
+            n_img_next = t_img;
+        }
+        const int n_ntile = t_ntile;
+        t_ntile = c_ntile;
+        run_chunk(ic<Q_LAST>{}, nchunks - 1);
+        t_ntile = n_ntile;
+    };
+
+    bool pending = false;
+    for (;;) {
+        int c0 = 0;
+        if (pending) {
+            run_chunk(ic<Q_FIRST>{}, 0);
+            c0 = 1;
+        }
+        for (int chunk = c0; chunk < nchunks - 1; ++chunk) run_chunk(ic<Q_MID>{}, chunk);
+        run_last();
+        finalize();
+        if (!have_next) break;
+        v += G;
+        cur_base = next_base;
+        cur_stats = next_stats;
+        cur_py = next_py;
+        epi_cur = epi_next;
+        pending = true;
+    }
+    __syncthreads();
+    store_stats();
+#pragma unroll
+    for (int k = 0; k < Q_NOUT; ++k) __builtin_amdgcn_raw_buffer_store_b32(__float_as_uint(outv[k]), r_out, o_lane, o_soff(pend_base, k), 0);
+}
+
+int conv_persist_grid_cus() {
+    constexpr int MAXDEV = 64;
+    static int cached[MAXDEV];
+    int dev = 0;
+    if (hipGetDevice(&dev) != hipSuccess || dev < 0 || dev >= MAXDEV) return 256;
+    int cus = cached[dev];
+    if (cus <= 0) {
+        if (hipDeviceGetAttribute(&cus, hipDeviceAttributeMultiprocessorCount, dev) != hipSuccess || cus <= 0) cus = 256;
+        cus -= cus % 8;
+        if (cus <= 0) cus = 8;
+        cached[dev] = cus;
+    }
+    return cus;
+}
+
+bool conv3x3_s16_ups_subpixel_ok(const ddnm_conv_desc* d) {
+    if (!d || !d->ups || d->ksize != 3 || d->stride != 1 || d->pad != 1 || d->Ho != d->Hin || d->Wo != d->Win) return false;
+    if (d->B <= 0 || d->Hin <= 0 || d->Win <= 0 || ((d->Hin | d->Win) & 1)) return false;
+    const int hs = d->Hin / 2, ws = d->Win / 2, cin = d->C0 + d->C1;
+    if (ws % 32 || hs % 8 || d->C0 <= 0 || d->C1 < 0 || cin % Q_KCH || d->C0 % Q_KCH || cin / Q_KCH < 2 || d->Cout <= 0 || d->Cout % 64) return false;
+    if (d->src_f16 || d->out_nchw || d->res || d->res_ups || d->badd || d->gn_scale || d->skip0) return false;
+    if (!conv_sizes_addressable(d)) return false;
+    const int64_t lim = (int64_t)1 << 31;
+    return (int64_t)d->B * d->Ho * d->Wo * d->Cout * 4 < lim && (int64_t)d->B * (d->Ho * d->Wo / 256) * d->Cout * 8 < lim &&
+           (int64_t)4 * d->Cout * Q_STEPS * cin * 4 < lim && (int64_t)d->B * hs * ws / 256 * (d->Cout / 32) < lim;
+}
+
+int conv3x3_s16_ups_subpixel_run(const ddnm_conv_desc* d, hipStream_t s) {
+    if (!d || !d->src0 || !d->weight || !d->out || !d->amax_in || !(d->acc_scale > 0.f)) return DDNM_E_BADARG;
+    if (d->C1 > 0 && !d->src1) return DDNM_E_BADARG;
+    if (!conv3x3_s16_ups_subpixel_ok(d)) return DDNM_E_SHAPE;
+    ConvArgs p;
+    p.d = *d;
+    p.Cin = d->C0 + d->C1;
+    p.ntaps = Q_STEPS;
+    p.Hs = d->Hin / 2;
+    p.Ws = d->Win / 2;
+    p.m_tiles = d->B * (p.Hs * p.Ws / 256);
+    p.n_tiles = d->Cout / 32;
+    p.TW = 32;
+    p.TW_log2 = 5;
+    p.tiles_x = p.Ws / 32;
+    p.ksplit = 1;
+    p.ws = nullptr;
+    const int total = p.m_tiles * p.n_tiles;
+    const int cus = conv_persist_grid_cus();
+    DDNM_LAUNCH(conv2x2x4_s16_subpixel_kernel, dim3(total < cus ? total : cus), dim3(Q_NTHREADS), 0, s, p, total);
+    return 0;
+}
diff --git a/ddnm_amd/guided_diffusion/models.py b/ddnm_amd/guided_diffusion/models.py
--- a/ddnm_amd/guided_diffusion/models.py
+++ b/ddnm_amd/guided_diffusion/models.py
@@ -9,6 +9,8 @@
 
 GN_EPS = 1e-6
 SPLIT16 = os.environ.get("DDNM_CONV_F32", "split16") != "mfma32"
+UPS_SUBPIXEL = os.environ.get("DDNM_UPS_SUBPIXEL", "1")
+UPS_SUBPIXEL_MIN_TILES = 128
 CIN_PAD = 32
 
 
@@ -27,6 +29,7 @@
     def __init__(self, config, device=None, split16=None):
         self.config = config
         self.split16 = SPLIT16 if split16 is None else bool(split16)
+        self.ups_subpixel = UPS_SUBPIXEL if self.split16 else "0"
         self.fused_attn = self.split16
         self.fused_attn_max_tokens = 64
         m = config.model
@@ -228,6 +231,9 @@
                     wu = g(f"up.{lvl}.upsample.conv.weight")
                     su = ops.s16_weight_scale(wu)
                     w[f"up.{lvl}.upsample.conv.s16"] = (ops.pack_conv_weight_s16(wu, su), su, None)
+                    lr = self.resolution >> lvl
+                    if c % 64 == 0 and lr % 32 == 0:
+                        w[f"up.{lvl}.upsample.conv.s16_subpixel"] = ops.upsample_weight_s16(wu)
                 w[f"up.{lvl}.upsample.conv.bias"] = g(f"up.{lvl}.upsample.conv.bias")
         w["norm_out.weight"], w["norm_out.bias"] = g("norm_out.weight"), g("norm_out.bias")
         w["conv_out.weight"] = ops.pack_conv_weight(g("conv_out.weight"))
@@ -377,11 +383,23 @@
                     h = self._attn(attns[ib], h)
             if has_up:
                 n = f"up.{lvl}.upsample.conv"
+                if self._ups_subpixel(n, h.t.shape, c):
+                    h = ops.conv2d(h, w[n + ".weight"], c, 3, bias=w[n + ".bias"], ups=True, emit_stats=True,
+                                   weight_s16=w[n + ".s16_subpixel"], ups_subpixel=True)
+                    continue
                 h = ops.conv2d(h, w[n + ".weight"], c, 3, bias=w[n + ".bias"], ups=True, emit_stats=True,
                                weight_s16=w.get(n + ".s16"))
         gn = self._gn(h, None, "norm_out")
         return ops.conv2d(h, w["conv_out.weight"], self.out_ch, 3, gn=gn, gn_silu=True, bias=w["conv_out.bias"],
                           out_nchw=True)
 
+    def _ups_subpixel(self, n, shape, c):
+        if self.ups_subpixel == "0" or (n + ".s16_subpixel") not in self.w:
+            return False
+        B, H, W = shape[0], shape[1], shape[2]
+        if self.ups_subpixel != "all" and B * (H * W // 256) * (c // 32) < UPS_SUBPIXEL_MIN_TILES:
+            return False
+        return ops.conv_runs_ups_subpixel(B, H, W, c, c)
+
     def __call__(self, x, t):
         return self.forward(x, t)
diff --git a/ddnm_amd/ops.py b/ddnm_amd/ops.py
--- a/ddnm_amd/ops.py
+++ b/ddnm_amd/ops.py
@@ -142,6 +142,38 @@
     lo = (p - hi.float()).to(torch.float16)
     hi, lo = hi.view(cp, taps, cin // 32, 1, 32), lo.view(cp, taps, cin // 32, 1, 32)
     return torch.cat([hi, lo], 3).contiguous()
+
+
+def upsample_phase_weights(w):
+    w = w.detach().to(torch.float64)
+    sel = torch.tensor([[[1, 0, 0], [0, 1, 1]], [[1, 1, 0], [0, 0, 1]]], dtype=torch.float64, device=w.device)
+    return torch.einsum("pak,qbl,oikl->pqoiab", sel, sel, w)
+
+
+UPS_SUBPIXEL = 2
+
+
+def pack_upsample_conv_weight_s16(w, scale):
+    cout, cin = w.shape[:2]
+    if tuple(w.shape[2:]) != (3, 3) or cin % 32 or cout % 64:
+        raise ValueError("phase packing needs 3x3 weights, Cin % 32 == 0 and Cout % 64 == 0")
+    wp = upsample_phase_weights(w) * float(scale)
+    wp = wp.reshape(2, 2, cout // 64, 64, cin, 4).permute(2, 0, 1, 3, 5, 4).reshape(4 * cout, 4, cin)
+    hi = wp.to(torch.float16)
+    lo = (wp - hi.double()).to(torch.float16)
+    hi, lo = hi.view(4 * cout, 4, cin // 32, 1, 32), lo.view(4 * cout, 4, cin // 32, 1, 32)
+    return torch.cat([hi, lo], 3).contiguous()
+
+
+def upsample_weight_s16(w):
+    sc = s16_weight_scale(upsample_phase_weights(w))
+    return (pack_upsample_conv_weight_s16(w, sc), sc, None)
+
+
+def conv_runs_ups_subpixel(B, H, W, cin, cout):
+    d = _shape_desc(B, 2 * H, 2 * W, cin, cout)
+    d.ups, d.flags = 1, UPS_SUBPIXEL
+    return _lib.lib().ddnm_conv3x3_s16_ups_subpixel_supported(ctypes.byref(d)) == 1
 
 
 def conv_runs_s16(B, H, W, cin, cout, ups=False):
@@ -209,7 +241,7 @@
 def conv2d(src0, weight, cout, ksize, *, src1=None, bias=None, badd=None, badd_stride=0, res=None, res_ups=False,
            gn=None, gn_silu=True, stride=1, pad=None, ups=False, out=None, out_nchw=False, out_hw=None, tile=0,
            emit_stats=False, weight_f16=None, skip=None, skip_weight=None, skip_weight_f16=None, weight_s16=None,
-           raw_amax=None, one_tile=False):
+           raw_amax=None, one_tile=False, ups_subpixel=False):
     a_src0, a_src1 = src0, src1
     src0, src1, res = tensor_of(src0), tensor_of(src1), tensor_of(res)
     B, Hs, Ws, C0 = src0.shape
@@ -235,6 +267,12 @@
     d.badd_stride, d.tile, d.res_ups = badd_stride, tile, int(res_ups)
     d.flags = 1 if (one_tile or FORCE_ONE_TILE) else 0
     L = _lib.lib()
+    if ups_subpixel:
+        d.flags = UPS_SUBPIXEL
+        if (not ups or weight_s16 is None or weight_f16 is not None or skip is not None
+                or L.ddnm_conv3x3_s16_ups_subpixel_supported(ctypes.byref(d)) != 1):
+            raise ValueError(f"ups_subpixel: launch (B={B}, {Hs}x{Ws} -> {Ho}x{Wo}, Cin={C0 + C1}, Cout={cout}) does not "
+                             "qualify (ddnm_conv3x3_s16_ups_subpixel_supported)")
     if out_nchw and cout <= 4 and skip is None and weight_f16 is None and L.ddnm_conv3x3_small_cout_f32_supported(ctypes.byref(d)) == 1:
         _launch(L.ddnm_conv3x3_small_cout_f32, d, "ddnm_conv3x3_small_cout_f32",
                 lambda: ("conv3x3_small_cout_f32", 2.0 * B * Ho * Wo * cout * 9 * C0,
@@ -245,7 +283,7 @@
         s0, s1 = tensor_of(skip[0]), tensor_of(skip[1])
         d.skip0, d.skip1 = _p(s0), _p(s1)
         d.SC0, d.SC1 = s0.shape[3], (0 if s1 is None else s1.shape[3])
-    s16 = (weight_s16 is not None and weight_f16 is None and ksize == 3 and stride == 1
+    s16 = ups_subpixel or (weight_s16 is not None and weight_f16 is None and ksize == 3 and stride == 1
            and (skip is None or (weight_s16[2] is not None and gn is not None and d.SC0 % 32 == 0 and d.SC1 % 32 == 0))
            and L.ddnm_conv3x3_s16_supported(ctypes.byref(d)) == 1)
     s16g = (not s16 and weight_s16 is not None and weight_f16 is None and skip is None and not _NO_S16_GATHER
@@ -319,7 +357,8 @@
         elif f16:
             variant = "conv3x3_halo_f16<256x128>"
         elif s16:
-            variant = "conv3x3_s16_persist<256x128>" if L.ddnm_conv3x3_s16_persistent(ctypes.byref(d)) == 1 else "conv3x3_halo_s16<256x128>"
+            variant = ("conv2x2x4_s16_subpixel<256x128>" if ups_subpixel else
+                       "conv3x3_s16_persist<256x128>" if L.ddnm_conv3x3_s16_persistent(ctypes.byref(d)) == 1 else "conv3x3_halo_s16<256x128>")
         elif s16g:
             variant = "conv_gather_s16"
         else:
@@ -327,6 +366,8 @@
             kind = "conv3x3_halo_f32" if (ksize == 3 and stride == 1) else "conv_gather_f32"
             variant = kind + {128: "<128x128>", 64: "<64x64>", 32: "<128x32>"}[tn]
         flops = 2.0 * B * Ho * Wo * cout * (ksize * ksize * (C0 + C1) + d.SC0 + d.SC1)
+        if ups_subpixel:
+            flops *= 16.0 / 36.0
         return variant, flops, (B, Ho, Wo, C0 + C1, cout, ksize, stride, int(ups), d.SC0 + d.SC1, gn is not None,
                                 res is not None)
     _launch(fn_run, d, "ddnm_conv2d", record)
diff --git a/include/ddnm_hip.h b/include/ddnm_hip.h
--- a/include/ddnm_hip.h
+++ b/include/ddnm_hip.h
@@ -52,6 +52,7 @@
 } ddnm_conv_desc;
 
 #define DDNM_CONV_ONE_TILE 1
+#define DDNM_CONV_UPS_SUBPIXEL 2
 #define DDNM_AMAX_N 32
 
 int ddnm_conv2d_f32(const ddnm_conv_desc* d, void* stream);
@@ -73,6 +74,7 @@
 int ddnm_conv3x3_s16_persistent(const ddnm_conv_desc* d);
 int64_t ddnm_conv3x3_s16_workspace_floats(const ddnm_conv_desc* d);
 int ddnm_conv3x3_s16_stats_tiles(const ddnm_conv_desc* d);
+int ddnm_conv3x3_s16_ups_subpixel_supported(const ddnm_conv_desc* d);
 float ddnm_conv3x3_s16_act_scale(void);
 
 int ddnm_conv_gather_s16_f32(const ddnm_conv_desc* d, void* stream);
```
